# zgchen33/MCGaze

Measured on AMD Instinct MI355X. Metric: clips/sec (7x3x224x224), higher is better.
Workload: dtype f16x3; 1 GPU; full multiclue_gaze_r50 forward (R-50 + FPN + 4 decoder stages + gaze head), 64 clips/GPU x 7 frames x 3x224x224, 64 clips/step; clips_per_gpu=64, clip_length=7, global_clips=64, chunk_frames=0, parallelism=single GPU, trunk_streams=2

## Files before the change

### include/mcgaze_hip.h

```cpp
#ifndef MCGAZE_HIP_H
#define MCGAZE_HIP_H

#include <stddef.h>
#include <stdint.h>

#ifdef __cplusplus
extern "C" {
#endif

#define MCG_ABI_VERSION 20

enum { MCG_OK = 0, MCG_ERR_ARG = 1, MCG_ERR_HIP = 2, MCG_ERR_UNSUPPORTED = 3, MCG_ERR_WORKSPACE = 4 };
typedef enum { MCG_F32 = 0, MCG_BF16 = 1, MCG_F16X3 = 2, MCG_F16 = 3 } mcg_dtype;
#define MCG_ELEM_BYTES(dt) (((dt) == MCG_BF16 || (dt) == MCG_F16) ? 2 : 4)
typedef void* mcg_stream;

int mcg_abi_version(void);
const char* mcg_build_id(void);
const char* mcg_last_error(void);
int mcg_device_info(int* cu_count, size_t* hbm_bytes, char* arch, int arch_len);

int mcg_nchw_to_nhwc(mcg_stream s, mcg_dtype dt, const float* src, void* dst, int N, int C, int H, int W);
int mcg_nhwc_to_nchw(mcg_stream s, mcg_dtype dt, const void* src, float* dst, int N, int C, int H, int W);

enum { MCG_RES_NONE = 0, MCG_RES_ADD = 1, MCG_RES_UPSAMPLE_ADD = 2 };
enum {
  MCG_FLAG_STAGED_GEMM = 1,
  MCG_FLAG_NO_SPECIALISED = 2,
  MCG_FLAG_NO_ATTN_BLOCK = 4
};
typedef struct {
  const void* x;
  const void* w;
  const float* bias;
  const void* residual;
  void* y;
  int N, H, W, Cin, Cout, KH, KW, stride, pad;
  int relu;
  int residual_mode;
  int Hr, Wr;
  const void* x2;
  int Cin2, stride2, H2, W2;
  int tile;
  int flags;
  float wscale;
} mcg_conv_desc;
int mcg_conv2d(mcg_stream s, mcg_dtype dt, const mcg_conv_desc* d);

int mcg_bottleneck_x3(mcg_stream s, const float* x, const float* src2, const void* wstream, const float* bias, float* y, float* z,
                      int frames, int H, int W, int cm, int nsrc, int cn, void* trace);

size_t mcg_conv3x3_wino_x3_weight_bytes(int Cin, int Cout, int g);
int mcg_conv3x3_wino_x3(mcg_stream s, const float* x, const void* u, const float* bias, float* y, int frames, int H, int W,
                        int Cin, int Cout, int relu, int tile, float wscale, int g);
int mcg_conv3x3_wino_x3_blocks(mcg_stream s, const float* x, const void* u, const float* bias, float* y, int frames, int H, int W,
                               int Cin, int Cout, int relu, float wscale, const int* block_list, const int* block_count, int max_blocks,
                               int grid_cap);

int mcg_pointwise_stream(mcg_stream s, mcg_dtype dt, const void* a, const void* wf, const float* bias, const void* res, void* y,
                         int M, int K, int N, int relu, int res_mode, int Ho, int Wo, int Hr, int Wr, float wscale,
                         const int* block_list, const int* block_count, int grid_cap);
int mcg_pointwise_dyn(mcg_stream s, mcg_dtype dt, const void* a, const void* wf, const float* bias, void* y, int M, float wscale, int grid_cap);
int mcg_pointwise_pair(mcg_stream s, mcg_dtype dt, const void* a1, const void* a2, const void* res, const void* w3f, const float* b3,
                       void* y, const void* w1f, const float* b1, void* z, int M, int K2, int C2, int grid_cap);

size_t mcg_stem_workspace_bytes(mcg_dtype dt, int N, int H, int W);
int mcg_stem_forward(mcg_stream s, mcg_dtype dt, const float* img, const void* w_stem, const float* bias,
                     void* y, int N, int H, int W, void* ws, size_t ws_bytes, int flags);

int mcg_roi_align(mcg_stream s, mcg_dtype dt, const void* const feats[4], const int feat_h[4], const int feat_w[4],
                  const int strides[4], int C, const float* boxes, int num_boxes, int boxes_per_frame,
                  void* out, int32_t* levels_out);
int mcg_roi_align_indexed(mcg_stream s, mcg_dtype dt, const void* const feats[4], const int feat_h[4], const int feat_w[4],
                          const int strides[4], int C, const float* boxes, int num_boxes, int boxes_per_frame,
                          const int32_t* frame_of, int pyramid_frames, void* out, int32_t* levels_out);
int mcg_roi_mark_blocks(mcg_stream s, const float* boxes, int num_boxes, int boxes_per_frame, int level, int H, int W, int stride,
                        int* state, int* list, int* count);

enum {
  MCG_SW_IN_PROJ_W = 0, MCG_SW_IN_PROJ_B, MCG_SW_OUT_PROJ_W, MCG_SW_OUT_PROJ_B, MCG_SW_ATTN_LN_G, MCG_SW_ATTN_LN_B,
  MCG_SW_DYN_W,
  MCG_SW_DYN_B,
  MCG_SW_NORM_IN_G, MCG_SW_NORM_IN_B, MCG_SW_NORM_OUT_G, MCG_SW_NORM_OUT_B,
  MCG_SW_FC_W, MCG_SW_FC_B, MCG_SW_FC_LN_G, MCG_SW_FC_LN_B, MCG_SW_IIC_LN_G, MCG_SW_IIC_LN_B,
  MCG_SW_FFN1_W, MCG_SW_FFN1_B, MCG_SW_FFN2_W, MCG_SW_FFN2_B, MCG_SW_FFN_LN_G, MCG_SW_FFN_LN_B,
  MCG_SW_CLS_FC_W, MCG_SW_CLS_LN_G, MCG_SW_CLS_LN_B,
  MCG_SW_REG_FC_W,
  MCG_SW_REG_LN_G,
  MCG_SW_REG_LN_B,
  MCG_SW_HEAD_CLS_W,
  MCG_SW_HEAD_CLS_B,
  MCG_SW_HEAD_REG_W,
  MCG_SW_HEAD_REG_B,
  MCG_SW_OUT_PROJ_WF, MCG_SW_CLS_FC_WF,
  MCG_SW_REG_FC_WF,
  MCG_SW_IN_PROJ_WF,
  MCG_SW_DYN_WF,
  MCG_SW_COUNT
};
enum {
  MCG_GW_FC_W = 0,
  MCG_GW_LN_G,
  MCG_GW_LN_B,
  MCG_GW_OUT_W,
  MCG_GW_OUT_B,
  MCG_GW_FUSE_W,
  MCG_GW_FUSE_B,
  MCG_GW_COUNT
};

size_t mcg_stage_workspace_bytes(mcg_dtype dt, int num_frames);
int mcg_stage_forward(mcg_stream s, mcg_dtype dt, const void* const weights[MCG_SW_COUNT], const void* roi_feat,
                      const void* obj_in, const float* boxes_in, int num_frames, int clip_length,
                      void* obj_out, float* boxes_out, float* cls_out, const float bbox_stds[4],
                      void* ws, size_t ws_bytes, int flags);
int mcg_stage_forward_ragged(mcg_stream s, mcg_dtype dt, const void* const weights[MCG_SW_COUNT], const void* roi_feat,
                             const void* obj_in, const float* boxes_in, int num_frames, const int* clip_start, int num_clips,
                             int max_clip_length, void* obj_out, float* boxes_out, float* cls_out, const float bbox_stds[4],
                             void* ws, size_t ws_bytes, int flags);

size_t mcg_gaze_head_workspace_bytes(mcg_dtype dt, int num_frames);
int mcg_gaze_head(mcg_stream s, mcg_dtype dt, const void* const weights[MCG_GW_COUNT], const void* obj,
                  int num_frames, float* gaze_out, void* ws, size_t ws_bytes);

typedef struct {
  const void* w;
  const float* bias;
  int cin, cout, k, stride, pad;
  const void* wf;
  float wscale;
  const void* wf4;
} mcg_conv_weights;

typedef struct {
  const void* wstream;
  const float* bias;
  int conv2_index;
  int cm, c, cn;
  int nsrc;
} mcg_fused_block;

typedef struct {
  int blocks[4];
  mcg_conv_weights stem;
  const mcg_conv_weights* convs;
  int num_convs;
  mcg_conv_weights lateral[4];
  mcg_conv_weights fpn_out[4];
  mcg_conv_weights c3_ds[4];
  const float* init_boxes;
  const void* init_feats;
  int num_stages;
  const void* const* stage_weights;
  const void* const* gaze_weights;
  float bbox_stds[4];
  const mcg_fused_block* fused;
  int num_fused;
} mcg_model_weights;

typedef struct mcg_engine mcg_engine;
int mcg_engine_create(mcg_engine** out, const mcg_model_weights* w, mcg_dtype dt);
void mcg_engine_destroy(mcg_engine* e);
int mcg_engine_set_option(mcg_engine* e, const char* name, int value);
int mcg_engine_range_audit(mcg_engine* e, unsigned long long* counts, const char** names, int capacity, int* n_out);
size_t mcg_engine_workspace_bytes(const mcg_engine* e, int num_frames, int H, int W, int chunk_frames);
int mcg_backbone_fpn_forward(mcg_engine* e, mcg_stream s, const float* img, int num_frames, int H, int W,
                             int chunk_frames, void* const pyramid[4], void* ws, size_t ws_bytes);
size_t mcg_trunk_workspace_bytes(const mcg_engine* e, int num_frames, int H, int W, int chunk_frames);
size_t mcg_decoder_workspace_bytes(const mcg_engine* e, int num_frames);
int mcg_decoder_forward(mcg_engine* e, mcg_stream s, const void* const pyramid[4], int num_frames, int clip_length, int H, int W,
                        const int* img_hw, float* gaze_out, float* boxes_out, float* scores_out, void* ws, size_t ws_bytes);
int mcg_decoder_forward_indexed(mcg_engine* e, mcg_stream s, const void* const pyramid[4], int pyramid_frames, const int32_t* frame_of,
                                int num_frames, int clip_length, int H, int W, const int* img_hw, float* gaze_out, float* boxes_out,
                                float* scores_out, void* ws, size_t ws_bytes);
int mcg_decoder_forward_ragged(mcg_engine* e, mcg_stream s, const void* const pyramid[4], int pyramid_frames, const int32_t* frame_of,
                               int num_frames, const int* clip_start, int num_clips, int max_clip_length, int H, int W, const int* img_hw,
                               float* gaze_out, float* boxes_out, float* scores_out, void* ws, size_t ws_bytes);
size_t mcg_deferred_pyramid_bytes(const mcg_engine* e, int num_frames, int H, int W);
int mcg_deferred_pyramid_levels(const mcg_engine* e, void* slot, int num_frames, int H, int W, void* levels[4], int* deferred);
int mcg_deferred_pyramid_state(const mcg_engine* e, void* slot, int num_frames, int H, int W, void** inner, int** flags, int** counts,
                               int** lists, int* blocks, int* lateral_deferred);
int mcg_inner_block_neighbours(int id, int H, int W, int out[9]);
int mcg_inner_mark_blocks(mcg_stream s, const int* out_list, const int* out_count, int H, int W, int nblk, int* state, int* list, int* count);
int mcg_backbone_fpn_forward_deferred(mcg_engine* e, mcg_stream s, const float* img, int num_frames, int H, int W, int chunk_frames,
                                      void* slot, size_t slot_bytes, void* ws, size_t ws_bytes);
int mcg_decoder_forward_deferred(mcg_engine* e, mcg_stream s, void* slot, size_t slot_bytes, int num_frames, int clip_length, int H, int W,
                                 const int* img_hw, float* gaze_out, float* boxes_out, float* scores_out, void* ws, size_t ws_bytes);
int mcg_decoder_forward_deferred_ragged(mcg_engine* e, mcg_stream s, void* slot, size_t slot_bytes, int num_frames, const int* clip_start,
                                        int num_clips, int max_clip_length, int H, int W, const int* img_hw, float* gaze_out,
                                        float* boxes_out, float* scores_out, void* ws, size_t ws_bytes);
int mcg_clip_forward(mcg_engine* e, mcg_stream s, const float* img, int num_frames, int clip_length, int H, int W,
                     const int* img_hw, int chunk_frames, float* gaze_out, float* boxes_out, float* scores_out,
                     void* ws, size_t ws_bytes);
int mcg_clip_forward_ragged(mcg_engine* e, mcg_stream s, const float* img, int num_frames, const int* clip_start, int num_clips,
                            int max_clip_length, int H, int W, const int* img_hw, int chunk_frames, float* gaze_out, float* boxes_out,
                            float* scores_out, void* ws, size_t ws_bytes);
int mcg_pyramid_scatter_rows(mcg_stream s, mcg_dtype dt, const void* const src[4], void* const dst[4],
                             int num_frames, int store_rows, int H, int W, const int32_t* row_of);
int mcg_merge_windows(mcg_stream s, const float* gaze, const float* boxes, const float* scores, int num_frames, const float* scale,
                      int scale_per_frame, const int32_t* plan, int num_dst, int max_src, float* store, int store_rows,
                      float person_threshold);
int mcg_smooth_gaze(mcg_stream s, const float* store, int store_rows, const int32_t* plan, int num_out, double alpha, float* out);

typedef struct mcg_frame_desc {
  const void* src;
  int src_h, src_w, src_pitch;
  int crop_y, crop_x, crop_h, crop_w;
  int out_h, out_w;
} mcg_frame_desc;
int mcg_preprocess_frames(mcg_stream stream, const mcg_frame_desc* frames_dev, int num_frames, float* dst, int pad_h, int pad_w,
                          const float mean[3], const float stdinv[3], int to_rgb);
typedef struct mcg_image_desc {
  const void* src;
  int h, w, pitch;
} mcg_image_desc;
int mcg_preprocess_head_crops(mcg_stream s, const mcg_image_desc* images_dev, int num_images, const float* boxes_dev,
                              const int32_t* image_of_dev, int n, double expand, int scale_w, int scale_h, mcg_frame_desc* desc_out_dev,
                              int32_t* img_hw_dev, float* scale_factor_dev, int32_t* flags_dev, float* dst, int pad_h, int pad_w,
                              const float mean[3], const float stdinv[3], int to_rgb);
typedef struct mcg_yuv_coef {
  int y_off, cy, cub, cug, cvg, cvr;
} mcg_yuv_coef;
typedef struct mcg_nv12_image_desc {
  const void* y;
  const void* uv;
  int h, w, pitch_y, pitch_uv;
} mcg_nv12_image_desc;
typedef struct mcg_nv12_frame_desc {
  const void* src;
  int src_h, src_w, src_pitch;
  int crop_y, crop_x, crop_h, crop_w;
  int out_h, out_w;
  const void* uv;
  int uv_pitch;
} mcg_nv12_frame_desc;
int mcg_preprocess_frames_nv12(mcg_stream stream, const mcg_nv12_frame_desc* frames_dev, int num_frames, float* dst, int pad_h, int pad_w,
                               const float mean[3], const float stdinv[3], int to_rgb, const mcg_yuv_coef* coef);
int mcg_preprocess_head_crops_nv12(mcg_stream s, const mcg_nv12_image_desc* images_dev, int num_images, const float* boxes_dev,
                                   const int32_t* image_of_dev, int n, double expand, int scale_w, int scale_h,
                                   mcg_nv12_frame_desc* desc_out_dev, int32_t* img_hw_dev, float* scale_factor_dev, int32_t* flags_dev,
                                   float* dst, int pad_h, int pad_w, const float mean[3], const float stdinv[3], int to_rgb,
                                   const mcg_yuv_coef* coef);

typedef struct mcg_arrow_desc {
  int seg[3][2][2];
  int thickness;
  int x0, y0, x1, y1;
  int image, flag;
  int reserved;
} mcg_arrow_desc;
int mcg_draw_gaze_arrows(mcg_stream s, const mcg_image_desc* images_dev, int num_images, int max_h, int max_w, const float* boxes_dev,
                         const float* gaze_dev, int gaze_stride, const int32_t* image_of_dev, int n, double length, int min_thickness,
                         double thickness_ratio, double tip_length, const unsigned char* color, const unsigned char* colors_dev,
                         mcg_arrow_desc* plan_out_dev, int32_t* flags_dev);
int mcg_draw_gaze_arrows_nv12(mcg_stream s, const mcg_nv12_image_desc* images_dev, int num_images, int max_h, int max_w, const float* boxes_dev,
                              const float* gaze_dev, int gaze_stride, const int32_t* image_of_dev, int n, double length, int min_thickness,
                              double thickness_ratio, double tip_length, const unsigned char* yuv, const unsigned char* yuvs_dev,
                              mcg_arrow_desc* plan_out_dev, int32_t* flags_dev);

size_t mcg_detect_heads_workspace_bytes(int num_images, int num_anchors);
int mcg_detect_heads(mcg_stream s, const float* pred_dev, int num_images, int num_anchors, int num_classes, long long image_stride, int row_stride,
                     int in_h, int in_w, const int32_t* frame_hw_dev , double conf_thres, double iou_thres,
                     int only_class , int agnostic, int max_nms, int max_det,
                     float* boxes_dev , float* scores_dev , int32_t* classes_dev ,
                     int32_t* image_of_dev , int32_t* counts_dev , int32_t* flags_dev ,
                     void* ws_dev, size_t ws_bytes);

enum { MCG_LETTERBOX_U8 = 0, MCG_LETTERBOX_F16 = 1, MCG_LETTERBOX_F32 = 2 };
typedef struct mcg_letterbox_desc {
  mcg_frame_desc frame;
  int top, left;
} mcg_letterbox_desc;
typedef struct mcg_nv12_letterbox_desc {
  mcg_nv12_frame_desc frame;
  int top, left;
} mcg_nv12_letterbox_desc;
int mcg_letterbox_frames(mcg_stream stream, const mcg_letterbox_desc* frames_dev, int num_frames, void* dst, int out_h, int out_w, int out_type,
                         int swap_rb);
int mcg_letterbox_frames_nv12(mcg_stream stream, const mcg_nv12_letterbox_desc* frames_dev, int num_frames, void* dst, int out_h, int out_w,
                              int out_type, int swap_rb, const mcg_yuv_coef* coef);

typedef struct mcg_track_header {
  int32_t next_id;
  int32_t frames_seen;
  int32_t reserved[2];
} mcg_track_header;
typedef struct mcg_track_slot {
  float box[4];
  int32_t id;
  int32_t age;
  int32_t reserved[2];
} mcg_track_slot;
size_t mcg_track_state_bytes(int num_sequences, int slots);
int mcg_track_heads(mcg_stream s, const float* boxes_dev, long long frame_stride, const int32_t* counts_dev, int num_sequences, int num_frames,
                    int max_det, int slots, double match_iou, int max_age, void* state_dev,
                    float* slot_boxes_dev , int32_t* image_of_dev , int32_t* track_id_dev ,
                    int32_t* age_dev , int32_t* det_of_dev , int32_t* flags_dev );

int mcg_track_heads_motion(mcg_stream s, const float* boxes_dev, long long frame_stride, const int32_t* counts_dev, int num_sequences,
                           int num_frames, int max_det, int slots, double match_iou, int max_age, double velocity_gain, double coast_decay,
                           void* state_dev, float* slot_boxes_dev , int32_t* image_of_dev ,
                           int32_t* track_id_dev , int32_t* age_dev , int32_t* det_of_dev ,
                           int32_t* flags_dev , float* state_boxes_dev );

int mcg_live_slots(mcg_stream s, const void* state_dev, int num_cameras, int slots, int tick, int ring_depth, float* crop_boxes_dev,
                   int32_t* image_of_dev, int32_t* ring_id_dev, float* ring_box_dev, int32_t* matched_dev);
int mcg_live_gate(mcg_stream s, const int32_t* ring_id_dev, const float* ring_box_dev, int ring_depth, int num_cameras, int slots, int tick,
                  const int32_t* table_dev, int num_entries, int first_out, int num_out, const float* fused_dev, const float* others_dev,
                  float* fused_smooth_dev, float* others_smooth_dev, int32_t* track_id_dev, int32_t* valid_dev, float* head_box_dev,
                  int32_t* image_of_dev, int32_t* smooth_valid_dev);

int mcg_live_lanes(mcg_stream s, const void* state_dev, int num_cameras, int slots, int lanes, int tick, int ring_depth,
                   int32_t* lane_state_dev, float* crop_boxes_dev, int32_t* image_of_dev, int32_t* ring_id_dev, float* ring_box_dev,
                   int32_t* ring_col_dev, int32_t* lane_of_dev, int32_t* matched_dev, int32_t* overflow_dev);
int mcg_live_gate_lanes(mcg_stream s, const int32_t* ring_id_dev, const float* ring_box_dev, const int32_t* ring_col_dev, int ring_depth,
                        int num_cameras, int slots, int lanes, int tick, const int32_t* table_dev, int num_entries, int first_out, int num_out,
                        const float* fused_dev, const float* others_dev, float* fused_smooth_dev, float* others_smooth_dev,
                        int32_t* track_id_dev, int32_t* valid_dev, int32_t* camera_dev, int32_t* slot_dev, float* head_box_dev,
                        int32_t* image_of_dev, int32_t* smooth_valid_dev);

int mcg_gaze_targets(mcg_stream s, const float* boxes_dev, const float* gaze_dev, int gaze_stride, const int32_t* image_of_dev, int n,
                     const float* regions_dev, const int32_t* region_image_dev, int m, int region_period, double expand, double camera_cos2,
                     int32_t* kind_dev, int32_t* target_dev, float* t_dev, float* hit_dev, int32_t* mutual_dev, int32_t* flags_dev);

int mcg_gaze_dwell(mcg_stream s, const int32_t* person_dev, const int32_t* tag_dev, const int32_t* kind_dev, const int32_t* ident_dev,
                   const int32_t* mutual_dev, int num_frames, int columns, int frame0, int enter, int exit_frames, int32_t* state_dev,
                   int32_t* region_frames_dev, int num_regions, int32_t* dwell_dev, int32_t* ended_dev, int32_t* events_dev, int max_events,
                   int32_t* num_events_dev);

#define MCG_ATTEND_POLY_VERTS 32
int mcg_gaze_targets_poly(mcg_stream s, const float* boxes_dev, const float* gaze_dev, int gaze_stride, const int32_t* image_of_dev, int n,
                          const float* region_xy_dev, int num_vertices, const int32_t* region_start_dev, const int32_t* region_image_dev, int m,
                          int region_period, double expand, double camera_cos2, int32_t* kind_dev, int32_t* target_dev, float* t_dev,
                          float* hit_dev, int32_t* mutual_dev, int32_t* flags_dev);

typedef struct mcg_stroke_desc {
  int seg[3][2][2];
  int thickness;
  int x0, y0, x1, y1;
  int image, flag;
  int layer, count;
  unsigned color, color_active;
  int reserved;
} mcg_stroke_desc;
int mcg_draw_attention(mcg_stream s, const mcg_image_desc* images_dev, int num_images, int max_h, int max_w, const float* boxes_dev,
                       const float* gaze_dev, int gaze_stride, const int32_t* image_of_dev, int n, const int32_t* kind_dev, const int32_t* target_dev,
                       const float* hit_dev, const int32_t* mutual_dev, const float* region_xy_dev, int num_vertices,
                       const int32_t* region_start_dev, const int32_t* region_image_dev, int m, int region_period, const unsigned char* palette,
                       double length, int min_thickness, double thickness_ratio, double tip_length, int line_thickness, int region_thickness,
                       void* workspace_dev, size_t workspace_bytes, int32_t* flags_dev, int32_t* region_flags_dev, int32_t* region_active_dev);
int mcg_draw_attention_nv12(mcg_stream s, const mcg_nv12_image_desc* images_dev, int num_images, int max_h, int max_w, const float* boxes_dev,
                            const float* gaze_dev, int gaze_stride, const int32_t* image_of_dev, int n, const int32_t* kind_dev,
                            const int32_t* target_dev, const float* hit_dev, const int32_t* mutual_dev, const float* region_xy_dev, int num_vertices,
                            const int32_t* region_start_dev, const int32_t* region_image_dev, int m, int region_period, const unsigned char* palette,
                            double length, int min_thickness, double thickness_ratio, double tip_length, int line_thickness, int region_thickness,
                            void* workspace_dev, size_t workspace_bytes, int32_t* flags_dev, int32_t* region_flags_dev, int32_t* region_active_dev);

#define MCG_LABEL_CHARS 24
typedef struct mcg_label_desc {
  int x, y;
  int x0, y0, x1, y1;
  int image, flag;
  int len;
  unsigned color;
  unsigned char text[MCG_LABEL_CHARS];
} mcg_label_desc;
int mcg_format_labels(mcg_stream s, const int32_t* id_dev, const int32_t* value_dev, int n, int num, int den, unsigned char* text_out_dev);
int mcg_draw_labels(mcg_stream s, const mcg_image_desc* images_dev, int num_images, int max_h, int max_w, const float* boxes_dev,
                    const int32_t* image_of_dev, const unsigned char* text_dev, const int32_t* place_dev, int n, const unsigned char* font_dev,
                    int scale, int advance, int pad, const unsigned char* color, const unsigned char* colors_dev, const unsigned char* background,
                    mcg_label_desc* plan_out_dev, int32_t* flags_dev);
int mcg_draw_labels_nv12(mcg_stream s, const mcg_nv12_image_desc* images_dev, int num_images, int max_h, int max_w, const float* boxes_dev,
                         const int32_t* image_of_dev, const unsigned char* text_dev, const int32_t* place_dev, int n, const unsigned char* font_dev,
                         int scale, int advance, int pad, const unsigned char* yuv, const unsigned char* yuvs_dev, const unsigned char* background,
                         mcg_label_desc* plan_out_dev, int32_t* flags_dev);

int mcg_gaze_heat_add(mcg_stream s, const float* hit_dev, const int32_t* kind_dev, const int32_t* image_of_dev, const int32_t* flags_dev,
                      const int32_t* mask_dev, int n, int32_t* heat_dev, int32_t* peak_dev, int C, int GH, int GW, int cell_shift, int radius,
                      int kinds, int period, int decay_shift, void* workspace_dev, size_t workspace_bytes);
int mcg_draw_heat(mcg_stream s, const mcg_image_desc* images_dev, int num_images, int max_h, int max_w, const int32_t* heat_dev,
                  const int32_t* full_dev, int C, int GH, int GW, int cell_shift, int period, const unsigned char* lut_dev, int min_level);
int mcg_draw_heat_nv12(mcg_stream s, const mcg_nv12_image_desc* images_dev, int num_images, int max_h, int max_w, const int32_t* heat_dev,
                       const int32_t* full_dev, int C, int GH, int GW, int cell_shift, int period, const unsigned char* lut_dev, int min_level);

typedef struct mcg_anon_desc {
  int image, flag;
  int x0, y0, x1, y1;
  int cx2, cy2;
  int W, H;
  int shift, shape;
} mcg_anon_desc;
int mcg_anonymize_heads(mcg_stream s, const mcg_image_desc* images_dev, int num_images, int max_h, int max_w, const float* boxes_dev,
                        const int32_t* image_of_dev, int n, double expand, int shape, int cell_shift, int blocks, int mode,
                        const unsigned char* color, mcg_anon_desc* plan_out_dev, int32_t* flags_dev);
int mcg_anonymize_heads_nv12(mcg_stream s, const mcg_nv12_image_desc* images_dev, int num_images, int max_h, int max_w, const float* boxes_dev,
                             const int32_t* image_of_dev, int n, double expand, int shape, int cell_shift, int blocks, int mode,
                             const unsigned char* yuv, mcg_anon_desc* plan_out_dev, int32_t* flags_dev);

int mcg_engine_profile_start(mcg_engine* e, int capacity);
int mcg_engine_profile_stop(mcg_engine* e, int* count, float* ms, double* flops, double* algo_bytes, int* cfg, int* shape_mnk, int capacity);
int mcg_bench_backbone_forward(mcg_engine* e, mcg_stream s, const float* img, int num_frames, int H, int W, void* ws, size_t ws_bytes);
int mcg_bench_backbone_levels(const mcg_engine* e, void* ws, int num_frames, int H, int W, void* levels[4]);

#ifdef __cplusplus
}
#endif
#endif
```

### mcgaze_amd/csrc/check_resources.py

```python
#!/usr/bin/env python3
import re
import sys

RULES = {
    'wino_x3w_kernel': dict(scratch=0, vgpr_spill=0, unit='engine'),
    'wino_x3w_blocks_kernel': dict(scratch=0, vgpr_spill=0, unit='engine'),
    'gaze_targets_kernel': dict(scratch=0, vgpr_spill=0, unit='attend'),
    'gaze_targets_poly_kernel': dict(scratch=0, vgpr_spill=0, unit='attend'),
    'gaze_mutual_kernel': dict(scratch=0, vgpr_spill=0, unit='attend'),
    'gaze_dwell_kernel': dict(scratch=0, vgpr_spill=0, unit='dwell'),
    'gaze_dwell_events_kernel': dict(scratch=0, vgpr_spill=0, unit='dwell'),
    'label_raster_kernel': dict(scratch=0, vgpr_spill=0, unit='labels'),
    'heat_render_kernel': dict(scratch=0, vgpr_spill=0, unit='heat'),
    'anonymize_render_kernel': dict(scratch=0, vgpr_spill=0, unit='anonymize'),
}


def parse(path):
    kernels, cur = [], None
    for line in open(path, errors='replace'):
        m = re.search(r'remark: (?:\s*)Function Name: (\S+)', line)
        if m:
            cur = dict(name=m.group(1))
            kernels.append(cur)
            continue
        m = re.search(r'remark:\s+([A-Za-z \[\]/]+): (\S+) \[-Rpass-analysis', line)
        if m and cur is not None:
            cur[m.group(1).strip()] = m.group(2)
    return kernels


def main():
    path = sys.argv[1]
    kernels = parse(path)
    other = [l.rstrip() for l in open(path, errors='replace') if 'Rpass-analysis=kernel-resource-usage' not in l and not re.match(r'\s+\d* *\|', l) and l.strip()
             and not l.startswith('In file included from') and not re.match(r'\d+ (warning|remark)s? generated', l.strip())]
    for l in other:
        print(l, file=sys.stderr)
    bad = []
    import os
    unit = os.path.basename(path).split('.')[0]
    for prefix, lim in RULES.items():
        if lim.get('unit') == unit and not any(prefix in k['name'] and 'VGPRs Spill' in k and 'ScratchSize [bytes/lane]' in k for k in kernels):
            bad.append(f'{prefix}: no resource remarks found in {path} (expected -Rpass-analysis=kernel-resource-usage output for it)')
    for k in kernels:
        for prefix, lim in RULES.items():
            if prefix in k['name']:
                scratch = int(k.get('ScratchSize [bytes/lane]', '0'))
                spill = int(k.get('VGPRs Spill', '0'))
                if scratch > lim['scratch'] or spill > lim['vgpr_spill']:
                    bad.append(f"{k['name']}: scratch {scratch} B/lane, {spill} spilled VGPRs (limits {lim['scratch']}, {lim['vgpr_spill']})")
    if '--table' in sys.argv:
        print('| kernel | VGPRs | AGPRs | SGPRs | scratch B/lane | VGPR spill | waves/SIMD |\n|---|---|---|---|---|---|---|')
        for k in kernels:
            print(f"| `{k['name']}` | {k.get('VGPRs')} | {k.get('AGPRs')} | {k.get('TotalSGPRs')} | {k.get('ScratchSize [bytes/lane]')} | {k.get('VGPRs Spill')} | {k.get('Occupancy [waves/SIMD]')} |")
    if bad:
        print('check_resources: kernels that must not spill (RULES):\n  ' + '\n  '.join(bad), file=sys.stderr)
        return 1
    return 0


if __name__ == '__main__':
    sys.exit(main())
```

### mcgaze_amd/csrc/engine.hip

```cpp
#include "igemm.hpp"
#include "pw_pair.hpp"
#include "pw_single.hpp"
#include "bneck_x3.hpp"
#include "pw_single_x3.hpp"
#include "wino_x3.hpp"

#include <stdarg.h>
#include <stdlib.h>
#include <string.h>

#include <map>
#include <mutex>
#include <string>
#include <vector>

int launch_roi_align(hipStream_t s, mcg_dtype dt, const void* const feats[4], const int feat_h[4], const int feat_w[4],
                     const int strides[4], int C, const float* boxes, int num_boxes, int boxes_per_frame, const int32_t* frame_of,
                     int pyramid_frames, void* out, int32_t* levels_out);
int launch_init_queries(hipStream_t s, mcg_dtype dt, const float* init_boxes, const void* init_feats, const int* img_hw,
                        const int32_t* frame_of, int pyramid_frames, int H, int W, float* boxes, void* obj, int N);
bool roi_mark_supported(int H, int W);
int launch_defer_clear(hipStream_t s, int* p, int n);
int launch_roi_mark(hipStream_t s, const float* boxes, int num_boxes, int boxes_per_frame, int level, int H, int W, int stride, int* state,
                    int* list, int* count);
int launch_inner_mark(hipStream_t s, const int* out_list, const int* out_count, int H, int W, int nblk, int* state, int* list, int* count);

struct mcg_engine {
  mcg_dtype dt;
  int blocks[4];
  mcg_conv_weights stem;
  std::vector<mcg_conv_weights> convs;
  mcg_conv_weights lateral[4], fpn_out[4], c3_ds[4];
  std::vector<mcg_fused_block> fused;
  bool bneck_fused = true;
  bool bneck_blocked = true;
  int winograd = 1;
  int wino_tile = -1;
  int fpn_deferred = 1;
  int fpn_lateral_deferred = 1;
  static constexpr int kAuditCap = 256;
  unsigned long long* audit_dev = nullptr;
  std::vector<std::string> audit_names;
  const float* init_boxes;
  const void* init_feats;
  int num_stages;
  std::vector<const void*> stage_w;
  const void* gaze_w[MCG_GW_COUNT];
  float stds[4];
  static constexpr int kMaxSplit = 4, kCandidates = 8;
  struct StreamPool* pool = nullptr;
  hipStream_t* cand = nullptr;
  hipEvent_t ev_fork = nullptr, ev_join[kMaxSplit - 1] = {};
  McgCtx ctx;
  Prof prof;
  int trunk_streams = 2;
  int max_range_frames = 0;
  bool pw_single = true;
  bool pw_pair = true;
  std::mutex mu;
};
struct StreamPool {
  hipStream_t cand[mcg_engine::kCandidates] = {};
  hipEvent_t ev_probe[3] = {};
  std::map<hipStream_t, std::vector<int>> side_of;
  std::mutex mu;
  bool ok = false;
};
static StreamPool* stream_pool_for_current_device() {
  static std::mutex g_mu;
  static std::map<int, StreamPool*> g_pools;
  int dev = 0;
  if (hipGetDevice(&dev) != hipSuccess) return nullptr;
  std::lock_guard<std::mutex> lock(g_mu);
  auto it = g_pools.find(dev);
  if (it != g_pools.end()) return it->second;
  StreamPool* p = new StreamPool();
  bool ok = true;
  for (int i = 0; i < mcg_engine::kCandidates; ++i) ok = ok && hipStreamCreateWithFlags(&p->cand[i], hipStreamNonBlocking) == hipSuccess;
  for (int i = 0; i < 3; ++i) ok = ok && hipEventCreate(&p->ev_probe[i]) == hipSuccess;
  p->ok = ok;
  g_pools[dev] = p;
  return p;
}
__global__ void probe_spin_kernel(long long ticks) {
  const long long t0 = wall_clock64();
  while (wall_clock64() - t0 < ticks) {}
}
static const std::vector<int>& side_streams_for(mcg_engine* e, hipStream_t s) {
  StreamPool* p = e->pool;
  std::lock_guard<std::mutex> lock(p->mu);
  auto it = p->side_of.find(s);
  if (it != p->side_of.end()) return it->second;
  std::vector<int> good, rest;
  const long long ticks = 15000;
  for (int c = 0; c < mcg_engine::kCandidates; ++c) {
    bool concurrent = false;
    if (hipEventRecord(p->ev_probe[0], s) == hipSuccess) {
      hipLaunchKernelGGL(probe_spin_kernel, dim3(1), dim3(64), 0, s, ticks);
      hipLaunchKernelGGL(probe_spin_kernel, dim3(1), dim3(64), 0, p->cand[c], ticks);
      float ms = 0.f;
      if (hipEventRecord(p->ev_probe[1], s) == hipSuccess && hipEventRecord(p->ev_probe[2], p->cand[c]) == hipSuccess &&
          hipEventSynchronize(p->ev_probe[1]) == hipSuccess && hipEventSynchronize(p->ev_probe[2]) == hipSuccess &&
          hipEventElapsedTime(&ms, p->ev_probe[0], p->ev_probe[2]) == hipSuccess)
        concurrent = ms < 0.15f * 1.6f;
    }
    (concurrent ? good : rest).push_back(c);
  }
  (void)hipGetLastError();
  good.insert(good.end(), rest.begin(), rest.end());
  return p->side_of.emplace(s, good).first->second;
}
static int range_frame_cap(const mcg_engine* e, int H, int W) {
  const long long per_frame = (long long)(H / 4) * (W / 4) * 256 * (mcg_is16(e->dt) ? 2 : 4);
  long long cap = 0x7FFFFF00ll / (per_frame > 0 ? per_frame : 1);
  if (e->max_range_frames > 0 && e->max_range_frames < cap) cap = e->max_range_frames;
  return cap < 1 ? 1 : (cap > 0x7fffffff ? 0x7fffffff : (int)cap);
}
static const int kMinFramesPerRange = 56;
static int trunk_ranges(const mcg_engine* e, int frames) {
  int k = e->trunk_streams;
  if (k > mcg_engine::kMaxSplit) k = mcg_engine::kMaxSplit;
  while (k > 1 && frames / k < kMinFramesPerRange) --k;
  return k < 1 ? 1 : k;
}

static inline size_t al256(size_t b) { return (b + 255) / 256 * 256; }
static inline size_t esize(mcg_dtype dt) { return mcg_is16(dt) ? 2 : 4; }

extern "C" void mcg_engine_destroy(mcg_engine* e);
extern "C" int mcg_engine_create(mcg_engine** out, const mcg_model_weights* w, mcg_dtype dt) {
  MCG_CHECK_ARG(out && w, "mcg_engine_create: null pointer");
  MCG_CHECK_ARG(dt == MCG_F32 || dt == MCG_BF16 || dt == MCG_F16X3 || dt == MCG_F16, "mcg_engine_create: unknown dtype %d", (int)dt);
  int expect = 0;
  for (int l = 0; l < 4; ++l) {
    MCG_CHECK_ARG(w->blocks[l] > 0, "mcg_engine_create: blocks[%d]=%d", l, w->blocks[l]);
    expect += 3 * w->blocks[l] + 1;
  }
  MCG_CHECK_ARG(w->num_convs == expect && w->convs, "mcg_engine_create: expected %d bottleneck convs, got %d", expect, w->num_convs);
  MCG_CHECK_ARG(w->num_stages > 0 && w->stage_weights && w->gaze_weights && w->init_boxes && w->init_feats, "mcg_engine_create: decoder tables missing");
  for (int i = 0; i < w->num_convs; ++i)
    MCG_CHECK_ARG(w->convs[i].w && w->convs[i].bias, "mcg_engine_create: conv %d has a null pointer", i);
  mcg_engine* e = new mcg_engine();
  e->dt = dt;
  memcpy(e->blocks, w->blocks, sizeof(e->blocks));
  e->stem = w->stem;
  e->convs.assign(w->convs, w->convs + w->num_convs);
  memcpy(e->lateral, w->lateral, sizeof(e->lateral));
  memcpy(e->fpn_out, w->fpn_out, sizeof(e->fpn_out));
  memcpy(e->c3_ds, w->c3_ds, sizeof(e->c3_ds));
  if (w->fused && w->num_fused > 0 && dt == MCG_F16X3) e->fused.assign(w->fused, w->fused + w->num_fused);
  e->init_boxes = w->init_boxes;
  e->init_feats = w->init_feats;
  e->num_stages = w->num_stages;
  e->stage_w.assign(w->stage_weights, w->stage_weights + (size_t)w->num_stages * MCG_SW_COUNT);
  memcpy(e->gaze_w, w->gaze_weights, sizeof(e->gaze_w));
  memcpy(e->stds, w->bbox_stds, sizeof(e->stds));
  bool ok = hipEventCreateWithFlags(&e->ev_fork, hipEventDisableTiming) == hipSuccess;
  e->pool = stream_pool_for_current_device();
  ok = ok && e->pool && e->pool->ok;
  if (e->pool) e->cand = e->pool->cand;
  for (int i = 0; i < mcg_engine::kMaxSplit - 1; ++i) ok = ok && hipEventCreateWithFlags(&e->ev_join[i], hipEventDisableTiming) == hipSuccess;
  if (!ok) {
    mcg_engine_destroy(e);
    mcg_set_error("mcg_engine_create: could not create the side streams / events");
    return MCG_ERR_HIP;
  }
  *out = e;
  return MCG_OK;
}

extern "C" int mcg_engine_set_option(mcg_engine* e, const char* name, int value) {
  MCG_CHECK_ARG(e && name, "mcg_engine_set_option: null pointer");
  std::lock_guard<std::mutex> lock(e->mu);
  if (!strcmp(name, "trunk_streams")) { MCG_CHECK_ARG(value >= 1 && value <= mcg_engine::kMaxSplit, "trunk_streams must be 1..%d", mcg_engine::kMaxSplit); e->trunk_streams = value; }
  else if (!strcmp(name, "max_range_frames")) { MCG_CHECK_ARG(value >= 0, "max_range_frames must be >= 0"); e->max_range_frames = value; }
  else if (!strcmp(name, "tile")) e->ctx.tile = value > 0 ? value : -1;
  else if (!strcmp(name, "staged_gemm")) e->ctx.staged = value != 0;
  else if (!strcmp(name, "conv3x3_c64")) e->ctx.c64 = value != 0;
  else if (!strcmp(name, "stem_fused")) e->ctx.stem_fused = value != 0;
  else if (!strcmp(name, "decoder_chain")) e->ctx.chain = value != 0;
  else if (!strcmp(name, "decoder_attn_block")) e->ctx.attn_block = value != 0;
  else if (!strcmp(name, "pointwise_pair")) e->pw_pair = value != 0;
  else if (!strcmp(name, "pointwise_stream")) e->pw_single = value != 0;
  else if (!strcmp(name, "bottleneck_fused")) e->bneck_fused = value != 0;
  else if (!strcmp(name, "bottleneck_blocked")) e->bneck_blocked = value != 0;
  else if (!strcmp(name, "winograd")) { MCG_CHECK_ARG(value >= 0 && value <= 2, "winograd must be 0, 1 or 2"); e->winograd = value; }
  else if (!strcmp(name, "fpn_deferred")) e->fpn_deferred = value != 0;
  else if (!strcmp(name, "fpn_lateral_deferred")) e->fpn_lateral_deferred = value != 0;
  else if (!strcmp(name, "wino_tile")) { MCG_CHECK_ARG(value >= -1 && value <= 3, "wino_tile must be -1 (by grid size) .. 3"); e->wino_tile = value; }
  else if (!strcmp(name, "range_audit")) {
    MCG_CHECK_ARG(!mcg_is16(e->dt) || !value, "range_audit: f32-storage engines only (MCG_F32, MCG_F16X3)");
    if (value && !e->audit_dev) {
      if (hipMalloc((void**)&e->audit_dev, sizeof(unsigned long long) * 2 * mcg_engine::kAuditCap) != hipSuccess) { e->audit_dev = nullptr; mcg_set_error("range_audit: hipMalloc failed"); return MCG_ERR_HIP; }
    }
    if (value && hipMemset(e->audit_dev, 0, sizeof(unsigned long long) * 2 * mcg_engine::kAuditCap) != hipSuccess) { mcg_set_error("range_audit: hipMemset failed"); return MCG_ERR_HIP; }
    if (!value && e->audit_dev) { (void)hipFree(e->audit_dev); e->audit_dev = nullptr; }
    e->audit_names.clear();
  }
  else { mcg_set_error("mcg_engine_set_option: unknown option '%s'", name); return MCG_ERR_ARG; }
  return MCG_OK;
}

extern "C" int mcg_engine_profile_start(mcg_engine* e, int capacity) {
  MCG_CHECK_ARG(e, "mcg_engine_profile_start: null engine");
  std::lock_guard<std::mutex> lock(e->mu);
  if (e->prof.recs) { mcg_set_error("mcg_engine_profile_start: already armed"); return MCG_ERR_ARG; }
  MCG_CHECK_ARG(capacity > 0 && capacity <= (1 << 20), "mcg_engine_profile_start: bad capacity %d", capacity);
  e->prof.recs = new ProfRec[capacity];
  for (int i = 0; i < capacity; ++i) { e->prof.recs[i].a = nullptr; e->prof.recs[i].b = nullptr; }
  for (int i = 0; i < capacity; ++i) {
    if (hipEventCreate(&e->prof.recs[i].a) != hipSuccess || hipEventCreate(&e->prof.recs[i].b) != hipSuccess) {
      for (int j = 0; j <= i; ++j) {
        if (e->prof.recs[j].a) (void)hipEventDestroy(e->prof.recs[j].a);
        if (e->prof.recs[j].b) (void)hipEventDestroy(e->prof.recs[j].b);
      }
      delete[] e->prof.recs;
      e->prof = Prof();
      mcg_set_error("mcg_engine_profile_start: hipEventCreate failed");
      return MCG_ERR_HIP;
    }
  }
  e->prof.cap = capacity; e->prof.n = 0;
  e->ctx.prof = &e->prof;
  return MCG_OK;
}
extern "C" int mcg_engine_profile_stop(mcg_engine* e, int* count, float* ms, double* flops, double* bytes, int* cfg, int* shape, int capacity) {
  MCG_CHECK_ARG(e, "mcg_engine_profile_stop: null engine");
  std::lock_guard<std::mutex> lock(e->mu);
  if (!e->prof.recs) { mcg_set_error("mcg_engine_profile_stop: not armed"); return MCG_ERR_ARG; }
  const int n = e->prof.n;
  int rc = MCG_OK;
  for (int i = 0; i < n; ++i) {
    const ProfRec& r = e->prof.recs[i];
    float t = 0.f;
    if (hipEventSynchronize(r.b) != hipSuccess || hipEventElapsedTime(&t, r.a, r.b) != hipSuccess) rc = MCG_ERR_HIP;
    if (i < capacity) {
      if (ms) ms[i] = t;
      if (flops) flops[i] = r.flops;
      if (bytes) bytes[i] = r.bytes;
      if (cfg) cfg[i] = r.cfg;
      if (shape) { shape[3 * i] = r.shape[0]; shape[3 * i + 1] = r.shape[1]; shape[3 * i + 2] = r.shape[2]; }
    }
  }
  for (int i = 0; i < e->prof.cap; ++i) { (void)hipEventDestroy(e->prof.recs[i].a); (void)hipEventDestroy(e->prof.recs[i].b); }
  delete[] e->prof.recs;
  e->prof = Prof();
  e->ctx.prof = nullptr;
  if (count) *count = n < capacity ? n : capacity;
  if (rc != MCG_OK) mcg_set_error("mcg_engine_profile_stop: event query failed");
  return rc;
}
extern "C" void mcg_engine_destroy(mcg_engine* e) {
  if (!e) return;
  if (e->ev_fork) (void)hipEventDestroy(e->ev_fork);
  for (int i = 0; i < mcg_engine::kMaxSplit - 1; ++i)
    if (e->ev_join[i]) (void)hipEventDestroy(e->ev_join[i]);
  if (e->prof.recs) {
    for (int i = 0; i < e->prof.cap; ++i) { (void)hipEventDestroy(e->prof.recs[i].a); (void)hipEventDestroy(e->prof.recs[i].b); }
    delete[] e->prof.recs;
  }
  if (e->audit_dev) (void)hipFree(e->audit_dev);
  delete e;
}

__global__ void range_audit_kernel(const float* __restrict__ x, long long n, unsigned long long* __restrict__ cnt) {
  unsigned long long big = 0, bad = 0;
  for (long long i = (long long)blockIdx.x * blockDim.x + threadIdx.x; i < n; i += (long long)gridDim.x * blockDim.x) {
    const float v = x[i];
    if (!(fabsf(v) <= 3.4028235e38f)) ++bad;
    else if (fabsf(v) > 65504.f) ++big;
  }
  big = (unsigned long long)wave_sum((float)big) ;
  bad = (unsigned long long)wave_sum((float)bad);
  if ((threadIdx.x & 63) == 0) {
    if (big) atomicAdd(cnt, big);
    if (bad) atomicAdd(cnt + 1, bad);
  }
}
struct AuditCursor { mcg_engine* e; hipStream_t s; int idx; bool naming; };
__attribute__((format(printf, 4, 5))) static void audit_tensor(AuditCursor& a, const void* p, long long elements, const char* fmt, ...) {
  if (!a.e->audit_dev || a.idx >= mcg_engine::kAuditCap) return;
  if (a.naming) {
    char name[64];
    va_list ap;
    va_start(ap, fmt);
    vsnprintf(name, sizeof(name), fmt, ap);
    va_end(ap);
    a.e->audit_names.push_back(name);
  }
  const long long per_thread = 16;
  long long blocks = (elements + 256 * per_thread - 1) / (256 * per_thread);
  if (blocks > 4096) blocks = 4096;
  if (blocks < 1) blocks = 1;
  hipLaunchKernelGGL(range_audit_kernel, dim3((int)blocks), dim3(256), 0, a.s, (const float*)p, elements, a.e->audit_dev + 2 * a.idx);
  ++a.idx;
}

struct TrunkWs {
  char *stem_ws, *x0, *xa, *xb, *o1, *o2, *ds, *c[4], *l[4];
  size_t stem_bytes, big, total;
};
static TrunkWs trunk_layout(mcg_dtype dt, int n, int H, int W, char* base) {
  const size_t es = esize(dt);
  const size_t h2 = H / 4, w2 = W / 4;
  TrunkWs t;
  size_t off = 0;
  auto take = [&](size_t bytes) { char* p = base ? base + off : nullptr; off += al256(bytes); return p; };
  t.stem_bytes = mcg_stem_workspace_bytes(dt, n, H, W);
  t.stem_ws = take(t.stem_bytes);
  t.big = (size_t)n * h2 * w2 * 256 * es;
  t.x0 = take((size_t)n * h2 * w2 * 64 * es);
  t.xa = take(t.big); t.xb = take(t.big);
  t.o1 = take(t.big / 2); t.o2 = take(t.big / 2);
  t.ds = take(t.big);
  for (int i = 0; i < 4; ++i) {
    const size_t hi = (H / 4) >> i, wi = (W / 4) >> i;
    t.c[i] = take((size_t)n * hi * wi * (256u << i) * es);
    t.l[i] = take((size_t)n * hi * wi * 256 * es);
  }
  t.total = off;
  return t;
}

static int wino_kind(const mcg_engine* e, mcg_dtype dt, const mcg_conv_weights& cw, int n, int h, int w, int rm) {
  return (dt == MCG_F16X3 && e->winograd && e->ctx.tile < 0 && cw.k == 3 && cw.stride == 1 && cw.pad == 1 && rm == MCG_RES_NONE)
             ? ((cw.wf4 && e->winograd >= 2 && wino_x3_applicable(n, h, w, cw.cin, cw.cout, 4)) ? 4 : ((cw.wf && wino_x3_applicable(n, h, w, cw.cin, cw.cout, 2)) ? 2 : 0))
             : 0;
}
static WinoParams wino_params(const mcg_conv_weights& cw, int g, const void* x, int n, int h, int w, void* y, int relu) {
  WinoParams wp;
  memset(&wp, 0, sizeof(wp));
  wp.x = (const float*)x; wp.u = g == 4 ? cw.wf4 : cw.wf; wp.bias = cw.bias; wp.y = (float*)y;
  wp.H = h; wp.W = w; wp.frames = n; wp.Cin = cw.cin; wp.Cout = cw.cout; wp.relu = relu; wp.wscale = cw.wscale;
  return wp;
}
static ProfRec* prof_begin_wino(const McgCtx& ctx, hipStream_t s, const mcg_conv_weights& cw, long long M, bool book = true) {
  return prof_begin(ctx, s, 73, (int)M, cw.cout, 9 * cw.cin, book ? 2.0 * M * 9.0 * cw.cin * cw.cout : 0.0,
                    book ? 4.0 * ((double)M * (cw.cin + cw.cout) + 9.0 * cw.cin * cw.cout) : 0.0);
}
static int launch_done(ProfRec* rec, hipStream_t s, int rc, const char* what) {
  prof_end(rec, s);
  if (rc) { mcg_set_error("%s launch failed", what); return MCG_ERR_HIP; }
  return MCG_OK;
}
static mcg_conv_desc conv_desc(mcg_dtype dt, const mcg_conv_weights& cw, const void* x, int n, int h, int w, void* y, int relu,
                               const void* res, int res_mode, int hr, int wr) {
  mcg_conv_desc d;
  memset(&d, 0, sizeof(d));
  d.x = x; d.w = cw.w; d.bias = cw.bias; d.residual = res; d.y = y;
  d.N = n; d.H = h; d.W = w; d.Cin = cw.cin; d.Cout = cw.cout; d.KH = cw.k; d.KW = cw.k; d.stride = cw.stride; d.pad = cw.pad;
  d.relu = relu; d.residual_mode = res_mode; d.Hr = hr; d.Wr = wr;
  d.wscale = dt == MCG_F16X3 ? cw.wscale : 0.f;
  return d;
}
static int conv_call(const mcg_engine* e, hipStream_t s, mcg_dtype dt, const mcg_conv_weights& cw, const void* x, int n, int h, int w, void* y,
                     int relu, const void* res, int res_mode, int hr, int wr) {
  const long long M = (long long)n * h * w;
  const int rm = res ? res_mode : MCG_RES_NONE;
  const long long res_m = rm == MCG_RES_UPSAMPLE_ADD ? (long long)n * hr * wr : M;
  const bool x3 = dt == MCG_F16X3;
  if ((x3 || mcg_is16(dt)) && e->pw_single && e->ctx.tile < 0 && cw.wf && cw.bias && cw.k == 1 && cw.stride == 1 && cw.pad == 0 && M < 0x7fffffffll &&
      (x3 ? pw_single_x3_applicable(cw.cin, cw.cout, rm, M, res_m) : !e->ctx.staged && pw_single_applicable(cw.cin, cw.cout, rm, M, res_m))) {
    PwSingleParams pp;
    memset(&pp, 0, sizeof(pp));
    pp.a = x; pp.res = res; pp.wf = cw.wf; pp.bias = cw.bias; pp.y = y;
    pp.M = (int)M; pp.relu = relu; pp.Ho = h; pp.Wo = w; pp.wscale = x3 ? cw.wscale : 0.f;
    if (rm == MCG_RES_UPSAMPLE_ADD) { pp.Hr = hr; pp.Wr = wr; pp.rscale_h = (float)hr / (float)h; pp.rscale_w = (float)wr / (float)w; }
    ProfRec* rec = prof_begin(e->ctx, s, x3 ? 71 : 61, pp.M, cw.cout, cw.cin, 2.0 * M * cw.cin * cw.cout,
                              (double)esize(dt) * ((double)M * (cw.cin + cw.cout) + (rm == MCG_RES_NONE ? 0.0 : (double)res_m) * cw.cout + (double)cw.cin * cw.cout));
    const int rmode = rm == MCG_RES_NONE ? 0 : (rm == MCG_RES_ADD ? 1 : 2);
    return launch_done(rec, s, x3 ? launch_pw_single_x3(s, pp, cw.cout, rmode) : launch_pw_single(s, pp, cw.cin, cw.cout, rmode, dt),
                       x3 ? "pw_single_x3" : "pw_single");
  }
  const int wg = wino_kind(e, dt, cw, n, h, w, rm);
  if (wg) {
    ProfRec* rec = prof_begin_wino(e->ctx, s, cw, M);
    return launch_done(rec, s, launch_wino_x3(s, wino_params(cw, wg, x, n, h, w, y, relu), e->wino_tile, wg), "wino_x3");
  }
  const mcg_conv_desc d = conv_desc(dt, cw, x, n, h, w, y, relu, res, res_mode, hr, wr);
  return conv2d_ctx(s, dt, &d, e->ctx);
}

struct TrunkCursor {
  const void* x;
  int h, w, ci;
  char *o1, *o2;
  bool o1_ready;
  bool x_blocked;
};
static const mcg_fused_block* fused_tail_at(const mcg_engine* e, int ci, int b) {
  if (!(e->dt == MCG_F16X3 && e->bneck_fused && e->ctx.tile < 0) || ci + 2 >= (int)e->convs.size()) return nullptr;
  const mcg_fused_block* f = nullptr;
  for (const mcg_fused_block& q : e->fused)
    if (q.conv2_index == ci + 1) f = &q;
  if (!f) return nullptr;
  const bool ds = b == 0;
  const mcg_conv_weights &d2 = e->convs[ci + 1], &d3 = e->convs[ci + 2];
  const int kk = ds ? e->convs[ci + 3].cin : 0, ss = ds ? e->convs[ci + 3].stride : 1;
  const int cn_i = ci + (ds ? 4 : 3);
  const bool nx = f->cn == 0 || (cn_i < (int)e->convs.size() && e->convs[cn_i].k == 1 && e->convs[cn_i].stride == 1 && e->convs[cn_i].cout == f->cn && e->convs[cn_i].cin == f->c);
  return (d2.k == 3 && d2.stride == 1 && d2.pad == 1 && d2.cin == f->cm && d2.cout == f->cm && d3.cout == f->c && f->nsrc == (ds ? 2 : 1) && nx &&
          bneck_x3_applicable(f->cm, f->c, f->cn, f->nsrc, kk, ss)) ? f : nullptr;
}
static int fused_tail_step(const mcg_engine* e, hipStream_t s, const TrunkWs& t, AuditCursor& au, TrunkCursor& c, const mcg_fused_block* fb,
                           int n, int l, int b, void* y) {
  const bool has_ds = b == 0;
  const int k2 = has_ds ? e->convs[c.ci + 3].cin : 0;
  BneckParams bp;
  memset(&bp, 0, sizeof(bp));
  bp.x = (const float*)c.o1; bp.res = (const float*)c.x; bp.wstream = (const char*)fb->wstream; bp.bias = fb->bias;
  bp.y = (float*)y; bp.z = (float*)c.o2; bp.H = c.h; bp.W = c.w;
  const long long blk_bytes = (long long)n * ((c.h + bnx::TH - 1) / bnx::TH) * ((c.w + bnx::TW - 1) / bnx::TW) * bnx::NPIX * fb->c * (long long)esize(e->dt);
  const mcg_fused_block* fnext = (b + 1 < e->blocks[l]) ? fused_tail_at(e, c.ci + (has_ds ? 4 : 3), b + 1) : nullptr;
  bp.res_blocked = c.x_blocked ? 1 : 0;
  bp.y_blocked = (e->bneck_blocked && !e->audit_dev && y != (void*)t.c[l] && fb->cn > 0 && fnext && fnext->nsrc == 1 && fnext->c == fb->c &&
                  blk_bytes <= (long long)t.big) ? 1 : 0;
  const double M = (double)n * c.h * c.w;
  ProfRec* rec = prof_begin(e->ctx, s, 70, n * c.h * c.w, fb->c + fb->cn, 9 * fb->cm + fb->cm + k2 + fb->c,
                            2.0 * M * (9.0 * fb->cm * fb->cm + (double)(fb->cm + k2) * fb->c + (double)fb->c * fb->cn),
                            4.0 * (M * (fb->cm + (has_ds ? k2 : fb->c) + fb->c + fb->cn) + 9.0 * fb->cm * fb->cm + (double)(fb->cm + k2) * fb->c + (double)fb->c * fb->cn));
  MCG_TRY(launch_done(rec, s, launch_bneck_x3(s, bp, n, fb->cm, fb->nsrc, fb->cn), "bneck_x3"));
  audit_tensor(au, y, (long long)n * c.h * c.w * fb->c, "layer%d.%d.out (fused tail)", l + 1, b);
  if (fb->cn > 0) {
    audit_tensor(au, c.o2, (long long)n * c.h * c.w * fb->cn, "layer%d.%d.next_conv1 (fused tail)", l + 1, b);
    std::swap(c.o1, c.o2);
    c.o1_ready = true;
  }
  c.x_blocked = bp.y_blocked != 0;
  return MCG_OK;
}
static const mcg_conv_weights* pw_pair_next(const mcg_engine* e, int ci, int l, int b, long long M) {
  const bool has_ds = b == 0;
  const mcg_conv_weights& c3 = e->convs[ci + 2];
  const mcg_conv_weights* c3w = has_ds ? (e->c3_ds[l].w ? &e->c3_ds[l] : nullptr) : &c3;
  const int ci_next = ci + (has_ds ? 4 : 3);
  const mcg_conv_weights* c1n = ci_next < (int)e->convs.size() ? &e->convs[ci_next] : nullptr;
  const int k2 = has_ds ? e->convs[ci + 3].cin : 0;
  return (mcg_is16(e->dt) && e->pw_pair && l == 0 && c3w && c1n && c3w->wf && c1n->wf && c3w->bias && c1n->bias && c1n->k == 1 && c1n->stride == 1 &&
          c1n->cin == c3.cout && pw_pair_applicable(c3.cin, k2, has_ds ? e->convs[ci + 3].stride : 1, c3.cout, c1n->cout, M) && M < 0x7fffffffll)
             ? c1n : nullptr;
}
static int pw_pair_step(const mcg_engine* e, hipStream_t s, TrunkCursor& c, const mcg_conv_weights& c1n, int n, int l, int b, void* y, int ho, int wo) {
  const bool has_ds = b == 0;
  const mcg_conv_weights& c3 = e->convs[c.ci + 2];
  const mcg_conv_weights& c3w = has_ds ? e->c3_ds[l] : c3;
  PwPairParams pp;
  memset(&pp, 0, sizeof(pp));
  pp.a1 = c.o2; pp.K1 = c3.cin;
  if (has_ds) { pp.a2 = c.x; pp.K2 = e->convs[c.ci + 3].cin; pp.stride2 = e->convs[c.ci + 3].stride; pp.H2 = c.h; pp.W2 = c.w; }
  else pp.res = c.x;
  pp.w3f = c3w.wf; pp.b3 = c3w.bias; pp.y = y;
  pp.w1f = c1n.wf; pp.b1 = c1n.bias; pp.z = c.o1;
  pp.M = n * ho * wo; pp.C = c3.cout; pp.C2 = c1n.cout; pp.Ho = ho; pp.Wo = wo;
  ProfRec* rec = prof_begin(e->ctx, s, 60, pp.M, pp.C + pp.C2, pp.K1 + pp.K2, 2.0 * pp.M * ((double)(pp.K1 + pp.K2) * pp.C + (double)pp.C * pp.C2),
                            2.0 * ((double)pp.M * (pp.K1 + pp.K2 + (has_ds ? 0 : pp.C) + pp.C + pp.C2) + (double)(pp.K1 + pp.K2) * pp.C + (double)pp.C * pp.C2));
  MCG_TRY(launch_done(rec, s, launch_pw_pair(s, pp, e->dt), "pw_pair"));
  c.o1_ready = true;
  return MCG_OK;
}
static int conv3_step(const mcg_engine* e, hipStream_t s, const TrunkWs& t, AuditCursor& au, const TrunkCursor& c, int n, int l, int b, void* y,
                      int ho, int wo) {
  const mcg_conv_weights& c3 = e->convs[c.ci + 2];
  if (b == 0 && e->c3_ds[l].w) {
    const mcg_conv_weights& ds = e->convs[c.ci + 3];
    mcg_conv_desc d = conv_desc(e->dt, e->c3_ds[l], c.o2, n, ho, wo, y, 1, nullptr, MCG_RES_NONE, 0, 0);
    d.Cin = c3.cin;
    d.x2 = c.x; d.Cin2 = ds.cin; d.stride2 = ds.stride; d.H2 = c.h; d.W2 = c.w;
    MCG_TRY(conv2d_ctx(s, e->dt, &d, e->ctx));
  } else {
    const void* identity = c.x;
    if (b == 0) {
      MCG_TRY(conv_call(e, s, e->dt, e->convs[c.ci + 3], c.x, n, c.h, c.w, t.ds, 0, nullptr, MCG_RES_NONE, 0, 0));
      identity = t.ds;
    }
    MCG_TRY(conv_call(e, s, e->dt, c3, c.o2, n, ho, wo, y, 1, identity, MCG_RES_ADD, 0, 0));
  }
  audit_tensor(au, y, (long long)n * ho * wo * c3.cout, "layer%d.%d.out", l + 1, b);
  return MCG_OK;
}

struct TrunkKeep { char *inner, *c2, *l1; };
static int trunk_chunk(mcg_engine* e, hipStream_t s, const float* img, int f0, int n, int H, int W, void* const pyr[4], char* wsbase,
                       bool backbone_only = false, const TrunkKeep tk = TrunkKeep{nullptr, nullptr, nullptr}) {
  const mcg_dtype dt = e->dt;
  const size_t es = esize(dt);
  TrunkWs t = trunk_layout(dt, n, H, W, wsbase);
  char* const inner0 = tk.inner;
  if (inner0) t.l[0] = inner0 + (size_t)f0 * (H / 4) * (W / 4) * 256 * es;
  const bool lateral_deferred = inner0 && tk.c2 && tk.l1;
  if (lateral_deferred) {
    t.c[0] = tk.c2 + (size_t)f0 * (H / 4) * (W / 4) * 256 * es;
    t.l[1] = tk.l1 + (size_t)f0 * (H / 8) * (W / 8) * 256 * es;
  }
  MCG_TRY(stem_forward_ctx(s, dt, img + (size_t)f0 * 3 * H * W, e->stem.w, e->stem.bias, t.x0, n, H, W, t.stem_ws, t.stem_bytes, e->ctx));
  AuditCursor au{e, s, 0, e->audit_dev != nullptr && e->audit_names.empty()};
  audit_tensor(au, t.x0, (long long)n * (H / 4) * (W / 4) * 64, "stem");
  TrunkCursor c{t.x0, H / 4, W / 4, 0, t.o1, t.o2, false, false};
  for (int l = 0; l < 4; ++l) {
    for (int b = 0; b < e->blocks[l]; ++b) {
      const mcg_conv_weights &c1 = e->convs[c.ci], &c2 = e->convs[c.ci + 1];
      const int ho = (c.h + 2 * c2.pad - c2.k) / c2.stride + 1, wo = (c.w + 2 * c2.pad - c2.k) / c2.stride + 1;
      void* y = (b == e->blocks[l] - 1) ? (void*)t.c[l] : (c.x == t.xa ? (void*)t.xb : (void*)t.xa);
      if (!c.o1_ready) {
        MCG_TRY(conv_call(e, s, dt, c1, c.x, n, c.h, c.w, c.o1, 1, nullptr, MCG_RES_NONE, 0, 0));
        audit_tensor(au, c.o1, (long long)n * c.h * c.w * c1.cout, "layer%d.%d.conv1", l + 1, b);
      }
      c.o1_ready = false;
      const mcg_fused_block* fb = fused_tail_at(e, c.ci, b);
      if (c.x_blocked && !(fb && fb->nsrc == 1)) { mcg_set_error("trunk: a blocked tensor reached a kernel that does not read that layout"); return MCG_ERR_UNSUPPORTED; }
      if (fb) {
        MCG_TRY(fused_tail_step(e, s, t, au, c, fb, n, l, b, y));
      } else {
        MCG_TRY(conv_call(e, s, dt, c2, c.o1, n, c.h, c.w, c.o2, 1, nullptr, MCG_RES_NONE, 0, 0));
        audit_tensor(au, c.o2, (long long)n * ho * wo * c2.cout, "layer%d.%d.conv2", l + 1, b);
        const mcg_conv_weights* c1n = pw_pair_next(e, c.ci, l, b, (long long)n * ho * wo);
        MCG_TRY(c1n ? pw_pair_step(e, s, c, *c1n, n, l, b, y, ho, wo) : conv3_step(e, s, t, au, c, n, l, b, y, ho, wo));
      }
      c.x = y; c.h = ho; c.w = wo;
      c.ci += b == 0 ? 4 : 3;
    }
  }
  if (backbone_only) return MCG_OK;
  int hs[4], wsz[4];
  for (int i = 0; i < 4; ++i) { hs[i] = (H / 4) >> i; wsz[i] = (W / 4) >> i; }
  for (int i = 3; i >= (lateral_deferred ? 1 : 0); --i) {
    const void* res = i == 3 ? nullptr : t.l[i + 1];
    MCG_TRY(conv_call(e, s, dt, e->lateral[i], t.c[i], n, hs[i], wsz[i], t.l[i], 0, res, res ? MCG_RES_UPSAMPLE_ADD : MCG_RES_NONE,
                      i == 3 ? 0 : hs[i + 1], i == 3 ? 0 : wsz[i + 1]));
    audit_tensor(au, t.l[i], (long long)n * hs[i] * wsz[i] * 256, "fpn.lateral%d (+ top-down)", i);
  }
  for (int i = inner0 ? 1 : 0; i < 4; ++i) {
    char* dst = (char*)pyr[i] + (size_t)f0 * hs[i] * wsz[i] * 256 * es;
    MCG_TRY(conv_call(e, s, dt, e->fpn_out[i], t.l[i], n, hs[i], wsz[i], dst, 0, nullptr, MCG_RES_NONE, 0, 0));
    audit_tensor(au, dst, (long long)n * hs[i] * wsz[i] * 256, "fpn.P%d", i + 2);
  }
  return MCG_OK;
}

extern "C" int mcg_engine_range_audit(mcg_engine* e, unsigned long long* counts, const char** names, int capacity, int* n_out) {
  MCG_CHECK_ARG(e && counts && n_out && capacity > 0, "mcg_engine_range_audit: bad argument");
  std::lock_guard<std::mutex> lock(e->mu);
  if (!e->audit_dev) { mcg_set_error("mcg_engine_range_audit: the range_audit option is off"); return MCG_ERR_ARG; }
  const int n = (int)e->audit_names.size() < capacity ? (int)e->audit_names.size() : capacity;
  if (hipDeviceSynchronize() != hipSuccess ||
      hipMemcpy(counts, e->audit_dev, sizeof(unsigned long long) * 2 * n, hipMemcpyDeviceToHost) != hipSuccess ||
      hipMemset(e->audit_dev, 0, sizeof(unsigned long long) * 2 * mcg_engine::kAuditCap) != hipSuccess) {
    mcg_set_error("mcg_engine_range_audit: device read failed");
    return MCG_ERR_HIP;
  }
  if (names) for (int i = 0; i < n; ++i) names[i] = e->audit_names[i].c_str();
  *n_out = n;
  return MCG_OK;
}

struct DecWs {
  char *roi, *obj_a, *obj_b, *stage_ws, *gaze_ws;
  float *boxes_a, *boxes_b, *cls;
  size_t stage_bytes, gaze_bytes, total;
};
static DecWs dec_layout(mcg_dtype dt, int N, char* base) {
  const size_t es = esize(dt), R = (size_t)N * 3;
  DecWs c;
  memset(&c, 0, sizeof(c));
  size_t off = 0;
  auto take = [&](size_t bytes) { char* p = base ? base + off : nullptr; off += al256(bytes); return p; };
  c.roi = take(R * 49 * 256 * es);
  c.obj_a = take(R * 256 * es); c.obj_b = take(R * 256 * es);
  c.boxes_a = (float*)take(R * 4 * 4); c.boxes_b = (float*)take(R * 4 * 4); c.cls = (float*)take(R * 4);
  c.stage_bytes = mcg_stage_workspace_bytes(dt, N); c.stage_ws = take(c.stage_bytes);
  c.gaze_bytes = mcg_gaze_head_workspace_bytes(dt, N); c.gaze_ws = take(c.gaze_bytes);
  c.total = off;
  return c;
}
static bool check_shape_ok(int N, int H, int W) { return N > 0 && H >= 32 && W >= 32 && H % 32 == 0 && W % 32 == 0; }
static size_t pyramid_bytes(mcg_dtype dt, int N, int H, int W, int level) {
  return al256((size_t)N * ((H / 4) >> level) * ((W / 4) >> level) * 256 * esize(dt));
}

struct DeferSlot {
  void* p[4];
  char* inner;
  int *state, *count, *list;
  int nblk;
  bool deferred;
  bool lateral;
  char *c2, *l1;
  int *istate, *icount, *ilist;
  size_t total;
};
static bool fpn_deferred_on(const mcg_engine* e, int N, int H, int W) {
  const mcg_conv_weights& cw = e->fpn_out[0];
  const int h = H / 4, w = W / 4;
  return e->fpn_deferred && e->dt == MCG_F16X3 && !e->audit_dev && e->num_stages > 0 && wino_kind(e, e->dt, cw, N, h, w, MCG_RES_NONE) == 2 &&
         wino_x3_blocks_applicable(N, h, w, cw.cin, cw.cout) && roi_mark_supported(h, w);
}
static bool fpn_lateral_deferred_on(const mcg_engine* e, int N, int H, int W) {
  const mcg_conv_weights& cw = e->lateral[0];
  const int h = H / 4, w = W / 4;
  return e->fpn_lateral_deferred && fpn_deferred_on(e, N, H, W) && e->pw_single && e->ctx.tile < 0 && cw.wf && cw.bias && cw.k == 1 && cw.stride == 1 &&
         cw.pad == 0 && h % 2 == 0 && w % 2 == 0 &&
         pw_single_x3_blocks_applicable(cw.cin, cw.cout, h, w, (long long)N * h * w, (long long)N * (h / 2) * (w / 2));
}
static DeferSlot defer_layout(const mcg_engine* e, int N, int H, int W, char* base) {
  DeferSlot d;
  memset(&d, 0, sizeof(d));
  size_t off = 0;
  auto take = [&](size_t bytes) { char* p = base ? base + off : nullptr; off += al256(bytes); return p; };
  for (int i = 0; i < 4; ++i) d.p[i] = take(pyramid_bytes(e->dt, N, H, W, i));
  d.deferred = fpn_deferred_on(e, N, H, W);
  if (d.deferred) {
    d.inner = take((size_t)N * (H / 4) * (W / 4) * 256 * esize(e->dt));
    d.nblk = N * wino_x3_blocks_per_frame(H / 4, W / 4);
    d.lateral = fpn_lateral_deferred_on(e, N, H, W);
    const size_t per = (size_t)d.nblk + e->num_stages;
    d.state = (int*)take(sizeof(int) * per * (d.lateral ? 2 : 1));
    d.count = d.state ? d.state + d.nblk : nullptr;
    d.list = (int*)take(sizeof(int) * (size_t)d.nblk * e->num_stages);
    if (d.lateral) {
      d.istate = d.state ? d.state + per : nullptr;
      d.icount = d.istate ? d.istate + d.nblk : nullptr;
      d.ilist = (int*)take(sizeof(int) * (size_t)d.nblk * e->num_stages);
      d.c2 = take((size_t)N * (H / 4) * (W / 4) * 256 * esize(e->dt));
      d.l1 = take((size_t)N * (H / 8) * (W / 8) * 256 * esize(e->dt));
    }
  }
  d.total = off;
  return d;
}

extern "C" size_t mcg_trunk_workspace_bytes(const mcg_engine* e, int N, int H, int W, int chunk) {
  if (!e || N <= 0) return 0;
  if (chunk <= 0 || chunk > N) chunk = N;
  if (chunk < N) return trunk_layout(e->dt, chunk, H, W, nullptr).total;
  size_t total = 0;
  const int cap = range_frame_cap(e, H, W);
  for (int k = 1; k <= mcg_engine::kMaxSplit; ++k) {
    const int per = (N + k - 1) / k < cap ? (N + k - 1) / k : cap;
    const size_t t = (size_t)k * al256(trunk_layout(e->dt, per, H, W, nullptr).total);
    if (t > total) total = t;
  }
  return total;
}
extern "C" size_t mcg_decoder_workspace_bytes(const mcg_engine* e, int N) {
  if (!e || N <= 0) return 0;
  return dec_layout(e->dt, N, nullptr).total;
}
extern "C" size_t mcg_engine_workspace_bytes(const mcg_engine* e, int N, int H, int W, int chunk) {
  if (!e || N <= 0) return 0;
  return mcg_trunk_workspace_bytes(e, N, H, W, chunk) + mcg_decoder_workspace_bytes(e, N) + defer_layout(e, N, H, W, nullptr).total;
}
extern "C" size_t mcg_deferred_pyramid_bytes(const mcg_engine* e, int N, int H, int W) {
  if (!e || N <= 0 || check_shape_ok(N, H, W) == false) return 0;
  return defer_layout(e, N, H, W, nullptr).total;
}

static int check_shape(int N, int H, int W) {
  MCG_CHECK_ARG(N > 0, "num_frames must be positive (got %d)", N);
  MCG_CHECK_ARG(H >= 32 && W >= 32 && H % 32 == 0 && W % 32 == 0, "frame size %dx%d must be a multiple of 32 (Pad(size_divisor=32))", H, W);
  return MCG_OK;
}

static int trunk_forward(mcg_engine* e, mcg_stream s_, const float* img, int N, int H, int W, int chunk,
                         void* const pyramid[4], void* ws, size_t ws_bytes, bool backbone_only, const TrunkKeep tk = TrunkKeep{nullptr, nullptr, nullptr}) {
  MCG_CHECK_ARG(e && img && (pyramid || backbone_only) && ws, "mcg_backbone_fpn_forward: null pointer");
  MCG_TRY(check_shape(N, H, W));
  std::lock_guard<std::mutex> lock(e->mu);
  if (chunk <= 0 || chunk > N) chunk = N;
  const size_t need = mcg_trunk_workspace_bytes(e, N, H, W, chunk);
  if (ws_bytes < need) { mcg_set_error("mcg_backbone_fpn_forward: workspace too small (%zu < %zu)", ws_bytes, need); return MCG_ERR_WORKSPACE; }
  const int k = chunk < N ? 1 : trunk_ranges(e, N), cap = range_frame_cap(e, H, W);
  const int per = chunk < N ? chunk : ((N + k - 1) / k < cap ? (N + k - 1) / k : cap);
  const hipStream_t s = (hipStream_t)s_;
  hipStream_t si[mcg_engine::kMaxSplit] = {s};
  if (k > 1) {
    const std::vector<int>& sides = side_streams_for(e, s);
    for (int i = 1; i < k; ++i) si[i] = e->cand[sides[i - 1]];
    if (hipEventRecord(e->ev_fork, s) != hipSuccess) { mcg_set_error("mcg_backbone_fpn_forward: hipEventRecord failed"); return MCG_ERR_HIP; }
    for (int i = 1; i < k; ++i)
      if (hipStreamWaitEvent(si[i], e->ev_fork, 0) != hipSuccess) { mcg_set_error("mcg_backbone_fpn_forward: hipStreamWaitEvent failed"); return MCG_ERR_HIP; }
  }
  const size_t part_ws = k > 1 ? al256(trunk_layout(e->dt, per, H, W, nullptr).total) : 0;
  int rc = MCG_OK;
  for (int f0 = 0, i = 0; f0 < N && rc == MCG_OK; f0 += per, i = (i + 1) % k)
    rc = trunk_chunk(e, si[i], img, f0, (N - f0) < per ? (N - f0) : per, H, W, pyramid, (char*)ws + (size_t)i * part_ws, backbone_only, tk);
  for (int i = 1; i < k; ++i) {
    if (hipEventRecord(e->ev_join[i - 1], si[i]) != hipSuccess || hipStreamWaitEvent(s, e->ev_join[i - 1], 0) != hipSuccess) {
      mcg_set_error("mcg_backbone_fpn_forward: join failed");
      rc = rc == MCG_OK ? MCG_ERR_HIP : rc;
    }
  }
  return rc;
}

extern "C" int mcg_bottleneck_x3(mcg_stream s, const float* x, const float* src2, const void* wstream, const float* bias, float* y, float* z,
                                 int frames, int H, int W, int cm, int nsrc, int cn, void* trace) {
  MCG_CHECK_ARG(x && src2 && wstream && bias && y && (z || cn == 0), "mcg_bottleneck_x3: null pointer");
  MCG_CHECK_ARG(frames > 0 && H > 0 && W > 0, "mcg_bottleneck_x3: empty problem");
  MCG_CHECK_ARG(bneck_x3_applicable(cm, 4 * cm, cn, nsrc, 64, 1), "mcg_bottleneck_x3: unsupported shape (cm=%d nsrc=%d cn=%d)", cm, nsrc, cn);
  BneckParams bp;
  memset(&bp, 0, sizeof(bp));
  bp.x = x; bp.res = src2; bp.wstream = (const char*)wstream; bp.bias = bias; bp.y = y; bp.z = z; bp.H = H; bp.W = W; bp.trace = (unsigned long long*)trace;
  if (launch_bneck_x3((hipStream_t)s, bp, frames, cm, nsrc, cn)) { mcg_set_error("mcg_bottleneck_x3: launch failed"); return MCG_ERR_HIP; }
  return MCG_OK;
}

extern "C" size_t mcg_conv3x3_wino_x3_weight_bytes(int Cin, int Cout, int g) {
  return (Cin > 0 && Cout > 0 && Cin % 32 == 0 && Cout % wnx::UNT == 0 && (g == 2 || g == 4)) ? wino_x3_weight_bytes(Cin, Cout, g) : 0;
}
extern "C" int mcg_conv3x3_wino_x3(mcg_stream s, const float* x, const void* u, const float* bias, float* y, int frames, int H, int W,
                                   int Cin, int Cout, int relu, int tile, float wscale, int g) {
  MCG_CHECK_ARG(x && u && y, "mcg_conv3x3_wino_x3: null pointer");
  MCG_CHECK_ARG(tile >= 0 && tile <= 4, "mcg_conv3x3_wino_x3: tile must be 0 (by grid size) .. 4");
  if (!wino_x3_applicable(frames, H, W, Cin, Cout, g)) {
    mcg_set_error("mcg_conv3x3_wino_x3: unsupported shape (frames=%d %dx%d, %d -> %d channels, F(%d,3)): Cin %% 32, Cout %% 128, W <= 62 (F(4,3): W %% 4 == 0, W >= 16), a tile's window within its buffer", frames, H, W, Cin, Cout, g);
    return MCG_ERR_UNSUPPORTED;
  }
  WinoParams wp;
  memset(&wp, 0, sizeof(wp));
  wp.x = x; wp.u = u; wp.bias = bias; wp.y = y; wp.H = H; wp.W = W; wp.frames = frames; wp.Cin = Cin; wp.Cout = Cout; wp.relu = relu;
  wp.wscale = wscale;
  if (launch_wino_x3((hipStream_t)s, wp, tile - 1, g)) { mcg_set_error("mcg_conv3x3_wino_x3: launch failed"); return MCG_ERR_HIP; }
  return MCG_OK;
}
extern "C" int mcg_conv3x3_wino_x3_blocks(mcg_stream s, const float* x, const void* u, const float* bias, float* y, int frames, int H, int W,
                                          int Cin, int Cout, int relu, float wscale, const int* block_list, const int* block_count,
                                          int max_blocks, int grid_cap) {
  MCG_CHECK_ARG(x && u && y && block_list && block_count, "mcg_conv3x3_wino_x3_blocks: null pointer");
  MCG_CHECK_ARG(max_blocks > 0 && grid_cap >= 0, "mcg_conv3x3_wino_x3_blocks: max_blocks must be positive and grid_cap >= 0 (max_blocks=%d grid_cap=%d)",
                max_blocks, grid_cap);
  if (H <= 0 || W <= 0 || H % 8 != 0 || W % 8 != 0 || !wino_x3_blocks_applicable(frames, H, W, Cin, Cout)) {
    mcg_set_error("mcg_conv3x3_wino_x3_blocks: unsupported shape (frames=%d %dx%d, %d -> %d channels): H %% 8, W %% 8, Cin %% 32, Cout %% 128, operands within 2 GiB",
                  frames, H, W, Cin, Cout);
    return MCG_ERR_UNSUPPORTED;
  }
  WinoParams wp;
  memset(&wp, 0, sizeof(wp));
  wp.x = x; wp.u = u; wp.bias = bias; wp.y = y; wp.H = H; wp.W = W; wp.frames = frames; wp.Cin = Cin; wp.Cout = Cout; wp.relu = relu;
  wp.wscale = wscale;
  if (launch_wino_x3_blocks((hipStream_t)s, wp, block_list, block_count, max_blocks, grid_cap)) {
    mcg_set_error("mcg_conv3x3_wino_x3_blocks: launch failed");
    return MCG_ERR_HIP;
  }
  return MCG_OK;
}

extern "C" int mcg_pointwise_stream(mcg_stream s, mcg_dtype dt, const void* a, const void* wf, const float* bias, const void* res, void* y,
                                    int M, int K, int N, int relu, int res_mode, int Ho, int Wo, int Hr, int Wr, float wscale,
                                    const int* block_list, const int* block_count, int grid_cap) {
  MCG_CHECK_ARG(a && wf && bias && y, "mcg_pointwise_stream: null pointer");
  MCG_CHECK_ARG(M > 0 && grid_cap >= 0, "mcg_pointwise_stream: M must be positive and grid_cap >= 0 (M=%d grid_cap=%d)", M, grid_cap);
  MCG_CHECK_ARG(res_mode >= MCG_RES_NONE && res_mode <= MCG_RES_UPSAMPLE_ADD && (res != nullptr) == (res_mode != MCG_RES_NONE),
                "mcg_pointwise_stream: res_mode %d needs %s residual", res_mode, res_mode == MCG_RES_NONE ? "no" : "a");
  MCG_CHECK_ARG((block_list != nullptr) == (block_count != nullptr), "mcg_pointwise_stream: block_list and block_count come together");
  const bool x3 = dt == MCG_F16X3, up = res_mode == MCG_RES_UPSAMPLE_ADD;
  if (up) MCG_CHECK_ARG(Ho > 0 && Wo > 0 && Hr > 0 && Wr > 0 && M % ((long long)Ho * Wo) == 0,
                        "mcg_pointwise_stream: upsample residual: M = frames * Ho * Wo (M=%d, %dx%d from %dx%d)", M, Ho, Wo, Hr, Wr);
  const long long res_rows = up ? M / ((long long)Ho * Wo) * Hr * Wr : M;
  bool ok = x3 ? pw_single_x3_dispatched(K, N, M, res_rows) : mcg_is16(dt) && pw_single_dispatched(K, N, res_mode, M, res_rows);
  if (block_list) ok = x3 && up && pw_single_x3_blocks_applicable(K, N, Ho, Wo, M, res_rows);
  if (!ok) {
    mcg_set_error("mcg_pointwise_stream: unsupported (dtype %d, %d -> %d channels, res_mode %d, M=%d%s): see include/mcgaze_hip.h for the table", (int)dt, K, N,
                  res_mode, M, block_list ? ", block list" : "");
    return MCG_ERR_UNSUPPORTED;
  }
  PwSingleParams pp;
  memset(&pp, 0, sizeof(pp));
  pp.a = a; pp.res = res; pp.wf = wf; pp.bias = bias; pp.y = y;
  pp.M = M; pp.relu = relu; pp.Ho = up ? Ho : 1; pp.Wo = up ? Wo : 1; pp.wscale = x3 ? wscale : 0.f;
  if (up) { pp.Hr = Hr; pp.Wr = Wr; pp.rscale_h = (float)Hr / (float)Ho; pp.rscale_w = (float)Wr / (float)Wo; }
  const int rc = block_list ? launch_pw_single_x3_blocks((hipStream_t)s, pp, block_list, block_count, M / 64, grid_cap)
                 : x3       ? launch_pw_single_x3((hipStream_t)s, pp, N, res_mode, grid_cap)
                            : launch_pw_single((hipStream_t)s, pp, K, N, res_mode, dt, grid_cap);
  if (rc) { mcg_set_error("mcg_pointwise_stream: launch failed"); return MCG_ERR_HIP; }
  return MCG_OK;
}

extern "C" int mcg_pointwise_pair(mcg_stream s, mcg_dtype dt, const void* a1, const void* a2, const void* res, const void* w3f, const float* b3,
                                  void* y, const void* w1f, const float* b1, void* z, int M, int K2, int C2, int grid_cap) {
  MCG_CHECK_ARG(a1 && w3f && b3 && y && w1f && b1 && z, "mcg_pointwise_pair: null pointer");
  MCG_CHECK_ARG(M > 0 && grid_cap >= 0, "mcg_pointwise_pair: M must be positive and grid_cap >= 0 (M=%d grid_cap=%d)", M, grid_cap);
  MCG_CHECK_ARG((a2 != nullptr) == (K2 != 0), "mcg_pointwise_pair: a second source comes with K2 = 64, none with K2 = 0");
  if (!mcg_is16(dt) || !pw_pair_applicable(64, K2, 1, 256, C2, M) || (K2 != 0 && res)) {
    mcg_set_error("mcg_pointwise_pair: unsupported (dtype %d, K2=%d, C2=%d, M=%d%s): bf16 / fp16, K2 0 or 64, C2 64 or 128, a residual only without a second source",
                  (int)dt, K2, C2, M, res ? ", residual" : "");
    return MCG_ERR_UNSUPPORTED;
  }
  PwPairParams pp;
  memset(&pp, 0, sizeof(pp));
  pp.a1 = a1; pp.K1 = 64; pp.a2 = a2; pp.K2 = K2; pp.stride2 = 1; pp.res = res;
  pp.w3f = w3f; pp.b3 = b3; pp.y = y; pp.w1f = w1f; pp.b1 = b1; pp.z = z;
  pp.M = M; pp.C = 256; pp.C2 = C2; pp.Ho = 1; pp.Wo = M; pp.H2 = 1; pp.W2 = M;
  if (launch_pw_pair((hipStream_t)s, pp, dt, grid_cap)) { mcg_set_error("mcg_pointwise_pair: launch failed"); return MCG_ERR_HIP; }
  return MCG_OK;
}

extern "C" int mcg_backbone_fpn_forward(mcg_engine* e, mcg_stream s, const float* img, int N, int H, int W, int chunk,
                                        void* const pyramid[4], void* ws, size_t ws_bytes) {
  return trunk_forward(e, s, img, N, H, W, chunk, pyramid, ws, ws_bytes, false);
}
extern "C" int mcg_bench_backbone_forward(mcg_engine* e, mcg_stream s, const float* img, int N, int H, int W, void* ws, size_t ws_bytes) {
  return trunk_forward(e, s, img, N, H, W, 0, nullptr, ws, ws_bytes, true);
}

extern "C" int mcg_bench_backbone_levels(const mcg_engine* e, void* ws, int N, int H, int W, void* levels[4]) {
  MCG_CHECK_ARG(e && ws && levels, "mcg_bench_backbone_levels: null pointer");
  MCG_TRY(check_shape(N, H, W));
  MCG_CHECK_ARG(trunk_ranges(e, N) == 1 && N <= range_frame_cap(e, H, W), "mcg_bench_backbone_levels: the batch runs as several frame ranges (set trunk_streams = 1)");
  const TrunkWs t = trunk_layout(e->dt, N, H, W, (char*)ws);
  for (int i = 0; i < 4; ++i) levels[i] = t.c[i];
  return MCG_OK;
}

static int defer_stage_forward(const mcg_engine* e, hipStream_t s, const DeferSlot& d, int st, const float* boxes, int N, int h, int w) {
  const mcg_conv_weights& cw = e->fpn_out[0];
  int* list = d.list + (size_t)st * d.nblk;
  MCG_TRY(launch_roi_mark(s, boxes, N * 3, 3, 0, h, w, 4, d.state, list, d.count + st));
  if (d.lateral) {
    const mcg_conv_weights& lw = e->lateral[0];
    int* ilist = d.ilist + (size_t)st * d.nblk;
    MCG_TRY(launch_inner_mark(s, list, d.count + st, h, w, d.nblk, d.istate, ilist, d.icount + st));
    const long long M = (long long)N * h * w, res_m = (long long)N * (h / 2) * (w / 2);
    PwSingleParams pp;
    memset(&pp, 0, sizeof(pp));
    pp.a = d.c2; pp.res = d.l1; pp.wf = lw.wf; pp.bias = lw.bias; pp.y = d.inner;
    pp.M = (int)M; pp.relu = 0; pp.Ho = h; pp.Wo = w; pp.wscale = lw.wscale;
    pp.Hr = h / 2; pp.Wr = w / 2; pp.rscale_h = (float)pp.Hr / (float)h; pp.rscale_w = (float)pp.Wr / (float)w;
    const bool book = st == 0;
    ProfRec* lrec = prof_begin(e->ctx, s, 71, pp.M, lw.cout, lw.cin, book ? 2.0 * M * lw.cin * lw.cout : 0.0,
                               book ? 4.0 * ((double)M * (lw.cin + lw.cout) + (double)res_m * lw.cout + (double)lw.cin * lw.cout) : 0.0);
    MCG_TRY(launch_done(lrec, s, launch_pw_single_x3_blocks(s, pp, ilist, d.icount + st, d.nblk), "pw_single_x3 block"));
  }
  ProfRec* rec = prof_begin_wino(e->ctx, s, cw, (long long)N * h * w, st == 0);
  return launch_done(rec, s, launch_wino_x3_blocks(s, wino_params(cw, 2, d.inner, N, h, w, d.p[0], 0), list, d.count + st, d.nblk), "wino_x3 block");
}

static int decoder_forward(mcg_engine* e, hipStream_t s, const void* const pyramid[4], int pyramid_frames, const int32_t* frame_of, int N,
                           const ClipTable& ct, int H, int W, const int* img_hw, float* gaze_out, float* boxes_out, float* scores_out, void* ws,
                           size_t ws_bytes, const DeferSlot* d = nullptr) {
  MCG_CHECK_ARG(e && pyramid && gaze_out && boxes_out && scores_out && ws, "mcg_decoder_forward: null pointer");
  MCG_TRY(check_shape(N, H, W));
  MCG_TRY(check_clips("mcg_decoder_forward", N, ct));
  DecWs c = dec_layout(e->dt, N, (char*)ws);
  if (ws_bytes < c.total) { mcg_set_error("mcg_decoder_forward: workspace too small (%zu < %zu)", ws_bytes, c.total); return MCG_ERR_WORKSPACE; }
  MCG_TRY(launch_init_queries(s, e->dt, e->init_boxes, e->init_feats, img_hw, frame_of, pyramid_frames, H, W, c.boxes_a, c.obj_a, N));
  int fh[4], fw[4];
  const int strides[4] = {4, 8, 16, 32};
  for (int i = 0; i < 4; ++i) { fh[i] = (H / 4) >> i; fw[i] = (W / 4) >> i; }
  char* obj_in = c.obj_a; char* obj_out = c.obj_b;
  float* b_in = c.boxes_a; float* b_out = c.boxes_b;
  const bool defer = d && d->deferred;
  if (defer) MCG_TRY(launch_defer_clear(s, d->state, (d->nblk + e->num_stages) * (d->lateral ? 2 : 1)));
  for (int st = 0; st < e->num_stages; ++st) {
    if (defer) MCG_TRY(defer_stage_forward(e, s, *d, st, b_in, N, fh[0], fw[0]));
    MCG_TRY(launch_roi_align(s, e->dt, pyramid, fh, fw, strides, 256, b_in, N * 3, 3, frame_of, pyramid_frames, c.roi, nullptr));
    float* bdst = (st == e->num_stages - 1) ? boxes_out : b_out;
    MCG_TRY(stage_forward_ctx(s, e->dt, &e->stage_w[(size_t)st * MCG_SW_COUNT], c.roi, obj_in, b_in, N, ct, obj_out, bdst,
                              c.cls, e->stds, c.stage_ws, c.stage_bytes, e->ctx));
    char* t = obj_in; obj_in = obj_out; obj_out = t;
    if (st != e->num_stages - 1) { float* tb = b_in; b_in = b_out; b_out = tb; }
  }
  MCG_TRY(gaze_head_ctx(s, e->dt, e->gaze_w, obj_in, N, gaze_out, c.gaze_ws, c.gaze_bytes, e->ctx, c.cls, scores_out));
  return MCG_OK;
}

extern "C" int mcg_decoder_forward(mcg_engine* e, mcg_stream s_, const void* const pyramid[4], int N, int clip_length, int H, int W,
                                   const int* img_hw, float* gaze_out, float* boxes_out, float* scores_out, void* ws, size_t ws_bytes) {
  return decoder_forward(e, (hipStream_t)s_, pyramid, N, nullptr, N, ClipTable::uniform(N, clip_length), H, W, img_hw, gaze_out, boxes_out, scores_out, ws,
                         ws_bytes);
}

extern "C" int mcg_decoder_forward_indexed(mcg_engine* e, mcg_stream s_, const void* const pyramid[4], int pyramid_frames, const int32_t* frame_of,
                                           int N, int clip_length, int H, int W, const int* img_hw, float* gaze_out, float* boxes_out,
                                           float* scores_out, void* ws, size_t ws_bytes) {
  MCG_CHECK_ARG(frame_of, "mcg_decoder_forward_indexed: null frame_of (mcg_decoder_forward is the plain path)");
  MCG_CHECK_ARG(pyramid_frames > 0, "mcg_decoder_forward_indexed: empty pyramid store (pyramid_frames=%d)", pyramid_frames);
  return decoder_forward(e, (hipStream_t)s_, pyramid, pyramid_frames, frame_of, N, ClipTable::uniform(N, clip_length), H, W, img_hw, gaze_out, boxes_out,
                         scores_out, ws, ws_bytes);
}

extern "C" int mcg_decoder_forward_ragged(mcg_engine* e, mcg_stream s_, const void* const pyramid[4], int pyramid_frames, const int32_t* frame_of,
                                          int N, const int* clip_start, int num_clips, int max_clip_length, int H, int W, const int* img_hw,
                                          float* gaze_out, float* boxes_out, float* scores_out, void* ws, size_t ws_bytes) {
  MCG_CHECK_ARG(clip_start, "mcg_decoder_forward_ragged: null clip_start (mcg_decoder_forward is the equal-length path)");
  MCG_CHECK_ARG(pyramid_frames > 0, "mcg_decoder_forward_ragged: empty pyramid store (pyramid_frames=%d)", pyramid_frames);
  MCG_CHECK_ARG(frame_of || pyramid_frames == N, "mcg_decoder_forward_ragged: without frame_of the pyramid holds one row per frame (%d rows, %d frames)",
                pyramid_frames, N);
  return decoder_forward(e, (hipStream_t)s_, pyramid, pyramid_frames, frame_of, N, ClipTable{clip_start, num_clips, max_clip_length}, H, W, img_hw,
                         gaze_out, boxes_out, scores_out, ws, ws_bytes);
}

extern "C" int mcg_deferred_pyramid_levels(const mcg_engine* e, void* slot, int N, int H, int W, void* levels[4], int* deferred) {
  MCG_CHECK_ARG(e && slot && levels, "mcg_deferred_pyramid_levels: null pointer");
  MCG_TRY(check_shape(N, H, W));
  const DeferSlot d = defer_layout(e, N, H, W, (char*)slot);
  for (int i = 0; i < 4; ++i) levels[i] = d.p[i];
  if (deferred) *deferred = d.deferred ? 1 : 0;
  return MCG_OK;
}

extern "C" int mcg_backbone_fpn_forward_deferred(mcg_engine* e, mcg_stream s, const float* img, int N, int H, int W, int chunk, void* slot,
                                                 size_t slot_bytes, void* ws, size_t ws_bytes) {
  MCG_CHECK_ARG(e && slot, "mcg_backbone_fpn_forward_deferred: null pointer");
  MCG_TRY(check_shape(N, H, W));
  const DeferSlot d = defer_layout(e, N, H, W, (char*)slot);
  if (slot_bytes < d.total) { mcg_set_error("mcg_backbone_fpn_forward_deferred: slot too small (%zu < %zu)", slot_bytes, d.total); return MCG_ERR_WORKSPACE; }
  return trunk_forward(e, s, img, N, H, W, chunk, d.p, ws, ws_bytes, false,
                       TrunkKeep{d.deferred ? d.inner : nullptr, d.lateral ? d.c2 : nullptr, d.lateral ? d.l1 : nullptr});
}

extern "C" int mcg_deferred_pyramid_state(const mcg_engine* e, void* slot, int N, int H, int W, void** inner, int** flags, int** counts, int** lists,
                                          int* blocks, int* lateral_deferred) {
  MCG_CHECK_ARG(e && slot, "mcg_deferred_pyramid_state: null pointer");
  MCG_TRY(check_shape(N, H, W));
  const DeferSlot d = defer_layout(e, N, H, W, (char*)slot);
  if (inner) *inner = d.inner;
  if (flags) *flags = d.istate;
  if (counts) *counts = d.icount;
  if (lists) *lists = d.ilist;
  if (blocks) *blocks = d.nblk;
  if (lateral_deferred) *lateral_deferred = d.lateral ? 1 : 0;
  return MCG_OK;
}

static int decoder_forward_deferred(mcg_engine* e, mcg_stream s, void* slot, size_t slot_bytes, int N, const ClipTable& ct, int H, int W,
                                    const int* img_hw, float* gaze_out, float* boxes_out, float* scores_out, void* ws, size_t ws_bytes) {
  MCG_CHECK_ARG(e && slot, "mcg_decoder_forward_deferred: null pointer");
  MCG_TRY(check_shape(N, H, W));
  const DeferSlot d = defer_layout(e, N, H, W, (char*)slot);
  if (slot_bytes < d.total) { mcg_set_error("mcg_decoder_forward_deferred: slot too small (%zu < %zu)", slot_bytes, d.total); return MCG_ERR_WORKSPACE; }
  return decoder_forward(e, (hipStream_t)s, d.p, N, nullptr, N, ct, H, W, img_hw, gaze_out, boxes_out, scores_out, ws, ws_bytes, &d);
}

extern "C" int mcg_decoder_forward_deferred(mcg_engine* e, mcg_stream s, void* slot, size_t slot_bytes, int N, int clip_length, int H, int W,
                                            const int* img_hw, float* gaze_out, float* boxes_out, float* scores_out, void* ws, size_t ws_bytes) {
  return decoder_forward_deferred(e, s, slot, slot_bytes, N, ClipTable::uniform(N, clip_length), H, W, img_hw, gaze_out, boxes_out, scores_out, ws, ws_bytes);
}

extern "C" int mcg_decoder_forward_deferred_ragged(mcg_engine* e, mcg_stream s, void* slot, size_t slot_bytes, int N, const int* clip_start,
                                                   int num_clips, int max_clip_length, int H, int W, const int* img_hw, float* gaze_out,
                                                   float* boxes_out, float* scores_out, void* ws, size_t ws_bytes) {
  MCG_CHECK_ARG(clip_start, "mcg_decoder_forward_deferred_ragged: null clip_start (mcg_decoder_forward_deferred is the equal-length path)");
  return decoder_forward_deferred(e, s, slot, slot_bytes, N, ClipTable{clip_start, num_clips, max_clip_length}, H, W, img_hw, gaze_out, boxes_out,
                                  scores_out, ws, ws_bytes);
}

static int clip_forward(mcg_engine* e, mcg_stream s_, const float* img, int N, const ClipTable& ct, int H, int W, const int* img_hw, int chunk,
                        float* gaze_out, float* boxes_out, float* scores_out, void* ws, size_t ws_bytes) {
  MCG_CHECK_ARG(e && img && gaze_out && boxes_out && scores_out && ws, "mcg_clip_forward: null pointer");
  MCG_TRY(check_shape(N, H, W));
  MCG_TRY(check_clips("mcg_clip_forward", N, ct));
  const size_t need = mcg_engine_workspace_bytes(e, N, H, W, chunk);
  if (ws_bytes < need) { mcg_set_error("mcg_clip_forward: workspace too small (%zu < %zu)", ws_bytes, need); return MCG_ERR_WORKSPACE; }
  char* base = (char*)ws;
  const size_t trunk_bytes = mcg_trunk_workspace_bytes(e, N, H, W, chunk);
  const size_t slot_bytes = defer_layout(e, N, H, W, nullptr).total;
  const size_t off = trunk_bytes + slot_bytes;
  MCG_TRY(mcg_backbone_fpn_forward_deferred(e, s_, img, N, H, W, chunk, base + trunk_bytes, slot_bytes, base, trunk_bytes));
  return decoder_forward_deferred(e, s_, base + trunk_bytes, slot_bytes, N, ct, H, W, img_hw, gaze_out, boxes_out, scores_out, base + off,
                                  ws_bytes - off);
}

extern "C" int mcg_clip_forward(mcg_engine* e, mcg_stream s_, const float* img, int N, int clip_length, int H, int W,
                                const int* img_hw, int chunk, float* gaze_out, float* boxes_out, float* scores_out,
                                void* ws, size_t ws_bytes) {
  return clip_forward(e, s_, img, N, ClipTable::uniform(N, clip_length), H, W, img_hw, chunk, gaze_out, boxes_out, scores_out, ws, ws_bytes);
}

extern "C" int mcg_clip_forward_ragged(mcg_engine* e, mcg_stream s_, const float* img, int N, const int* clip_start, int num_clips,
                                       int max_clip_length, int H, int W, const int* img_hw, int chunk, float* gaze_out, float* boxes_out,
                                       float* scores_out, void* ws, size_t ws_bytes) {
  MCG_CHECK_ARG(clip_start, "mcg_clip_forward_ragged: null clip_start (mcg_clip_forward is the equal-length path)");
  return clip_forward(e, s_, img, N, ClipTable{clip_start, num_clips, max_clip_length}, H, W, img_hw, chunk, gaze_out, boxes_out, scores_out, ws,
                      ws_bytes);
}
```

### mcgaze_amd/csrc/roi_align.hip

```cpp
#include "common.hpp"
#include "roi_sample.hpp"

struct RoiLevels {
  const void* feat[4];
  int h[4], w[4];
  float scale[4];
};

template <typename T>
__global__ __launch_bounds__(256) void roi_align_kernel(RoiLevels lv, int C, const float* __restrict__ boxes, int boxes_per_frame,
                                                        const int32_t* __restrict__ frame_of, int pyramid_frames,
                                                        T* __restrict__ out, int32_t* __restrict__ levels_out, float finest_scale) {
  constexpr int EPC = Elem<T>::kPerChunk;
  constexpr int P = 7, S = 2, NS = P * S;
  __shared__ int s_lo[2][NS], s_hi[2][NS];
  __shared__ float s_l[2][NS], s_h[2][NS];
  __shared__ int s_valid[2][NS];
  const int box = blockIdx.x, tid = threadIdx.x;
  const float x1 = boxes[box * 4 + 0], y1 = boxes[box * 4 + 1], x2 = boxes[box * 4 + 2], y2 = boxes[box * 4 + 3];
  const int level = roi_level(x1, y1, x2, y2, finest_scale);
  const int H = lv.h[level], W = lv.w[level];
  const float ss = lv.scale[level];
  if (tid < 2 * NS) {
    const int axis = tid / NS, i = tid % NS;
    int lo, hi, valid;
    float l;
    roi_axis_sample<P, S>(axis == 0 ? y1 : x1, axis == 0 ? y2 : x2, ss, axis == 0 ? H : W, i, lo, hi, l, valid);
    s_lo[axis][i] = lo; s_hi[axis][i] = hi; s_l[axis][i] = l; s_h[axis][i] = 1.f - l; s_valid[axis][i] = valid;
  }
  if (tid == 0) {
    if (levels_out) levels_out[box] = level;
  }
  __syncthreads();
  int frame = box / boxes_per_frame;
  bool bad_row = false;
  if (frame_of) {
    frame = __builtin_amdgcn_readfirstlane(frame_of[frame]);
    bad_row = frame < 0 || frame >= pyramid_frames;
    if (bad_row) frame = 0;
  }
  const T* __restrict__ F = (const T*)lv.feat[level] + (long long)frame * H * W * C;
  const int groups = C / EPC, bins_per_pass = 256 / groups;
  const int cg = tid % groups, slot = tid / groups;
  if (bad_row) {
    float nan[EPC];
#pragma unroll
    for (int e = 0; e < EPC; ++e) nan[e] = __builtin_nanf("");
    for (int bin = slot; bin < P * P; bin += bins_per_pass)
      *(uint4*)(out + ((long long)box * (P * P) + bin) * C + cg * EPC) = f32_to_chunk(nan, (T*)nullptr);
    return;
  }
  for (int bin = slot; bin < P * P; bin += bins_per_pass) {
    const int ph = bin / P, pw = bin % P;
    float acc[EPC];
#pragma unroll
    for (int e = 0; e < EPC; ++e) acc[e] = 0.f;
#pragma unroll
    for (int iy = 0; iy < S; ++iy) {
      const int yi = ph * S + iy;
#pragma unroll
      for (int ix = 0; ix < S; ++ix) {
        const int xi = pw * S + ix;
        if (!(s_valid[0][yi] && s_valid[1][xi])) continue;
        const int yl = s_lo[0][yi], yh = s_hi[0][yi], xl = s_lo[1][xi], xh = s_hi[1][xi];
        const float ly = s_l[0][yi], hy = s_h[0][yi], lx = s_l[1][xi], hx = s_h[1][xi];
        const float w1 = hy * hx, w2 = hy * lx, w3 = ly * hx, w4 = ly * lx;
        float v1[EPC], v2[EPC], v3[EPC], v4[EPC];
        chunk_to_f32(*(const uint4*)(F + ((long long)yl * W + xl) * C + cg * EPC), v1, (T*)nullptr);
        chunk_to_f32(*(const uint4*)(F + ((long long)yl * W + xh) * C + cg * EPC), v2, (T*)nullptr);
        chunk_to_f32(*(const uint4*)(F + ((long long)yh * W + xl) * C + cg * EPC), v3, (T*)nullptr);
        chunk_to_f32(*(const uint4*)(F + ((long long)yh * W + xh) * C + cg * EPC), v4, (T*)nullptr);
#pragma unroll
        for (int e = 0; e < EPC; ++e) acc[e] += w1 * v1[e] + w2 * v2[e] + w3 * v3[e] + w4 * v4[e];
      }
    }
#pragma unroll
    for (int e = 0; e < EPC; ++e) acc[e] *= (1.0f / (float)(S * S));
    *(uint4*)(out + ((long long)box * (P * P) + bin) * C + cg * EPC) = f32_to_chunk(acc, (T*)nullptr);
  }
}

constexpr int kMarkMaxBlocks = 64;
__global__ __launch_bounds__(256) void roi_mark_kernel(const float* __restrict__ boxes, int boxes_per_frame, int level_deferred, int H, int W,
                                                       float ss, int* __restrict__ state, int* __restrict__ list, int* __restrict__ count,
                                                       float finest_scale) {
  constexpr int P = 7, S = 2, NS = P * S;
  __shared__ int s_hit[2][kMarkMaxBlocks];
  const int box = blockIdx.x, tid = threadIdx.x;
  const float x1 = boxes[box * 4 + 0], y1 = boxes[box * 4 + 1], x2 = boxes[box * 4 + 2], y2 = boxes[box * 4 + 3];
  if (roi_level(x1, y1, x2, y2, finest_scale) != level_deferred) return;
  const int by_n = (H + 7) / 8, bx_n = (W + 7) / 8;
  if (tid < 2 * kMarkMaxBlocks) s_hit[tid / kMarkMaxBlocks][tid % kMarkMaxBlocks] = 0;
  __syncthreads();
  if (tid < 2 * NS) {
    const int axis = tid / NS, i = tid % NS;
    int lo, hi, valid;
    float l;
    roi_axis_sample<P, S>(axis == 0 ? y1 : x1, axis == 0 ? y2 : x2, ss, axis == 0 ? H : W, i, lo, hi, l, valid);
    if (valid) { s_hit[axis][lo >> 3] = 1; s_hit[axis][hi >> 3] = 1; }
  }
  __syncthreads();
  const int frame = box / boxes_per_frame;
  for (int t = tid; t < by_n * bx_n; t += 256) {
    const int by = t / bx_n, bx = t - by * bx_n;
    if (s_hit[0][by] && s_hit[1][bx]) {
      const int id = frame * (by_n * bx_n) + t;
      if (atomicCAS(&state[id], 0, 1) == 0) list[atomicAdd(count, 1)] = id;
    }
  }
}
__host__ __device__ inline int inner_neighbour(int id, int k, int by_n, int bx_n) {
  const int bpf = by_n * bx_n, f = id / bpf, rem = id - f * bpf, by = rem / bx_n + k / 3 - 1, bx = rem % bx_n + k % 3 - 1;
  return (by < 0 || by >= by_n || bx < 0 || bx >= bx_n) ? -1 : f * bpf + by * bx_n + bx;
}
__global__ __launch_bounds__(256) void inner_mark_kernel(const int* __restrict__ out_list, const int* __restrict__ out_count, int by_n, int bx_n,
                                                         int nblk, int* __restrict__ state, int* __restrict__ list, int* __restrict__ count) {
  const int n = min(*out_count, nblk) * 9;
  for (int t = blockIdx.x * blockDim.x + threadIdx.x; t < n; t += gridDim.x * blockDim.x) {
    const int src = out_list[t / 9];
    if (src < 0 || src >= nblk) continue;
    const int id = inner_neighbour(src, t % 9, by_n, bx_n);
    if (id >= 0 && atomicCAS(&state[id], 0, 1) == 0) list[atomicAdd(count, 1)] = id;
  }
}
int launch_inner_mark(hipStream_t s, const int* out_list, const int* out_count, int H, int W, int nblk, int* state, int* list, int* count) {
  const long long threads = (long long)nblk * 9;
  const int blocks = (int)((threads + 255) / 256 < 1024 ? (threads + 255) / 256 : 1024);
  hipLaunchKernelGGL(inner_mark_kernel, dim3(blocks > 0 ? blocks : 1), dim3(256), 0, s, out_list, out_count, (H + 7) / 8, (W + 7) / 8, nblk, state,
                     list, count);
  MCG_CHECK_LAUNCH("inner_mark");
  return MCG_OK;
}
extern "C" int mcg_inner_block_neighbours(int id, int H, int W, int out[9]) {
  int n = 0;
  for (int k = 0; k < 9; ++k) {
    const int v = inner_neighbour(id, k, (H + 7) / 8, (W + 7) / 8);
    if (v >= 0) out[n++] = v;
  }
  return n;
}
__global__ void defer_clear_kernel(int* __restrict__ p, int n) {
  for (int i = blockIdx.x * blockDim.x + threadIdx.x; i < n; i += gridDim.x * blockDim.x) p[i] = 0;
}
bool roi_mark_supported(int H, int W) { return (H + 7) / 8 <= kMarkMaxBlocks && (W + 7) / 8 <= kMarkMaxBlocks; }
int launch_defer_clear(hipStream_t s, int* p, int n) {
  const int blocks = (n + 255) / 256 < 1024 ? (n + 255) / 256 : 1024;
  hipLaunchKernelGGL(defer_clear_kernel, dim3(blocks > 0 ? blocks : 1), dim3(256), 0, s, p, n);
  MCG_CHECK_LAUNCH("defer_clear");
  return MCG_OK;
}
int launch_roi_mark(hipStream_t s, const float* boxes, int num_boxes, int boxes_per_frame, int level, int H, int W, int stride, int* state,
                    int* list, int* count) {
  MCG_CHECK_ARG(roi_mark_supported(H, W), "roi_mark: deferred level of %dx%d pixels exceeds %d blocks per axis", H, W, kMarkMaxBlocks);
  hipLaunchKernelGGL(roi_mark_kernel, dim3(num_boxes), dim3(256), 0, s, boxes, boxes_per_frame, level, H, W, 1.0f / (float)stride, state, list,
                     count, 56.f);
  MCG_CHECK_LAUNCH("roi_mark");
  return MCG_OK;
}
extern "C" int mcg_roi_mark_blocks(mcg_stream s, const float* boxes, int num_boxes, int boxes_per_frame, int level, int H, int W, int stride,
                                   int* state, int* list, int* count) {
  MCG_CHECK_ARG(boxes && state && list && count, "mcg_roi_mark_blocks: null pointer");
  MCG_CHECK_ARG(num_boxes > 0 && boxes_per_frame > 0, "mcg_roi_mark_blocks: empty box set");
  MCG_CHECK_ARG(level >= 0 && level <= 3 && H > 0 && W > 0 && stride > 0, "mcg_roi_mark_blocks: bad level (level=%d %dx%d stride=%d)", level, H, W, stride);
  return launch_roi_mark((hipStream_t)s, boxes, num_boxes, boxes_per_frame, level, H, W, stride, state, list, count);
}
extern "C" int mcg_inner_mark_blocks(mcg_stream s, const int* out_list, const int* out_count, int H, int W, int nblk, int* state, int* list,
                                     int* count) {
  MCG_CHECK_ARG(out_list && out_count && state && list && count, "mcg_inner_mark_blocks: null pointer");
  MCG_CHECK_ARG(H > 0 && W > 0 && nblk > 0 && nblk % (((H + 7) / 8) * ((W + 7) / 8)) == 0,
                "mcg_inner_mark_blocks: nblk = frames * blocks per frame (nblk=%d, %dx%d pixels)", nblk, H, W);
  return launch_inner_mark((hipStream_t)s, out_list, out_count, H, W, nblk, state, list, count);
}

int launch_roi_align(hipStream_t s, mcg_dtype dt, const void* const feats[4], const int feat_h[4], const int feat_w[4],
                     const int strides[4], int C, const float* boxes, int num_boxes, int boxes_per_frame, const int32_t* frame_of,
                     int pyramid_frames, void* out, int32_t* levels_out) {
  RoiLevels lv;
  for (int i = 0; i < 4; ++i) {
    lv.feat[i] = feats[i]; lv.h[i] = feat_h[i]; lv.w[i] = feat_w[i];
    lv.scale[i] = 1.0f / (float)strides[i];
  }
  const int epc = mcg_is16(dt) ? 8 : 4;
  MCG_CHECK_ARG(C % epc == 0 && C / epc <= 256 && 256 % (C / epc) == 0, "roi_align: unsupported channel count %d", C);
  dispatch_elem(dt, [&](auto e) {
    hipLaunchKernelGGL(roi_align_kernel<decltype(e)>, dim3(num_boxes), dim3(256), 0, s, lv, C, boxes, boxes_per_frame, frame_of, pyramid_frames, (decltype(e)*)out, levels_out, 56.f);
  });
  MCG_CHECK_LAUNCH("roi_align");
  return MCG_OK;
}

extern "C" int mcg_roi_align(mcg_stream s, mcg_dtype dt, const void* const feats[4], const int feat_h[4], const int feat_w[4],
                             const int strides[4], int C, const float* boxes, int num_boxes, int boxes_per_frame,
                             void* out, int32_t* levels_out) {
  MCG_CHECK_ARG(feats && feat_h && feat_w && strides && boxes && out, "mcg_roi_align: null pointer");
  MCG_CHECK_ARG(num_boxes > 0 && boxes_per_frame > 0, "mcg_roi_align: empty box set");
  for (int i = 0; i < 4; ++i) MCG_CHECK_ARG(feats[i] && feat_h[i] > 0 && feat_w[i] > 0 && strides[i] > 0, "mcg_roi_align: bad level %d", i);
  return launch_roi_align((hipStream_t)s, dt, feats, feat_h, feat_w, strides, C, boxes, num_boxes, boxes_per_frame, nullptr, 0, out, levels_out);
}

extern "C" int mcg_roi_align_indexed(mcg_stream s, mcg_dtype dt, const void* const feats[4], const int feat_h[4], const int feat_w[4],
                                     const int strides[4], int C, const float* boxes, int num_boxes, int boxes_per_frame,
                                     const int32_t* frame_of, int pyramid_frames, void* out, int32_t* levels_out) {
  MCG_CHECK_ARG(feats && feat_h && feat_w && strides && boxes && out && frame_of, "mcg_roi_align_indexed: null pointer");
  MCG_CHECK_ARG(num_boxes > 0 && boxes_per_frame > 0 && pyramid_frames > 0, "mcg_roi_align_indexed: empty box set or pyramid");
  for (int i = 0; i < 4; ++i) MCG_CHECK_ARG(feats[i] && feat_h[i] > 0 && feat_w[i] > 0 && strides[i] > 0, "mcg_roi_align_indexed: bad level %d", i);
  return launch_roi_align((hipStream_t)s, dt, feats, feat_h, feat_w, strides, C, boxes, num_boxes, boxes_per_frame, frame_of, pyramid_frames,
                          out, levels_out);
}
```

### mcgaze_amd/csrc/wino_x3.hpp

```cpp
#pragma once
#include "igemm_dma.hpp"

namespace wnx {
constexpr int KS = 16;
constexpr int UNT = 128;
constexpr int ustage(int g) { return (g + 2) * 4 * 2 * 1024; }
constexpr int wcap(int g, int ct) { return (g == 4 && ct == 4) ? 32 * 1024 : 48 * 1024; }
constexpr int W_LDS = 4 * 64 * 128 * 4;
}

struct WinoParams {
  const float* x;
  const void* u;
  const float* bias;
  float* y;
  int H, W, PW, frames, Cin, Cout, relu;
  int total_pairs, n_tiles;
  int tpf, gpf;
  float wscale;
  const int* blk_list;
  const int* blk_count;
  int bxn, bpf;
};

// ... 281 lines not shown
#pragma unroll
        for (int j2 = 0; j2 < CT; ++j2) acc[i2][j2] = x3_mfma(fh[SL][i2], bl[j2], acc[i2][j2]);
#pragma unroll
      for (int i2 = 0; i2 < RT; ++i2)
#pragma unroll
        for (int j2 = 0; j2 < CT; ++j2) acc[i2][j2] = x3_mfma(fh[SL][i2], bh[j2], acc[i2][j2]);
      static_for<2 * NM1 - 1>([&](auto) {
        __builtin_amdgcn_sched_group_barrier(0x008, 1, 0);
        __builtin_amdgcn_sched_group_barrier(0x002, VPM, 0);
      });
      __builtin_amdgcn_sched_group_barrier(0x008, 1, 0);
      __builtin_amdgcn_sched_group_barrier(0x002, 8, 0);
    });
  }
  asm volatile("s_waitcnt vmcnt(0) lgkmcnt(0)" ::: "memory");
  __syncthreads();

  constexpr int PP = 32 * RT, CPR = NT / 4;
  static_assert(NV * PP * NT * 4 <= 2 * WIN_CAP + 2 * BSTAGE, "epilogue staging");
  float* const C = (float*)smem;
  const float wsc = p.wscale > 0.f ? p.wscale : 1.f;
#pragma unroll 1
  for (int pass = 0; pass < RH; ++pass) {
    if (rh == pass) {
#pragma unroll
      for (int rt = 0; rt < RT; ++rt)
#pragma unroll
        for (int ct = 0; ct < CT; ++ct) stage_acc<PP, NT>(C, nu, rt, ct, lane, acc[rt][ct]);
    }
    __syncthreads();
    for (int item = tid; item < PP * CPR; item += NTHREADS) {
      const int prl = item / CPR, ch4 = (item - prl * CPR) * 4;
      const int q = q0 + pass * PP + prl, R = q / p.PW;
      epilogue_item<G, PP, NT>(p, C, prl, ch4, n0, wsc, R, G * (q - R * p.PW), q < q_end);
    }
    __syncthreads();
  }
}

typedef uint32_t u32x4v __attribute__((ext_vector_type(4)));
template <int IMM>
__device__ __forceinline__ void buf_load16(u32x4v& dst, uint32_t voffset, const u32x4& srd, uint32_t soffset_uniform) {
  asm volatile("buffer_load_dwordx4 %0, %1, %2, %3 offen offset:%4" : "=&v"(dst) : "v"(voffset), "s"(srd), "s"(soffset_uniform), "n"(IMM) : "memory");
}
template <int NB, bool BLK>
__device__ __forceinline__ void wino_x3w_tile(const WinoParams& p, const int logical) {
  using namespace wnx;
  constexpr int G = 2, NW = 4, RT = 4, CT = 4, MT = 128, NT = 128;
  constexpr int ROWB = NB * 1024, WIN_CAP = 48 * 1024, USTAGE = ustage(2);
  constexpr int MAXP = WIN_CAP / 1024 / NW;
  constexpr int HB = MAXP / 2;
  constexpr int BWR = 10;
  static_assert(!BLK || (NB == 1 && RT * BWR <= NW * MAXP), "block tile: one piece per window row, every block's rows in the window");
  extern __shared__ __attribute__((aligned(16))) char smem[];
  char* const s_win = smem;
  const int tid = threadIdx.x, lane = tid & 63;
  const int wave = __builtin_amdgcn_readfirstlane(tid >> 6);
  const int nu = wave;
  const int mt = logical / p.n_tiles, ntile = logical - mt * p.n_tiles;
  int q0 = 0, q_end = 0;
  int bf[RT], by0[RT], bxg[RT];
  uint32_t bokm = 0;
  if constexpr (BLK) {
    const int cnt = __builtin_amdgcn_readfirstlane(*p.blk_count);
#pragma unroll
    for (int rt = 0; rt < RT; ++rt) {
      const int e = RT * mt + rt;
      if (e < cnt) bokm |= 1u << rt;
      const int id = __builtin_amdgcn_readfirstlane(p.blk_list[e < cnt ? e : RT * mt]);
      const int f = id / p.bpf, r = id - f * p.bpf, by = r / p.bxn;
      bf[rt] = f; by0[rt] = 8 * by; bxg[rt] = 4 * (r - by * p.bxn);
    }
  } else {
    tile_range(p, mt, MT, q0, q_end);
  }
  auto pick = [&](const int (&a)[RT], int i) { return i == 0 ? a[0] : (i == 1 ? a[1] : (i == 2 ? a[2] : a[3])); };
  const int q_last = q_end - 1;
  const int sig_b = BLK ? 0 : __builtin_amdgcn_readfirstlane(slot_of(p, q0) - 1);
  const int NP = BLK ? RT * BWR : __builtin_amdgcn_readfirstlane((slot_of(p, q_last) - sig_b + 2) * NB);
  const int NSL = p.Cin / KS, KT = 3 * NSL;
  const int n0 = ntile * NT;
  const u32x4 srd_x = make_srd(p.x);
  const u32x4 srd_u = make_srd((const char*)p.u + (size_t)(n0 / UNT) * KT * USTAGE);
  const uint32_t lds_win = (uint32_t)(uintptr_t)(__attribute__((address_space(3))) char*)s_win;

  uint32_t prow[MAXP];
  int pxo[MAXP];
  uint32_t pokm = 0, prowokm = 0;
  static_for<MAXP>([&](auto nc) {
    constexpr int n = decltype(nc)::value;
    const int pi = wave + NW * n;
    if constexpr (BLK) {
      const int rb = min(pi / BWR, RT - 1), y = pick(by0, rb) + pi - BWR * rb - 1, f = pick(bf, rb);
      const bool rowok = y >= 0 && y < p.H;
      if (pi < NP && ((bokm >> rb) & 1)) pokm |= 1u << n;
      if (rowok) prowokm |= 1u << n;
      prow[n] = __builtin_amdgcn_readfirstlane(row_base(p, f, rowok ? y : 0));
      pxo[n] = __builtin_amdgcn_readfirstlane(2 * pick(bxg, rb));
    } else {
      const WinRow row = win_row(p, sig_b + pi / NB);
      if (pi < NP) pokm |= 1u << n;
      if (row.ok) prowokm |= 1u << n;
      prow[n] = __builtin_amdgcn_readfirstlane(row.base);
      pxo[n] = 0;
    }
  });
  pokm = __builtin_amdgcn_readfirstlane(pokm);
  prowokm = __builtin_amdgcn_readfirstlane(prowokm);
  int l_x, l_c;
  win_lane<G>(lane, wave & (NB - 1), l_x, l_c);
  const uint32_t w_voff = BLK ? (uint32_t)(4 * l_c * 4) : win_voff(p, l_x, l_c);
  auto piece_voff = [&](auto nc) -> uint32_t {
    constexpr int n = decltype(nc)::value;
    if (!(prowokm & (1u << n))) return MCG_OOB_OFFSET;
    if constexpr (BLK) {
      const int x = pxo[n] + l_x;
      return (unsigned)x < (unsigned)p.W ? (uint32_t)(x * p.Cin * 4) + w_voff : MCG_OOB_OFFSET;
    } else {
      return w_voff;
    }
  };
  auto issue_window = [&](auto hc, int cs, uint32_t dst) {
    constexpr int h0 = decltype(hc)::value * HB;
    static_for<HB>([&](auto nc) {
      constexpr int n = h0 + decltype(nc)::value;
      if (pokm & (1u << n)) {
        const uint32_t v = piece_voff(std::integral_constant<int, n>{});
        lds_dma16<0>(v, srd_x, prow[n] + (uint32_t)cs * (KS * 4), dst + (uint32_t)(wave + NW * n) * 1024u);
      }
    });
  };
  const uint32_t b_voff = (uint32_t)lane * 16u + (uint32_t)nu * 8192u;
  u32x4v bh[2][CT], bl[2][CT];
  auto issue_b1 = [&](auto slc, auto jc, uint32_t koff) {
    constexpr int SLX = decltype(slc)::value, J = decltype(jc)::value;
    if constexpr (J & 1) buf_load16<(J & 3) * 1024>(bl[SLX][J >> 1], b_voff, srd_u, koff + (J >> 2) * 4096u);
    else buf_load16<(J & 3) * 1024>(bh[SLX][J >> 1], b_voff, srd_u, koff + (J >> 2) * 4096u);
  };

  int toff[2];
  float tsg;
  f23_position(nu, toff, tsg);
  const int pl = lane & 31, h = lane >> 5;
  const char* ap[RT][2][2];
#pragma unroll
  for (int rt = 0; rt < RT; ++rt) {
    int jrow, xg;
    if constexpr (BLK) {
      jrow = BWR * rt + (pl >> 2);
      xg = pl & 3;
    } else {
      const int q = min(q0 + rt * 32 + pl, q_last);
      xg = q - q / p.PW * p.PW;
      jrow = slot_of(p, q) - sig_b - 1;
    }
#pragma unroll
    for (int t = 0; t < 2; ++t)
#pragma unroll
      for (int ch = 0; ch < 2; ++ch) ap[rt][t][ch] = a_addr<G>(s_win, jrow, ROWB, xg, toff[t], 2 * h + ch);
  }

  f32x16 acc[RT][CT];
#pragma unroll
  for (int i = 0; i < RT; ++i)
#pragma unroll
    for (int j = 0; j < CT; ++j)
#pragma unroll
      for (int r = 0; r < 16; ++r) acc[i][j][r] = 0.f;

  struct Raw { uint4 d[RT][2][2]; };
  auto load_raw = [&](auto wbc, auto kyc, Raw& r) {
    constexpr int AOFF = decltype(wbc)::value * WIN_CAP + decltype(kyc)::value * ROWB;
#pragma unroll
    for (int rt = 0; rt < RT; ++rt)
#pragma unroll
      for (int t = 0; t < 2; ++t) { r.d[rt][t][0] = *(const uint4*)(ap[rt][t][0] + AOFF); r.d[rt][t][1] = *(const uint4*)(ap[rt][t][1] + AOFF); }
  };

  issue_window(std::integral_constant<int, 0>{}, 0, lds_win);
  issue_window(std::integral_constant<int, 1>{}, 0, lds_win);
  static_for<8>([&](auto jc) { issue_b1(std::integral_constant<int, 0>{}, jc, 0u); });
  if (NSL > 1) issue_window(std::integral_constant<int, 0>{}, 1, lds_win + WIN_CAP);
  bf16x8 fh[2][RT], fl[2][RT];
  asm volatile("s_waitcnt vmcnt(0)" ::: "memory");
  __builtin_amdgcn_s_barrier();
  {
    Raw r0;
    load_raw(std::integral_constant<int, 0>{}, std::integral_constant<int, 0>{}, r0);
#pragma unroll
    for (int rt = 0; rt < RT; ++rt) f23_fragment(r0.d[rt], tsg, fh[0][rt], fl[0][rt]);
  }
  constexpr int NM1 = RT * CT;
  uint32_t nh[RT][4], nl[RT][4];
#pragma nounroll
  for (int s2 = 0; s2 < NSL / 2; ++s2) {
    static_for<6>([&](auto uc) {
      constexpr int U = decltype(uc)::value, KY = U % 3, SL = U & 1, WB = U / 3;
      constexpr int U1 = (U + 1) % 6, KY1 = U1 % 3, WB1 = U1 / 3;
      const int k = 6 * s2 + U, cs = 2 * s2 + WB;
      asm volatile("s_waitcnt vmcnt(0)"
                   : "+v"(bh[SL][0]), "+v"(bh[SL][1]), "+v"(bh[SL][2]), "+v"(bh[SL][3]), "+v"(bl[SL][0]), "+v"(bl[SL][1]), "+v"(bl[SL][2]), "+v"(bl[SL][3])
                   :
                   : "memory");
      if constexpr (KY == 2) __builtin_amdgcn_s_barrier();
      Raw raw;
      load_raw(std::integral_constant<int, WB1>{}, std::integral_constant<int, KY1>{}, raw);
      __builtin_amdgcn_sched_barrier(0);
      const uint32_t kn = (uint32_t)min(k + 1, KT - 1) * USTAGE;
      auto vmem_slot = [&](auto vc) {
        constexpr int V = decltype(vc)::value;
        if constexpr (V < 8) {
          issue_b1(std::integral_constant<int, SL ^ 1>{}, std::integral_constant<int, V>{}, kn);
        } else if constexpr (KY != 1 && V < 8 + HB) {
          constexpr int n = (KY == 0 ? HB : 0) + (V - 8);
          const int csn = KY == 0 ? cs + 1 : cs + 2;
          if (csn < NSL && (pokm & (1u << n))) {
            const uint32_t v = piece_voff(std::integral_constant<int, n>{});
            lds_dma16<0>(v, srd_x, prow[n] + (uint32_t)csn * (KS * 4), lds_win + (KY == 0 ? (WB ^ 1) : WB) * WIN_CAP + (uint32_t)(wave + NW * n) * 1024u);
          }
        }
      };
      static_for<NM1>([&](auto mc) {
        constexpr int M = decltype(mc)::value, I = M / CT, J = M % CT;
        acc[I][J] = x3_mfma(fl[SL][I], __builtin_bit_cast(bf16x8, bh[SL][J]), acc[I][J]);
        if constexpr (M % 3 == 0) {
          __builtin_amdgcn_sched_barrier(0);
          vmem_slot(std::integral_constant<int, M / 3>{});
          __builtin_amdgcn_sched_barrier(0);
        }
      });
      __builtin_amdgcn_sched_barrier(0);
      static_for<8>([&](auto qc) {
        constexpr int Q = decltype(qc)::value, I = Q & 3, TERM3 = Q >> 2;
        constexpr int XR = Q >> 1, XC = Q & 1;
        {
          float v[4];
          f23_chunk(raw.d[XR][0][XC], raw.d[XR][1][XC], tsg, v);
          split_pair(v[0], v[1], nh[XR][2 * XC], nl[XR][2 * XC]);
          split_pair(v[2], v[3], nh[XR][2 * XC + 1], nl[XR][2 * XC + 1]);
        }
#pragma unroll
        for (int j2 = 0; j2 < CT; ++j2)
          acc[I][j2] = x3_mfma(fh[SL][I], __builtin_bit_cast(bf16x8, TERM3 ? bh[SL][j2] : bl[SL][j2]), acc[I][j2]);
        asm volatile("" : "+v"(nh[XR][2 * XC]), "+v"(nh[XR][2 * XC + 1]), "+v"(nl[XR][2 * XC]), "+v"(nl[XR][2 * XC + 1]));
        static_for<4>([&](auto) {
          __builtin_amdgcn_sched_group_barrier(0x008, 1, 0);
          __builtin_amdgcn_sched_group_barrier(0x002, 4, 0);
        });
        __builtin_amdgcn_sched_barrier(0);
        vmem_slot(std::integral_constant<int, 6 + Q>{});
        __builtin_amdgcn_sched_barrier(0);
      });
#pragma unroll
      for (int rt = 0; rt < RT; ++rt) {
        fh[SL ^ 1][rt] = __builtin_bit_cast(bf16x8, make_uint4(nh[rt][0], nh[rt][1], nh[rt][2], nh[rt][3]));
        fl[SL ^ 1][rt] = __builtin_bit_cast(bf16x8, make_uint4(nl[rt][0], nl[rt][1], nl[rt][2], nl[rt][3]));
      }
    });
  }
  asm volatile("s_waitcnt vmcnt(0) lgkmcnt(0)"
               : "+v"(bh[0][0]), "+v"(bh[0][1]), "+v"(bh[0][2]), "+v"(bh[0][3]), "+v"(bl[0][0]), "+v"(bl[0][1]), "+v"(bl[0][2]), "+v"(bl[0][3]),
                 "+v"(bh[1][0]), "+v"(bh[1][1]), "+v"(bh[1][2]), "+v"(bh[1][3]), "+v"(bl[1][0]), "+v"(bl[1][1]), "+v"(bl[1][2]), "+v"(bl[1][3])
               :
               : "memory");
  __syncthreads();

  constexpr int PP = 64, CPR = NT / 4;
  float* const C = (float*)smem;
  const float wsc = p.wscale > 0.f ? p.wscale : 1.f;
#pragma unroll
  for (int pass = 0; pass < 2; ++pass) {
#pragma unroll
    for (int rt = 0; rt < 2; ++rt)
#pragma unroll
      for (int ct = 0; ct < CT; ++ct) stage_acc<PP, NT>(C, nu, rt, ct, lane, acc[2 * pass + rt][ct]);
    __syncthreads();
    for (int item = tid; item < PP * CPR; item += 256) {
      const int prl = item / CPR, ch4 = (item - prl * CPR) * 4;
      if constexpr (BLK) {
        const int rt = 2 * pass + (prl >> 5), pl = prl & 31;
        const int y = pick(by0, rt) + (pl >> 2), xo = G * (pick(bxg, rt) + (pl & 3));
        epilogue_item<G, PP, NT>(p, C, prl, ch4, n0, wsc, pick(bf, rt) * p.H + y, xo, ((bokm >> rt) & 1) && y < p.H && xo < p.W);
      } else {
        const int q = q0 + pass * PP + prl, R = q / p.PW;
        epilogue_item<G, PP, NT>(p, C, prl, ch4, n0, wsc, R, G * (q - R * p.PW), q < q_end);
      }
    }
    __syncthreads();
  }
}
template <int NB>
__global__ __launch_bounds__(256, 1) void wino_x3w_kernel(const WinoParams p) {
  wino_x3w_tile<NB, false>(p, xcd_remap(blockIdx.x, gridDim.x));
}
__global__ __launch_bounds__(256, 1) void wino_x3w_blocks_kernel(const WinoParams p) {
  const int units = __builtin_amdgcn_readfirstlane(((*p.blk_count + 3) >> 2) * p.n_tiles);
  const int padded = p.n_tiles == 2 ? (units + 15) & ~15 : units;
  for (int u = blockIdx.x; u < padded; u += gridDim.x) {
    int logical = u;
    if (p.n_tiles == 2) { const int x = u & 7, j = u >> 3; logical = (j & 1) + 2 * (x + 8 * (j >> 1)); }
    if (logical < units) wino_x3w_tile<1, true>(p, logical);
  }
}

static inline int wino_x3_tile_groups(int g, int shape) { return g == 2 ? ((shape == 0 || shape == 3) ? 128 : (shape == 1 ? 64 : 32)) : (shape == 0 ? 64 : 32); }
static inline int wino_x3_tile_channels(int shape) { return (shape == 0 || shape == 3) ? 128 : 64; }
static inline int wino_x3_pieces(int W, int g) { return (g * ((W + g - 1) / g) + 2 + 8 * g - 1) / (8 * g) * (g / 2); }
static inline int wino_x3_max_rows(int H, int W, int mt, int g, bool cross) {
  const int PW = (W + g - 1) / g;
  int rows = (PW - 1 + mt - 1) / PW + 1;
  if (!cross && rows > H) rows = H;
  const int nz = cross ? (rows >= 2 ? (rows - 2) / H + 1 : 0) : 0;
  return rows + nz + 2;
}
static inline int wino_x3_nb_template(int pieces) { return pieces <= 1 ? 1 : (pieces <= 2 ? 2 : 4); }
static inline bool wino_x3_operands_ok(int frames, int H, int W, int Cin, int Cout) {
  const long long px = (long long)frames * H * W;
  return Cin % 32 == 0 && Cout % wnx::UNT == 0 && H >= 1 && W >= 2 && frames >= 1 && px * Cin * 4 < MCG_DMA_MAX_BYTES &&
         px * Cout * 4 < MCG_DMA_MAX_BYTES && px < 0x7fffffffLL;
}
static inline int wino_x3_mode(int frames, int H, int W, int Cin, int Cout, int g) {
  if (!wino_x3_operands_ok(frames, H, W, Cin, Cout) || (g != 2 && g != 4)) return 0;
  if (g == 4 && (W % 4 != 0 || W < 16)) return 0;
  const int pcs = wino_x3_pieces(W, g);
  if (pcs > 4) return 0;
  const int nb = wino_x3_nb_template(pcs);
  const int mt = wino_x3_tile_groups(g, 0), cap = wnx::wcap(g, 4);
  if (wino_x3_max_rows(H, W, mt, g, true) * nb * 1024 <= cap) return 1;
  if (wino_x3_max_rows(H, W, mt, g, false) * nb * 1024 <= cap) return 2;
  return 0;
}
static inline bool wino_x3_applicable(int frames, int H, int W, int Cin, int Cout, int g = 2) { return wino_x3_mode(frames, H, W, Cin, Cout, g) != 0; }
static inline size_t wino_x3_weight_bytes(int Cin, int Cout, int g = 2) { return (size_t)(Cout / wnx::UNT) * (3 * Cin / wnx::KS) * wnx::ustage(g); }

template <int NB, int RH, int RT, int CT, int G>
static inline int launch_wino_x3_t(hipStream_t s, const WinoParams& p, int grid) {
  constexpr int kLds = 2 * wnx::wcap(G, CT) + 2 * ((G + 2) * CT * 2 * 1024);
  if (kernel_ready<wino_x3_kernel<NB, RH, RT, CT, G>>(kLds)) return 1;
  hipLaunchKernelGGL((wino_x3_kernel<NB, RH, RT, CT, G>), dim3(grid), dim3(64 * (G + 2) * RH), kLds, s, p);
  return hipGetLastError() == hipSuccess ? 0 : 1;
}
template <int NB>
static inline int launch_wino_x3w(hipStream_t s, const WinoParams& p, int grid) {
  if (kernel_ready<wino_x3w_kernel<NB>>(wnx::W_LDS)) return 1;
  hipLaunchKernelGGL((wino_x3w_kernel<NB>), dim3(grid), dim3(256), wnx::W_LDS, s, p);
  return hipGetLastError() == hipSuccess ? 0 : 1;
}
template <int NB>
static inline int launch_wino_x3_nb(hipStream_t s, const WinoParams& p, int g, int shape, int grid) {
  if (g == 2 && shape == 3) return launch_wino_x3w<NB>(s, p, grid);
  if (g == 4) return shape == 0 ? launch_wino_x3_t<NB, 2, 1, 4, 4>(s, p, grid) : launch_wino_x3_t<NB, 1, 1, 2, 4>(s, p, grid);
  if (shape == 0) return launch_wino_x3_t<NB, 2, 2, 4, 2>(s, p, grid);
  if (shape == 1) return launch_wino_x3_t<NB, 2, 1, 2, 2>(s, p, grid);
  return launch_wino_x3_t<NB, 1, 1, 2, 2>(s, p, grid);
}
static inline bool wino_x3_blocks_applicable(int frames, int H, int W, int Cin, int Cout) { return wino_x3_operands_ok(frames, H, W, Cin, Cout); }
static inline int wino_x3_blocks_per_frame(int H, int W) { return ((H + 7) / 8) * ((W + 7) / 8); }
static inline int launch_wino_x3_blocks(hipStream_t s, WinoParams p, const int* list, const int* count, int max_blocks, int cap = 0) {
  int cus;
  if (kernel_ready<wino_x3w_blocks_kernel>(wnx::W_LDS, &cus)) return 1;
  p.PW = (p.W + 1) / 2;
  p.n_tiles = p.Cout / 128;
  p.bxn = (p.W + 7) / 8;
  p.bpf = wino_x3_blocks_per_frame(p.H, p.W);
  p.blk_list = list; p.blk_count = count;
  const int units = (max_blocks + 3) / 4 * p.n_tiles;
  int grid = units < cus ? units : cus / 16 * 16;
  if (cap > 0 && grid > cap) grid = cap;
  hipLaunchKernelGGL(wino_x3w_blocks_kernel, dim3(grid > 0 ? grid : 1), dim3(256), wnx::W_LDS, s, p);
  return hipGetLastError() == hipSuccess ? 0 : 1;
}
static const int kWinoMinGrid = 130;
static inline int launch_wino_x3(hipStream_t s, WinoParams p, int shape = -1, int g = 2) {
  const int mode = wino_x3_mode(p.frames, p.H, p.W, p.Cin, p.Cout, g);
  if (mode == 0) return 1;
  p.PW = (p.W + g - 1) / g;
  p.gpf = p.H * p.PW;
  p.total_pairs = p.frames * p.gpf;
  auto mtiles = [&](int sh) {
    const int mt = wino_x3_tile_groups(g, sh);
    return mode == 2 ? p.frames * ((p.gpf + mt - 1) / mt) : (p.total_pairs + mt - 1) / mt;
  };
  auto grid_of = [&](int sh) { return mtiles(sh) * (p.Cout / wino_x3_tile_channels(sh)); };
  if (shape < 0) shape = grid_of(0) >= kWinoMinGrid ? (g == 2 ? 3 : 0) : ((g == 2 && grid_of(1) >= kWinoMinGrid) ? 1 : 2);
  if (g == 4 && (shape == 1 || shape == 3)) shape = 2;
  p.n_tiles = p.Cout / wino_x3_tile_channels(shape);
  p.tpf = mode == 2 ? (p.gpf + wino_x3_tile_groups(g, shape) - 1) / wino_x3_tile_groups(g, shape) : 0;
  const int grid = grid_of(shape);
  const int nb = wino_x3_nb_template(wino_x3_pieces(p.W, g));
  if (nb == 1) return launch_wino_x3_nb<1>(s, p, g, shape, grid);
  if (nb == 2) return launch_wino_x3_nb<2>(s, p, g, shape, grid);
  return launch_wino_x3_nb<4>(s, p, g, shape, grid);
}
```

### mcgaze_amd/engine.py

```python
import ctypes as C
import os

import numpy as np
import torch

from . import lib as L
from .packing import PackedWeights

_TORCH_DT = {'bf16': torch.bfloat16, 'f16': torch.float16, 'fp16': torch.float16, 'fp32': torch.float32, 'f32': torch.float32, 'f16x3': torch.float32, 'bf16x3': torch.float32}
_CODE = {'bf16': L.MCG_BF16, 'f16': L.MCG_F16, 'fp16': L.MCG_F16, 'fp32': L.MCG_F32, 'f32': L.MCG_F32, 'f16x3': L.MCG_F16X3,
         'bf16x3': L.MCG_F16X3}


def _code(dtype):
    return L.MCG_BF16 if dtype == torch.bfloat16 else (L.MCG_F16 if dtype == torch.float16 else L.MCG_F32)


def _ptr(t):
    return C.c_void_p(t.data_ptr()) if t is not None else C.c_void_p(0)


def _stream(device=None):
    return C.c_void_p(torch.cuda.current_stream(device).cuda_stream)


def _require_gpu():
    if not torch.cuda.is_available():
        raise L.McgError('mcgaze_amd needs a HIP device (MI355X / gfx950); there is no CPU fallback path')


def _ws(nbytes, device):
    return torch.empty(max(int(nbytes), 256), dtype=torch.uint8, device=device)


def to_nhwc(x_nchw, dtype):
    _require_gpu()
    lib = L.load()
    N, Cc, H, W = x_nchw.shape
    x = x_nchw.contiguous().float()
    out = torch.empty(N, H, W, Cc, dtype=dtype, device=x.device)
    L.check(lib.mcg_nchw_to_nhwc(_stream(), _code(dtype), _ptr(x), _ptr(out), N, Cc, H, W), 'mcg_nchw_to_nhwc')
    return out


def to_nchw(x_nhwc):
    _require_gpu()
    lib = L.load()
    N, H, W, Cc = x_nhwc.shape
    out = torch.empty(N, Cc, H, W, dtype=torch.float32, device=x_nhwc.device)
    L.check(lib.mcg_nhwc_to_nchw(_stream(), _code(x_nhwc.dtype), _ptr(x_nhwc.contiguous()), _ptr(out), N, Cc, H, W), 'mcg_nhwc_to_nchw')
    return out


def conv2d(x, w, bias=None, stride=1, pad=0, relu=False, residual=None, residual_mode=L.RES_NONE, x2=None, stride2=1, split=False,
           tile=0, flags=0, prescale=True):
    _require_gpu()
    lib = L.load()
    N, H, W, Cin = x.shape
    Cout, KH, KW, _ = w.shape
    wscale = 0.0
    if split:
        from .packing import pow2_prescale, split_pack
        assert x.dtype == torch.float32 and w.dtype == torch.float32
        ws, wscale = pow2_prescale(w.reshape(Cout, -1).cpu()) if prescale else (w.reshape(Cout, -1).cpu(), 0.0)
        w = split_pack(ws).to(x.device)
    Cin2 = x2.shape[3] if x2 is not None else 0
    Ho, Wo = (H + 2 * pad - KH) // stride + 1, (W + 2 * pad - KW) // stride + 1
    y = torch.empty(N, Ho, Wo, Cout, dtype=x.dtype, device=x.device)
    d = L.ConvDesc(x.data_ptr(), w.data_ptr(), bias.data_ptr() if bias is not None else None,
                   residual.data_ptr() if residual is not None else None, y.data_ptr(),
                   N, H, W, Cin, Cout, KH, KW, stride, pad, int(relu), residual_mode if residual is not None else L.RES_NONE,
                   residual.shape[1] if residual is not None else 0, residual.shape[2] if residual is not None else 0,
                   x2.data_ptr() if x2 is not None else None, Cin2, stride2, x2.shape[1] if x2 is not None else 0,
                   x2.shape[2] if x2 is not None else 0, tile, flags, wscale)
    L.check(lib.mcg_conv2d(_stream(), L.MCG_F16X3 if split else _code(x.dtype), C.byref(d)), 'mcg_conv2d')
    return y


def pointwise_weights(w, dtype, split=False, device='cuda'):
    from .packing import frag_major, frag_major_split, pow2_prescale
    if split:
        ws, wscale = pow2_prescale(w.cpu())
        return frag_major_split(ws).to(device), wscale
    return frag_major(w.cpu().to(dtype)).contiguous().to(device), 0.0


def _rows_out(out, M, N, dtype, device):
    if out is None:
        return torch.empty(M, N, dtype=dtype, device=device)
    assert out.is_contiguous() and out.dtype == dtype and out.shape[0] >= M and tuple(out.shape[1:]) == (N,), (tuple(out.shape), M, N)
    return out


def pointwise_stream(a, wf, bias, N, relu=False, residual=None, residual_mode=L.RES_NONE, out_hw=None, split=False, wscale=0.0,
                     many_slices=False, blocks=None, grid_cap=0, out=None):
    _require_gpu()
    lib = L.load()
    M, K = a.shape
    code = L.MCG_F16X3 if split else _code(a.dtype)
    y = _rows_out(out, M, N, a.dtype, a.device)
    a = a.contiguous()
    if many_slices:
        assert residual is None and blocks is None and N == 32768 and K == 256
        L.check(lib.mcg_pointwise_dyn(_stream(), code, _ptr(a), _ptr(wf), _ptr(bias), _ptr(y), M, wscale, grid_cap), 'mcg_pointwise_dyn')
        return y
    mode = residual_mode if residual is not None else L.RES_NONE
    Ho, Wo = out_hw if out_hw is not None else (1, M)
    Hr, Wr = (residual.shape[1], residual.shape[2]) if mode == L.RES_UPSAMPLE_ADD else (Ho, Wo)
    blist = bcount = None
    if blocks is not None:
        blist, bcount = _block_list(blocks, a.device)
    L.check(lib.mcg_pointwise_stream(_stream(), code, _ptr(a), _ptr(wf), _ptr(bias), _ptr(residual.contiguous() if residual is not None else None),
                                     _ptr(y), M, K, N, int(relu), mode, Ho, Wo, Hr, Wr, wscale, _ptr(blist), _ptr(bcount), grid_cap),
            'mcg_pointwise_stream')
    return y


def pointwise_pair(a1, w3f, b3, w1f, b1, C2, a2=None, residual=None, grid_cap=0, out=None):
    _require_gpu()
    lib = L.load()
    M = a1.shape[0]
    y = _rows_out(out[0] if out else None, M, 256, a1.dtype, a1.device)
    z = _rows_out(out[1] if out else None, M, C2, a1.dtype, a1.device)
    cont = lambda t: t.contiguous() if t is not None else None
    L.check(lib.mcg_pointwise_pair(_stream(), _code(a1.dtype), _ptr(a1.contiguous()), _ptr(cont(a2)), _ptr(cont(residual)), _ptr(w3f), _ptr(b3),
                                   _ptr(y), _ptr(w1f), _ptr(b1), _ptr(z), M, a2.shape[1] if a2 is not None else 0, C2, grid_cap), 'mcg_pointwise_pair')
    return y, z


def conv3x3_wino(x, w, bias=None, relu=False, tile=0, g=2):
    _require_gpu()
    lib = L.load()
    N, H, W, Cin = x.shape
    Cout = w.shape[0]
    u, wscale = wino_weights(w, g, x.device)
    assert u.numel() * 2 == lib.mcg_conv3x3_wino_x3_weight_bytes(Cin, Cout, g), (u.numel(), Cin, Cout)
    y = torch.empty(N, H, W, Cout, dtype=torch.float32, device=x.device)
    L.check(lib.mcg_conv3x3_wino_x3(_stream(), _ptr(x.contiguous()), _ptr(u), _ptr(bias), _ptr(y), N, H, W, Cin, Cout, int(relu), tile, wscale, g), 'mcg_conv3x3_wino_x3')
    return y


def _block_list(blocks, device):
    if isinstance(blocks, tuple) and len(blocks) == 2 and all(isinstance(t, torch.Tensor) for t in blocks):
        blist, bcount = blocks
        for t in (blist, bcount):
            assert t.dtype == torch.int32 and t.is_contiguous() and t.device == torch.device(device), (t.dtype, t.device)
        assert blist.dim() == 1 and blist.numel() >= 1 and bcount.numel() == 1
        return blist, bcount
    ids = _flat_ints(blocks, 'blocks must be a flat sequence', 'blocks must be integers', False)
    blist = torch.zeros(max(len(ids), 1), dtype=torch.int32, device=device)
    blist[:len(ids)] = torch.from_numpy(ids.astype(np.int32)).to(device)
    return blist, torch.tensor([len(ids)], dtype=torch.int32, device=device)


def wino_weights(w, g=2, device='cuda'):
    from .packing import pow2_prescale, wino_pack
    ws, wscale = pow2_prescale(w.cpu())
    return wino_pack(ws, g=g).to(device), wscale


def conv3x3_wino_blocks(x, packed, blocks, out, bias=None, relu=False, grid_cap=0):
    _require_gpu()
    lib = L.load()
    N, H, W, Cin = x.shape
    u, wscale = packed
    Cout = out.shape[-1]
    assert x.dtype == torch.float32 and x.is_contiguous() and out.dtype == torch.float32 and out.is_contiguous() and tuple(out.shape) == (N, H, W, Cout)
    assert u.numel() * 2 == lib.mcg_conv3x3_wino_x3_weight_bytes(Cin, Cout, 2), (u.numel(), Cin, Cout)
    blist, bcount = _block_list(blocks, x.device)
    L.check(lib.mcg_conv3x3_wino_x3_blocks(_stream(), _ptr(x), _ptr(u), _ptr(bias), _ptr(out), N, H, W, Cin, Cout, int(relu), wscale,
                                           _ptr(blist), _ptr(bcount), blist.numel(), grid_cap), 'mcg_conv3x3_wino_x3_blocks')
    return out


def bottleneck_x3(x, src2, wstream, bias, cn, nsrc, trace=None):
    _require_gpu()
    lib = L.load()
    N, H, W, cm = x.shape
    y = torch.empty(N, H, W, 4 * cm, dtype=torch.float32, device=x.device)
    z = torch.empty(N, H, W, cn, dtype=torch.float32, device=x.device) if cn else None
    L.check(lib.mcg_bottleneck_x3(_stream(), _ptr(x.contiguous()), _ptr(src2.contiguous()), _ptr(wstream), _ptr(bias), _ptr(y), _ptr(z),
                                  N, H, W, cm, nsrc, cn, _ptr(trace)), 'mcg_bottleneck_x3')
    return y, z


def stem(img, w_stem, bias, dtype, flags=0, split=False):
    _require_gpu()
    lib = L.load()
    N, _, H, W = img.shape
    code = L.MCG_F16X3 if split else _code(dtype)
    ws = _ws(lib.mcg_stem_workspace_bytes(code, N, H, W), img.device)
    y = torch.empty(N, H // 4, W // 4, 64, dtype=dtype, device=img.device)
    L.check(lib.mcg_stem_forward(_stream(), code, _ptr(img.contiguous()), _ptr(w_stem), _ptr(bias), _ptr(y), N, H, W,
                                 _ptr(ws), ws.numel(), flags), 'mcg_stem_forward')
    return y


def roi_align(feats, boxes, strides=(4, 8, 16, 32)):
    return roi_align_indexed(feats, boxes, None, strides)


def _mark_buffers(nblk, state, blist, count, device):
    z = lambda n: torch.zeros(n, dtype=torch.int32, device=device)
    state, blist, count = (z(nblk) if state is None else state), (z(nblk) if blist is None else blist), (z(1) if count is None else count)
    for t in (state, blist, count):
        assert t.dtype == torch.int32 and t.is_contiguous() and t.device == torch.device(device), (t.dtype, t.device)
    assert state.numel() == nblk and blist.numel() >= nblk and count.numel() == 1, (state.numel(), blist.numel(), nblk)
    return state, blist, count


def roi_mark_blocks(boxes, hw, level=0, stride=4, state=None, blist=None, count=None):
    _require_gpu()
    lib = L.load()
    N, P = boxes.shape[:2]
    H, W = hw
    b = boxes.contiguous().float()
    state, blist, count = _mark_buffers(N * ((H + 7) // 8) * ((W + 7) // 8), state, blist, count, b.device)
    L.check(lib.mcg_roi_mark_blocks(_stream(), _ptr(b), N * P, P, level, H, W, stride, _ptr(state), _ptr(blist), _ptr(count)), 'mcg_roi_mark_blocks')
    return state, blist, count


def inner_mark_blocks(out_list, out_count, hw, frames, state=None, blist=None, count=None):
    _require_gpu()
    lib = L.load()
    H, W = hw
    nblk = frames * ((H + 7) // 8) * ((W + 7) // 8)
    state, blist, count = _mark_buffers(nblk, state, blist, count, out_list.device)
    _mark_buffers(nblk, state, out_list, out_count, out_list.device)
    L.check(lib.mcg_inner_mark_blocks(_stream(), _ptr(out_list), _ptr(out_count), H, W, nblk, _ptr(state), _ptr(blist), _ptr(count)), 'mcg_inner_mark_blocks')
    return state, blist, count


def roi_align_indexed(feats, boxes, frame_of, strides=(4, 8, 16, 32)):
    _require_gpu()
    lib = L.load()
    N, P = boxes.shape[:2]
    K, Cc = feats[0].shape[0], feats[0].shape[-1]
    name, gather = 'mcg_roi_align', ()
    if frame_of is not None:
        table = torch.from_numpy(check_frame_table(frame_of, K, 1)).to(boxes.device)
        if table.numel() != N:
            raise L.McgError(f'frame_of holds {table.numel()} entries for {N} frames of boxes')
        name, gather = 'mcg_roi_align_indexed', (_ptr(table), K)
    out = torch.empty(N * P, 49, Cc, dtype=feats[0].dtype, device=boxes.device)
    lv = torch.empty(N * P, dtype=torch.int32, device=boxes.device)
    fp = (C.c_void_p * 4)(*[f.data_ptr() for f in feats])
    fh = (C.c_int * 4)(*[f.shape[1] for f in feats])
    fw = (C.c_int * 4)(*[f.shape[2] for f in feats])
    st = (C.c_int * 4)(*strides)
    b = boxes.contiguous().float()
    L.check(getattr(lib, name)(_stream(), _code(feats[0].dtype), fp, fh, fw, st, Cc, _ptr(b), N * P, P, *gather, _ptr(out), _ptr(lv)), name)
    return out, lv


def _flat_ints(seq, must, must_int, nonempty):
    t = seq.numpy() if isinstance(seq, torch.Tensor) else seq
    try:
        a = np.asarray(t)
    except Exception as ex:
        raise L.McgError(f'{must} ({ex})')
    if a.ndim != 1 or (nonempty and a.size == 0) or (a.size and not np.issubdtype(a.dtype, np.integer)):
        raise L.McgError(f'{must_int} (got {a.dtype} of shape {a.shape})')
    return a


def check_frame_table(frame_of, pyramid_frames, clip_length):
    a = _flat_ints(frame_of, 'frame_of must be a flat sequence of row indices', 'frame_of must be a flat sequence of integer row indices', False)
    if clip_length < 1 or a.size == 0 or a.size % clip_length:
        raise L.McgError(f'frame_of holds {a.size} entries, not a positive multiple of clip_length={clip_length}')
    if pyramid_frames < 1 or int(a.min()) < 0 or int(a.max()) >= pyramid_frames:
        raise L.McgError(f'frame_of entries must lie in [0, {pyramid_frames}) (got {int(a.min())} .. {int(a.max())})')
    return a.astype(np.int32)


def check_row_table(rows, store_rows, num_frames):
    a = _flat_ints(rows, 'rows must be a flat sequence of row indices', 'rows must be a flat sequence of integer row indices', False)
    if a.size != int(num_frames):
        raise L.McgError(f'rows holds {a.size} entries for {int(num_frames)} frames')
    if a.size and (store_rows < 1 or int(a.min()) < 0 or int(a.max()) >= store_rows):
        raise L.McgError(f'rows entries must lie in [0, {store_rows}) (got {int(a.min())} .. {int(a.max())})')
    if a.size > 1 and len(set(a.tolist())) != a.size:
        u, n = np.unique(a, return_counts=True)
        raise L.McgError(f'rows names row {int(u[n.argmax()])} for {int(n.max())} frames: every frame needs a row of its own')
    return a.astype(np.int32)


def check_clip_lengths(lengths, num_frames):
    a = _flat_ints(lengths, 'clip lengths must be a flat sequence of integers', 'clip lengths must be a non-empty flat sequence of integers', True)
    if int(a.min()) < 1:
        raise L.McgError(f'every clip must hold at least one frame (got a length of {int(a.min())})')
    total = int(a.astype(np.int64).sum())
    if num_frames is not None and total != int(num_frames):
        raise L.McgError(f'clip lengths sum to {total} frames, the batch holds {int(num_frames)}')
    start = np.zeros(a.size + 1, dtype=np.int32)
    np.cumsum(a, out=start[1:])
    return start


class ClipTable:

    def __init__(self, lengths, device='cuda:0'):
        self.start = check_clip_lengths(lengths, None)
        self.num_frames, self.num_clips, self.max_len = int(self.start[-1]), self.start.size - 1, int(np.diff(self.start).max())
        self.device = torch.device(device)
        self.table = torch.from_numpy(self.start).to(self.device)


def _upload_table(table, device):
    t = torch.as_tensor(table)
    return t.pin_memory().to(device, non_blocking=True) if torch.device(device).type == 'cuda' else t.to(device)


def _outputs(N, device, alloc=torch.empty):
    return dict(gaze=alloc(4, N, 3, dtype=torch.float32, device=device), boxes=alloc(N, 3, 4, dtype=torch.float32, device=device),
                scores=alloc(N, 3, dtype=torch.float32, device=device))


class _Clips:

    def __init__(self, clip_length, num_frames, device):
        self.ragged = not isinstance(clip_length, (int, np.integer))
        if not self.ragged:
            self.args = (clip_length,)
        elif isinstance(clip_length, ClipTable):
            ct = clip_length
            if ct.num_frames != num_frames or ct.device != torch.device(device):
                raise L.McgError(f'the ClipTable holds {ct.num_frames} frames on {ct.device}, the batch {num_frames} on {device}')
            self.table, self.args = ct.table, (_ptr(ct.table), ct.num_clips, ct.max_len)
        else:
            start = check_clip_lengths(clip_length, num_frames)
            self.table = _upload_table(start, device)
            self.args = (_ptr(self.table), start.size - 1, int(np.diff(start).max()))

    def pick(self, fixed, ragged):
        return ragged if self.ragged else fixed


def _table(d, keys):
    return (C.c_void_p * len(keys))(*[d[k].data_ptr() for k in keys])


def stage_forward(stage_w, roi_feat, obj, boxes, clip_length, stds=(0.5, 0.5, 1.0, 1.0), split=False, flags=0):
    _require_gpu()
    lib = L.load()
    N = obj.shape[0]
    dt = L.MCG_F16X3 if split else _code(obj.dtype)
    ws = _ws(lib.mcg_stage_workspace_bytes(dt, N), obj.device)
    obj_out = torch.empty_like(obj)
    boxes_out = torch.empty(N, 3, 4, dtype=torch.float32, device=obj.device)
    cls = torch.empty(N, 3, dtype=torch.float32, device=obj.device)
    sd = (C.c_float * 4)(*stds)
    clips = _Clips(clip_length, N, obj.device)
    name = clips.pick('mcg_stage_forward', 'mcg_stage_forward_ragged')
    L.check(getattr(lib, name)(_stream(), dt, _table(stage_w, L.STAGE_KEYS), _ptr(roi_feat.contiguous()), _ptr(obj.contiguous()),
                               _ptr(boxes.contiguous().float()), N, *clips.args, _ptr(obj_out), _ptr(boxes_out), _ptr(cls), sd, _ptr(ws), ws.numel(),
                               flags), name)
    return obj_out, boxes_out, cls


def gaze_head(gaze_w, obj, split=False):
    _require_gpu()
    lib = L.load()
    N = obj.shape[0]
    dt = L.MCG_F16X3 if split else _code(obj.dtype)
    ws = _ws(lib.mcg_gaze_head_workspace_bytes(dt, N), obj.device)
    out = torch.empty(4, N, 3, dtype=torch.float32, device=obj.device)
    L.check(lib.mcg_gaze_head(_stream(), dt, _table(gaze_w, L.GAZE_KEYS), _ptr(obj.contiguous()), N, _ptr(out), _ptr(ws), ws.numel()), 'mcg_gaze_head')
    return out


class HipEngine:

    def __init__(self, state_dict, depth=50, num_stages=4, precision='f16x3', device='cuda:0', bbox_stds=(0.5, 0.5, 1.0, 1.0), fuse_downsample=True):
        _require_gpu()
        self.lib = L.load()
        self.device = torch.device(device)
        self.dtype = _TORCH_DT[precision]
        self.code = _CODE[precision]
        self.precision = precision
        self.weights = PackedWeights(state_dict, depth=depth, num_stages=num_stages, dtype=self.dtype, device=self.device,
                                     fuse_downsample=fuse_downsample, split=self.code == L.MCG_F16X3)
        w = self.weights
        mk = lambda c: L.ConvWeights(c['w'].data_ptr(), c['bias'].data_ptr(), c['cin'], c['cout'], c['k'], c['stride'], c['pad'],
                                     c['wf'].data_ptr() if c.get('wf') is not None else None, float(c.get('wscale', 0.0)),
                                     c['wf4'].data_ptr() if c.get('wf4') is not None else None)
        self._convs = (L.ConvWeights * len(w.convs))(*[mk(c) for c in w.convs])
        self._stage_tab = (C.c_void_p * (num_stages * L.SW_COUNT))(*[st[k].data_ptr() for st in w.stages for k in L.STAGE_KEYS])
        self._gaze_tab = _table(w.gaze, L.GAZE_KEYS)
        mw = L.ModelWeights()
        mw.blocks = (C.c_int * 4)(*w.blocks)
        mw.stem = mk(w.stem)
        mw.convs = C.cast(self._convs, C.POINTER(L.ConvWeights))
        mw.num_convs = len(w.convs)
        mw.lateral = (L.ConvWeights * 4)(*[mk(c) for c in w.lateral])
        mw.fpn_out = (L.ConvWeights * 4)(*[mk(c) for c in w.fpn_out])
        if len(w.c3_ds) == 4:
            mw.c3_ds = (L.ConvWeights * 4)(*[mk(c) for c in w.c3_ds])
        mw.init_boxes = w.init_boxes.data_ptr()
        mw.init_feats = w.init_feats.data_ptr()
        mw.num_stages = num_stages
        mw.stage_weights = C.cast(self._stage_tab, C.POINTER(C.c_void_p))
        mw.gaze_weights = C.cast(self._gaze_tab, C.POINTER(C.c_void_p))
        mw.bbox_stds = (C.c_float * 4)(*bbox_stds)
        if w.fused:
            self._fused = (L.FusedBlock * len(w.fused))(*[L.FusedBlock(f['wstream'].data_ptr(), f['bias'].data_ptr(), f['conv2_index'], f['cm'], f['c'],
                                                                      f['cn'], f['nsrc']) for f in w.fused])
            mw.fused, mw.num_fused = C.cast(self._fused, C.POINTER(L.FusedBlock)), len(w.fused)
        self._handle = C.c_void_p()
        with torch.cuda.device(self.device):
            L.check(self.lib.mcg_engine_create(C.byref(self._handle), C.byref(mw), self.code), 'mcg_engine_create')
        self._ws = None
        self._dec_ws = None
        self._row_ws = None

    def set_option(self, name, value):
        L.check(self.lib.mcg_engine_set_option(self._handle, name.encode(), int(value)), f'mcg_engine_set_option({name})')

    def range_audit(self, capacity=256):
        counts = (C.c_ulonglong * (2 * capacity))()
        names = (C.c_char_p * capacity)()
        n = C.c_int()
        L.check(self.lib.mcg_engine_range_audit(self._handle, counts, names, capacity, C.byref(n)), 'mcg_engine_range_audit')
        return [(names[i].decode(), int(counts[2 * i]), int(counts[2 * i + 1])) for i in range(n.value)]

    def profile_start(self, capacity=4096):
        L.check(self.lib.mcg_engine_profile_start(self._handle, capacity), 'mcg_engine_profile_start')

    def profile_stop(self, capacity=4096):
        cnt = C.c_int()
        ms = (C.c_float * capacity)(); fl = (C.c_double * capacity)(); by = (C.c_double * capacity)()
        cf = (C.c_int * capacity)(); sh = (C.c_int * (3 * capacity))()
        L.check(self.lib.mcg_engine_profile_stop(self._handle, C.byref(cnt), ms, fl, by, cf, sh, capacity), 'mcg_engine_profile_stop')
        return [(ms[i], fl[i], cf[i], (sh[3 * i], sh[3 * i + 1], sh[3 * i + 2]), by[i]) for i in range(cnt.value)]

    def backbone_only(self, img, return_levels=False):
        self._check_img(img)
        N, _, H, W = img.shape
        with torch.cuda.device(self.device):
            ws = self._workspace(N, H, W, 0)
            L.check(self.lib.mcg_bench_backbone_forward(self._handle, _stream(self.device), _ptr(img), N, H, W, _ptr(ws), ws.numel()), 'mcg_bench_backbone_forward')
            if not return_levels:
                return None
            tab = (C.c_void_p * 4)()
            L.check(self.lib.mcg_bench_backbone_levels(self._handle, _ptr(ws), N, H, W, tab), 'mcg_bench_backbone_levels')
            es = ws.element_size() * (2 if self.dtype in (torch.bfloat16, torch.float16) else 4)
            out = []
            for i in range(4):
                shape = (N, (H // 4) >> i, (W // 4) >> i, 256 << i)
                n = shape[0] * shape[1] * shape[2] * shape[3]
                off = tab[i] - ws.data_ptr()
                out.append(ws[off:off + n * es].view(self.dtype).view(shape))
            return out

    def __del__(self):
        h = getattr(self, '_handle', None)
        if h is not None and h.value:
            self.lib.mcg_engine_destroy(h)
            self._handle = None

    def _grown(self, name, need):
        if getattr(self, name) is None or getattr(self, name).numel() < need:
            setattr(self, name, None)
            setattr(self, name, _ws(need, self.device))
        return getattr(self, name)

    def _workspace(self, N, H, W, chunk):
        return self._grown('_ws', self.lib.mcg_engine_workspace_bytes(self._handle, N, H, W, chunk))

    def _check_img(self, img):
        if not (img.is_cuda and img.device == self.device and img.dtype == torch.float32 and img.is_contiguous() and img.dim() == 4):
            raise L.McgError(f'img must be a contiguous float32 [N,3,H,W] tensor on {self.device} (got {img.dtype} {tuple(img.shape)} on {img.device})')

    def backbone_fpn(self, img, chunk_frames=0, out=None, row=0):
        self._check_img(img)
        N, _, H, W = img.shape
# ... 207 lines not shown
```

### mcgaze_amd/lib.py

```python
import ctypes as C
import os

_HERE = os.path.dirname(os.path.abspath(__file__))
LIB_PATH = os.environ.get('MCGAZE_LIB') or os.path.join(_HERE, 'libmcgaze_hip.so')

MCG_OK = 0
MCG_F32, MCG_BF16, MCG_F16X3, MCG_F16 = 0, 1, 2, 3
ABI_VERSION = 20
RES_NONE, RES_ADD, RES_UPSAMPLE_ADD = 0, 1, 2
FLAG_STAGED_GEMM, FLAG_NO_SPECIALISED, FLAG_NO_ATTN_BLOCK = 1, 2, 4

STAGE_KEYS = [
    'IN_PROJ_W', 'IN_PROJ_B', 'OUT_PROJ_W', 'OUT_PROJ_B', 'ATTN_LN_G', 'ATTN_LN_B', 'DYN_W', 'DYN_B',
    'NORM_IN_G', 'NORM_IN_B', 'NORM_OUT_G', 'NORM_OUT_B', 'FC_W', 'FC_B', 'FC_LN_G', 'FC_LN_B', 'IIC_LN_G', 'IIC_LN_B',
    'FFN1_W', 'FFN1_B', 'FFN2_W', 'FFN2_B', 'FFN_LN_G', 'FFN_LN_B', 'CLS_FC_W', 'CLS_LN_G', 'CLS_LN_B',
    'REG_FC_W', 'REG_LN_G', 'REG_LN_B', 'HEAD_CLS_W', 'HEAD_CLS_B', 'HEAD_REG_W', 'HEAD_REG_B', 'OUT_PROJ_WF', 'CLS_FC_WF', 'REG_FC_WF', 'IN_PROJ_WF', 'DYN_WF']
GAZE_KEYS = ['FC_W', 'LN_G', 'LN_B', 'OUT_W', 'OUT_B', 'FUSE_W', 'FUSE_B']
SW_COUNT, GW_COUNT = len(STAGE_KEYS), len(GAZE_KEYS)

EXPORTS = ['mcg_abi_version', 'mcg_build_id', 'mcg_last_error', 'mcg_device_info', 'mcg_nchw_to_nhwc', 'mcg_nhwc_to_nchw', 'mcg_conv2d',
           'mcg_stem_workspace_bytes', 'mcg_stem_forward', 'mcg_roi_align', 'mcg_stage_workspace_bytes', 'mcg_stage_forward',
           'mcg_gaze_head_workspace_bytes', 'mcg_gaze_head', 'mcg_engine_create', 'mcg_engine_destroy',
           'mcg_engine_workspace_bytes', 'mcg_trunk_workspace_bytes', 'mcg_decoder_workspace_bytes', 'mcg_backbone_fpn_forward',
           'mcg_decoder_forward', 'mcg_clip_forward', 'mcg_preprocess_frames', 'mcg_engine_set_option', 'mcg_engine_profile_start',
           'mcg_engine_profile_stop', 'mcg_bench_backbone_forward', 'mcg_bottleneck_x3', 'mcg_bench_backbone_levels', 'mcg_conv3x3_wino_x3',
           'mcg_conv3x3_wino_x3_weight_bytes', 'mcg_engine_range_audit', 'mcg_roi_align_indexed', 'mcg_decoder_forward_indexed',
           'mcg_deferred_pyramid_bytes', 'mcg_deferred_pyramid_levels', 'mcg_backbone_fpn_forward_deferred', 'mcg_decoder_forward_deferred',
           'mcg_stage_forward_ragged', 'mcg_decoder_forward_ragged', 'mcg_decoder_forward_deferred_ragged', 'mcg_clip_forward_ragged',
           'mcg_pyramid_scatter_rows', 'mcg_preprocess_head_crops', 'mcg_merge_windows', 'mcg_smooth_gaze', 'mcg_preprocess_frames_nv12',
           'mcg_preprocess_head_crops_nv12', 'mcg_draw_gaze_arrows', 'mcg_draw_gaze_arrows_nv12',
           'mcg_detect_heads_workspace_bytes', 'mcg_detect_heads', 'mcg_letterbox_frames', 'mcg_letterbox_frames_nv12',
           'mcg_track_state_bytes', 'mcg_track_heads', 'mcg_track_heads_motion', 'mcg_live_slots', 'mcg_live_gate', 'mcg_live_lanes', 'mcg_live_gate_lanes',
           'mcg_deferred_pyramid_state', 'mcg_inner_block_neighbours', 'mcg_gaze_targets', 'mcg_gaze_dwell', 'mcg_gaze_targets_poly',
           'mcg_pointwise_stream', 'mcg_pointwise_dyn', 'mcg_pointwise_pair', 'mcg_draw_attention', 'mcg_draw_attention_nv12',
           'mcg_format_labels', 'mcg_draw_labels', 'mcg_draw_labels_nv12', 'mcg_gaze_heat_add', 'mcg_draw_heat', 'mcg_draw_heat_nv12',
           'mcg_anonymize_heads', 'mcg_anonymize_heads_nv12', 'mcg_roi_mark_blocks', 'mcg_inner_mark_blocks', 'mcg_conv3x3_wino_x3_blocks']
LABEL_CHARS = 24
LETTERBOX_U8, LETTERBOX_F16, LETTERBOX_F32 = 0, 1, 2


class ConvDesc(C.Structure):
    _fields_ = [('x', C.c_void_p), ('w', C.c_void_p), ('bias', C.c_void_p), ('residual', C.c_void_p), ('y', C.c_void_p),
                ('N', C.c_int), ('H', C.c_int), ('W', C.c_int), ('Cin', C.c_int), ('Cout', C.c_int), ('KH', C.c_int),
                ('KW', C.c_int), ('stride', C.c_int), ('pad', C.c_int), ('relu', C.c_int), ('residual_mode', C.c_int),
                ('Hr', C.c_int), ('Wr', C.c_int), ('x2', C.c_void_p), ('Cin2', C.c_int), ('stride2', C.c_int), ('H2', C.c_int),
                ('W2', C.c_int), ('tile', C.c_int), ('flags', C.c_int), ('wscale', C.c_float)]


class ConvWeights(C.Structure):
    _fields_ = [('w', C.c_void_p), ('bias', C.c_void_p), ('cin', C.c_int), ('cout', C.c_int), ('k', C.c_int),
                ('stride', C.c_int), ('pad', C.c_int), ('wf', C.c_void_p), ('wscale', C.c_float), ('wf4', C.c_void_p)]


class FusedBlock(C.Structure):
    _fields_ = [('wstream', C.c_void_p), ('bias', C.c_void_p), ('conv2_index', C.c_int), ('cm', C.c_int), ('c', C.c_int), ('cn', C.c_int),
                ('nsrc', C.c_int)]


class ModelWeights(C.Structure):
    _fields_ = [('blocks', C.c_int * 4), ('stem', ConvWeights), ('convs', C.POINTER(ConvWeights)), ('num_convs', C.c_int),
                ('lateral', ConvWeights * 4), ('fpn_out', ConvWeights * 4), ('c3_ds', ConvWeights * 4), ('init_boxes', C.c_void_p),
                ('init_feats', C.c_void_p), ('num_stages', C.c_int), ('stage_weights', C.POINTER(C.c_void_p)),
                ('gaze_weights', C.POINTER(C.c_void_p)), ('bbox_stds', C.c_float * 4), ('fused', C.POINTER(FusedBlock)), ('num_fused', C.c_int)]


class FrameDesc(C.Structure):
    _fields_ = [('src', C.c_void_p), ('src_h', C.c_int), ('src_w', C.c_int), ('src_pitch', C.c_int), ('crop_y', C.c_int),
                ('crop_x', C.c_int), ('crop_h', C.c_int), ('crop_w', C.c_int), ('out_h', C.c_int), ('out_w', C.c_int)]


class ImageDesc(C.Structure):
    _fields_ = [('src', C.c_void_p), ('h', C.c_int), ('w', C.c_int), ('pitch', C.c_int)]


class YuvCoef(C.Structure):
    _fields_ = [(n, C.c_int) for n in ('y_off', 'cy', 'cub', 'cug', 'cvg', 'cvr')]


class Nv12ImageDesc(C.Structure):
    _fields_ = [('y', C.c_void_p), ('uv', C.c_void_p), ('h', C.c_int), ('w', C.c_int), ('pitch_y', C.c_int), ('pitch_uv', C.c_int)]


class Nv12FrameDesc(C.Structure):
    _fields_ = FrameDesc._fields_ + [('uv', C.c_void_p), ('uv_pitch', C.c_int)]


class LetterboxDesc(C.Structure):
    _fields_ = [('frame', FrameDesc), ('top', C.c_int), ('left', C.c_int)]


class Nv12LetterboxDesc(C.Structure):
    _fields_ = [('frame', Nv12FrameDesc), ('top', C.c_int), ('left', C.c_int)]


class ArrowDesc(C.Structure):
    _fields_ = [('seg', C.c_int * 2 * 2 * 3), ('thickness', C.c_int), ('x0', C.c_int), ('y0', C.c_int), ('x1', C.c_int), ('y1', C.c_int),
                ('image', C.c_int), ('flag', C.c_int), ('reserved', C.c_int)]


class StrokeDesc(C.Structure):
    _fields_ = [('seg', C.c_int * 2 * 2 * 3), ('thickness', C.c_int), ('x0', C.c_int), ('y0', C.c_int), ('x1', C.c_int), ('y1', C.c_int),
                ('image', C.c_int), ('flag', C.c_int), ('layer', C.c_int), ('count', C.c_int), ('color', C.c_uint), ('color_active', C.c_uint),
                ('reserved', C.c_int)]


class LabelDesc(C.Structure):
    _fields_ = [(n, C.c_int) for n in ('x', 'y', 'x0', 'y0', 'x1', 'y1', 'image', 'flag', 'len')] + [('color', C.c_uint), ('text', C.c_ubyte * LABEL_CHARS)]


class AnonDesc(C.Structure):
    _fields_ = [(n, C.c_int) for n in ('image', 'flag', 'x0', 'y0', 'x1', 'y1', 'cx2', 'cy2', 'W', 'H', 'shift', 'shape')]


class McgError(RuntimeError):
    pass


_lib = None


def load():
    global _lib
    if _lib is not None:
        return _lib
    if not os.path.exists(LIB_PATH):
        raise McgError(f'{LIB_PATH} not found: build it with `python -c "import __graft_entry__ as g; g.build()"` '
                       f'(or `make -C mcgaze_amd/csrc`); mcgaze_amd has no CPU fallback')
    lib = C.CDLL(LIB_PATH)
    vp, i, sz = C.c_void_p, C.c_int, C.c_size_t
    lib.mcg_abi_version.restype = i
    lib.mcg_last_error.restype = C.c_char_p
    lib.mcg_build_id.restype = C.c_char_p
    lib.mcg_device_info.argtypes = [C.POINTER(i), C.POINTER(sz), C.c_char_p, i]
    lib.mcg_nchw_to_nhwc.argtypes = [vp, i, vp, vp, i, i, i, i]
    lib.mcg_nhwc_to_nchw.argtypes = [vp, i, vp, vp, i, i, i, i]
    lib.mcg_conv2d.argtypes = [vp, i, C.POINTER(ConvDesc)]
    lib.mcg_stem_workspace_bytes.restype = sz
    lib.mcg_stem_workspace_bytes.argtypes = [i, i, i, i]
    lib.mcg_stem_forward.argtypes = [vp, i, vp, vp, vp, vp, i, i, i, vp, sz, i]
    lib.mcg_roi_align.argtypes = [vp, i, C.POINTER(vp), C.POINTER(i), C.POINTER(i), C.POINTER(i), i, vp, i, i, vp, vp]
    lib.mcg_roi_align_indexed.argtypes = [vp, i, C.POINTER(vp), C.POINTER(i), C.POINTER(i), C.POINTER(i), i, vp, i, i, vp, i, vp, vp]
    lib.mcg_stage_workspace_bytes.restype = sz
    lib.mcg_stage_workspace_bytes.argtypes = [i, i]
    lib.mcg_stage_forward.argtypes = [vp, i, C.POINTER(vp), vp, vp, vp, i, i, vp, vp, vp, C.POINTER(C.c_float), vp, sz, i]
    lib.mcg_gaze_head_workspace_bytes.restype = sz
    lib.mcg_gaze_head_workspace_bytes.argtypes = [i, i]
    lib.mcg_gaze_head.argtypes = [vp, i, C.POINTER(vp), vp, i, vp, vp, sz]
    lib.mcg_engine_create.argtypes = [C.POINTER(vp), C.POINTER(ModelWeights), i]
    lib.mcg_engine_destroy.argtypes = [vp]
    lib.mcg_engine_destroy.restype = None
    lib.mcg_engine_workspace_bytes.restype = sz
    lib.mcg_engine_workspace_bytes.argtypes = [vp, i, i, i, i]
    lib.mcg_trunk_workspace_bytes.restype = sz
    lib.mcg_trunk_workspace_bytes.argtypes = [vp, i, i, i, i]
    lib.mcg_decoder_workspace_bytes.restype = sz
    lib.mcg_decoder_workspace_bytes.argtypes = [vp, i]
    lib.mcg_decoder_forward.argtypes = [vp, vp, C.POINTER(vp), i, i, i, i, vp, vp, vp, vp, vp, sz]
    lib.mcg_decoder_forward_indexed.argtypes = [vp, vp, C.POINTER(vp), i, vp, i, i, i, i, vp, vp, vp, vp, vp, sz]
    lib.mcg_backbone_fpn_forward.argtypes = [vp, vp, vp, i, i, i, i, C.POINTER(vp), vp, sz]
    lib.mcg_deferred_pyramid_bytes.restype = sz
    lib.mcg_deferred_pyramid_bytes.argtypes = [vp, i, i, i]
    lib.mcg_deferred_pyramid_levels.argtypes = [vp, vp, i, i, i, C.POINTER(vp), C.POINTER(i)]
    lib.mcg_deferred_pyramid_state.argtypes = [vp, vp, i, i, i, C.POINTER(vp), C.POINTER(vp), C.POINTER(vp), C.POINTER(vp), C.POINTER(i), C.POINTER(i)]
    lib.mcg_inner_block_neighbours.argtypes = [i, i, i, C.POINTER(i)]
    lib.mcg_backbone_fpn_forward_deferred.argtypes = [vp, vp, vp, i, i, i, i, vp, sz, vp, sz]
    lib.mcg_decoder_forward_deferred.argtypes = [vp, vp, vp, sz, i, i, i, i, vp, vp, vp, vp, vp, sz]
    lib.mcg_clip_forward.argtypes = [vp, vp, vp, i, i, i, i, vp, i, vp, vp, vp, vp, sz]
    lib.mcg_stage_forward_ragged.argtypes = [vp, i, C.POINTER(vp), vp, vp, vp, i, vp, i, i, vp, vp, vp, C.POINTER(C.c_float), vp, sz, i]
    lib.mcg_decoder_forward_ragged.argtypes = [vp, vp, C.POINTER(vp), i, vp, i, vp, i, i, i, i, vp, vp, vp, vp, vp, sz]
    lib.mcg_decoder_forward_deferred_ragged.argtypes = [vp, vp, vp, sz, i, vp, i, i, i, i, vp, vp, vp, vp, vp, sz]
    lib.mcg_clip_forward_ragged.argtypes = [vp, vp, vp, i, vp, i, i, i, i, vp, i, vp, vp, vp, vp, sz]
    lib.mcg_pyramid_scatter_rows.argtypes = [vp, i, C.POINTER(vp), C.POINTER(vp), i, i, i, i, vp]
    lib.mcg_merge_windows.argtypes = [vp, vp, vp, vp, i, vp, i, vp, i, i, vp, i, C.c_float]
    lib.mcg_smooth_gaze.argtypes = [vp, vp, i, vp, i, C.c_double, vp]
    lib.mcg_preprocess_frames.argtypes =[vp, vp, i, vp, i, i, C.POINTER(C.c_float), C.POINTER(C.c_float), i]
    lib.mcg_preprocess_head_crops.argtypes = [vp, vp, i, vp, vp, i, C.c_double, i, i, vp, vp, vp, vp, vp, i, i, C.POINTER(C.c_float), C.POINTER(C.c_float), i]
    lib.mcg_preprocess_frames_nv12.argtypes = lib.mcg_preprocess_frames.argtypes + [C.POINTER(YuvCoef)]
    lib.mcg_preprocess_head_crops_nv12.argtypes = lib.mcg_preprocess_head_crops.argtypes + [C.POINTER(YuvCoef)]
    u8p = C.POINTER(C.c_ubyte)
    lib.mcg_draw_gaze_arrows.argtypes = [vp, vp, i, i, i, vp, vp, i, vp, i, C.c_double, i, C.c_double, C.c_double, u8p, vp, vp, vp]
    lib.mcg_draw_gaze_arrows_nv12.argtypes = lib.mcg_draw_gaze_arrows.argtypes
    lib.mcg_detect_heads_workspace_bytes.restype = sz
    lib.mcg_detect_heads_workspace_bytes.argtypes = [i, i]
    lib.mcg_detect_heads.argtypes = [vp, vp, i, i, i, C.c_longlong, i, i, i, vp, C.c_double, C.c_double, i, i, i, i, vp, vp, vp, vp, vp, vp, vp, sz]
    lib.mcg_letterbox_frames.argtypes = [vp, vp, i, vp, i, i, i, i]
    lib.mcg_letterbox_frames_nv12.argtypes = lib.mcg_letterbox_frames.argtypes + [C.POINTER(YuvCoef)]
    lib.mcg_track_state_bytes.restype = sz
    lib.mcg_track_state_bytes.argtypes = [i, i]
    lib.mcg_track_heads.argtypes = [vp, vp, C.c_longlong, vp, i, i, i, i, C.c_double, i, vp, vp, vp, vp, vp, vp, vp]
    lib.mcg_track_heads_motion.argtypes = [vp, vp, C.c_longlong, vp, i, i, i, i, C.c_double, i, C.c_double, C.c_double, vp, vp, vp, vp, vp, vp, vp, vp]
    lib.mcg_live_slots.argtypes = [vp, vp, i, i, i, i, vp, vp, vp, vp, vp]
    lib.mcg_live_gate.argtypes = [vp, vp, vp, i, i, i, i, vp, i, i, i, vp, vp, vp, vp, vp, vp, vp, vp, vp]
    lib.mcg_live_lanes.argtypes = [vp, vp, i, i, i, i, i, vp, vp, vp, vp, vp, vp, vp, vp, vp]
    lib.mcg_live_gate_lanes.argtypes = [vp, vp, vp, vp, i, i, i, i, i, vp, i, i, i, vp, vp, vp, vp, vp, vp, vp, vp, vp, vp, vp]
    lib.mcg_gaze_targets.argtypes = [vp, vp, vp, i, vp, i, vp, vp, i, i, C.c_double, C.c_double, vp, vp, vp, vp, vp, vp]
    lib.mcg_gaze_targets_poly.argtypes = [vp, vp, vp, i, vp, i, vp, i, vp, vp, i, i, C.c_double, C.c_double, vp, vp, vp, vp, vp, vp]
    lib.mcg_draw_attention.argtypes = [vp, vp, i, i, i, vp, vp, i, vp, i, vp, vp, vp, vp, vp, i, vp, vp, i, i, u8p, C.c_double, i, C.c_double, C.c_double,
                                       i, i, vp, sz, vp, vp, vp]
    lib.mcg_draw_attention_nv12.argtypes = lib.mcg_draw_attention.argtypes
    lib.mcg_format_labels.argtypes = [vp, vp, vp, i, i, i, vp]
    lib.mcg_draw_labels.argtypes = [vp, vp, i, i, i, vp, vp, vp, vp, i, vp, i, i, i, u8p, vp, u8p, vp, vp]
    lib.mcg_draw_labels_nv12.argtypes = lib.mcg_draw_labels.argtypes
    lib.mcg_gaze_heat_add.argtypes = [vp, vp, vp, vp, vp, vp, i, vp, vp, i, i, i, i, i, i, i, i, vp, sz]
    lib.mcg_draw_heat.argtypes = [vp, vp, i, i, i, vp, vp, i, i, i, i, i, vp, i]
    lib.mcg_draw_heat_nv12.argtypes = lib.mcg_draw_heat.argtypes
    lib.mcg_anonymize_heads.argtypes = [vp, vp, i, i, i, vp, vp, i, C.c_double, i, i, i, i, u8p, vp, vp]
    lib.mcg_anonymize_heads_nv12.argtypes = lib.mcg_anonymize_heads.argtypes
    lib.mcg_gaze_dwell.argtypes =[vp, vp, vp, vp, vp, vp, i, i, i, i, i, vp, vp, i, vp, vp, vp, i, vp]
    lib.mcg_engine_set_option.argtypes = [vp, C.c_char_p, i]
    lib.mcg_engine_profile_start.argtypes = [vp, i]
    lib.mcg_engine_profile_stop.argtypes = [vp, C.POINTER(i), C.POINTER(C.c_float), C.POINTER(C.c_double), C.POINTER(C.c_double), C.POINTER(i), C.POINTER(i), i]
    lib.mcg_bench_backbone_forward.argtypes = [vp, vp, vp, i, i, i, vp, sz]
    lib.mcg_bench_backbone_levels.argtypes = [vp, vp, i, i, i, C.POINTER(vp)]
    lib.mcg_bottleneck_x3.argtypes = [vp, vp, vp, vp, vp, vp, vp, i, i, i, i, i, i, vp]
    lib.mcg_conv3x3_wino_x3.argtypes = [vp, vp, vp, vp, vp, i, i, i, i, i, i, i, C.c_float, i]
    lib.mcg_conv3x3_wino_x3_blocks.argtypes = [vp, vp, vp, vp, vp, i, i, i, i, i, i, C.c_float, vp, vp, i, i]
    lib.mcg_roi_mark_blocks.argtypes = [vp, vp, i, i, i, i, i, i, vp, vp, vp]
    lib.mcg_inner_mark_blocks.argtypes = [vp, vp, vp, i, i, i, vp, vp, vp]
    lib.mcg_conv3x3_wino_x3_weight_bytes.restype = sz
    lib.mcg_pointwise_stream.argtypes = [vp, i, vp, vp, vp, vp, vp, i, i, i, i, i, i, i, i, i, C.c_float, vp, vp, i]
    lib.mcg_pointwise_dyn.argtypes = [vp, i, vp, vp, vp, vp, i, C.c_float, i]
    lib.mcg_pointwise_pair.argtypes = [vp, i, vp, vp, vp, vp, vp, vp, vp, vp, vp, i, i, i, i]
    lib.mcg_engine_range_audit.argtypes = [vp, C.POINTER(C.c_ulonglong), C.POINTER(C.c_char_p), i, C.POINTER(i)]
    lib.mcg_conv3x3_wino_x3_weight_bytes.argtypes = [i, i, i]
    for name in EXPORTS:
        fn = getattr(lib, name)
        if fn.restype is C.c_int and name not in ('mcg_abi_version',):
            fn.restype = i
    if lib.mcg_abi_version() != ABI_VERSION:
        raise McgError(f'ABI mismatch: library reports {lib.mcg_abi_version()}, binding expects {ABI_VERSION}')
    _lib = lib
    return lib


def build_id():
    return load().mcg_build_id().decode()


def source_id():
    import hashlib
    src = os.path.join(_HERE, 'csrc')
    names = sorted(n for n in os.listdir(src) if n.endswith('.hip') or n.endswith('.hpp'))
    h = hashlib.sha256()
    for n in names:
        h.update(open(os.path.join(src, n), 'rb').read())
    h.update(open(os.path.join(_HERE, '..', 'include', 'mcgaze_hip.h'), 'rb').read())
    return h.hexdigest()[:16]


def check(rc, what):
    if rc != MCG_OK:
        msg = load().mcg_last_error().decode(errors='replace')
        raise McgError(f'{what} failed (code {rc}): {msg}')
```

Before: 3629 clips/s.

## Defer FPN output convs on coarse levels to frames hit by ROI boxes

Extends deferred FPN computation to levels P3-P5. The trunk keeps their lateral inputs and skips the output convs. Each decoder stage's ROI mark kernel now also records which frames have boxes mapped to each level. A new frame-list Winograd kernel then computes the output conv only for those frames. This avoids computing pyramid outputs that ROI align never reads, at the cost of extra slot memory, atomics in the mark kernel and per-stage kernel launches. By default only P5 (mask 8) is deferred.

```diff
diff --git a/include/mcgaze_hip.h b/include/mcgaze_hip.h
--- a/include/mcgaze_hip.h
+++ b/include/mcgaze_hip.h
@@ -56,6 +56,8 @@
 int mcg_conv3x3_wino_x3_blocks(mcg_stream s, const float* x, const void* u, const float* bias, float* y, int frames, int H, int W,
                                int Cin, int Cout, int relu, float wscale, const int* block_list, const int* block_count, int max_blocks,
                                int grid_cap);
+int mcg_conv3x3_wino_x3_frames(mcg_stream s, const float* x, const void* u, const float* bias, float* y, int frames, int H, int W,
+                               int Cin, int Cout, const int* frame_list, const int* frame_count, int grid_cap);
 
 int mcg_pointwise_stream(mcg_stream s, mcg_dtype dt, const void* a, const void* wf, const float* bias, const void* res, void* y,
                          int M, int K, int N, int relu, int res_mode, int Ho, int Wo, int Hr, int Wr, float wscale,
@@ -76,6 +78,7 @@
                           const int32_t* frame_of, int pyramid_frames, void* out, int32_t* levels_out);
 int mcg_roi_mark_blocks(mcg_stream s, const float* boxes, int num_boxes, int boxes_per_frame, int level, int H, int W, int stride,
                         int* state, int* list, int* count);
+int mcg_roi_mark_frames(mcg_stream s, const float* boxes, int num_boxes, int boxes_per_frame, int level, int* state, int* list, int* count);
 
 enum {
   MCG_SW_IN_PROJ_W = 0, MCG_SW_IN_PROJ_B, MCG_SW_OUT_PROJ_W, MCG_SW_OUT_PROJ_B, MCG_SW_ATTN_LN_G, MCG_SW_ATTN_LN_B,
@@ -180,6 +183,8 @@
 int mcg_deferred_pyramid_levels(const mcg_engine* e, void* slot, int num_frames, int H, int W, void* levels[4], int* deferred);
 int mcg_deferred_pyramid_state(const mcg_engine* e, void* slot, int num_frames, int H, int W, void** inner, int** flags, int** counts,
                                int** lists, int* blocks, int* lateral_deferred);
+int mcg_deferred_pyramid_frame_state(const mcg_engine* e, void* slot, int num_frames, int H, int W, int level, int** flags, int** counts,
+                                     int** lists, int* frame_deferred);
 int mcg_inner_block_neighbours(int id, int H, int W, int out[9]);
 int mcg_inner_mark_blocks(mcg_stream s, const int* out_list, const int* out_count, int H, int W, int nblk, int* state, int* list, int* count);
 int mcg_backbone_fpn_forward_deferred(mcg_engine* e, mcg_stream s, const float* img, int num_frames, int H, int W, int chunk_frames,
diff --git a/mcgaze_amd/csrc/check_resources.py b/mcgaze_amd/csrc/check_resources.py
--- a/mcgaze_amd/csrc/check_resources.py
+++ b/mcgaze_amd/csrc/check_resources.py
@@ -5,6 +5,7 @@
 RULES = {
     'wino_x3w_kernel': dict(scratch=0, vgpr_spill=0, unit='engine'),
     'wino_x3w_blocks_kernel': dict(scratch=0, vgpr_spill=0, unit='engine'),
+    'wino_x3w_frames_kernel': dict(scratch=0, vgpr_spill=0, unit='engine'),
     'gaze_targets_kernel': dict(scratch=0, vgpr_spill=0, unit='attend'),
     'gaze_targets_poly_kernel': dict(scratch=0, vgpr_spill=0, unit='attend'),
     'gaze_mutual_kernel': dict(scratch=0, vgpr_spill=0, unit='attend'),
diff --git a/mcgaze_amd/csrc/engine.hip b/mcgaze_amd/csrc/engine.hip
--- a/mcgaze_amd/csrc/engine.hip
+++ b/mcgaze_amd/csrc/engine.hip
@@ -22,7 +22,7 @@
 bool roi_mark_supported(int H, int W);
 int launch_defer_clear(hipStream_t s, int* p, int n);
 int launch_roi_mark(hipStream_t s, const float* boxes, int num_boxes, int boxes_per_frame, int level, int H, int W, int stride, int* state,
-                    int* list, int* count);
+                    int* list, int* count, int* const* frame_state, int* const* frame_list, int* const* frame_count);
 int launch_inner_mark(hipStream_t s, const int* out_list, const int* out_count, int H, int W, int nblk, int* state, int* list, int* count);
 
 struct mcg_engine {
@@ -38,6 +38,8 @@
   int wino_tile = -1;
   int fpn_deferred = 1;
   int fpn_lateral_deferred = 1;
+  int fpn_levels_deferred = 1;
+  static constexpr int kDeferLevelsDefault = 8;
   static constexpr int kAuditCap = 256;
   unsigned long long* audit_dev = nullptr;
   std::vector<std::string> audit_names;
@@ -187,6 +189,10 @@
   else if (!strcmp(name, "winograd")) { MCG_CHECK_ARG(value >= 0 && value <= 2, "winograd must be 0, 1 or 2"); e->winograd = value; }
   else if (!strcmp(name, "fpn_deferred")) e->fpn_deferred = value != 0;
   else if (!strcmp(name, "fpn_lateral_deferred")) e->fpn_lateral_deferred = value != 0;
+  else if (!strcmp(name, "fpn_levels_deferred")) {
+    MCG_CHECK_ARG(value >= 0 && value <= 15 && !(value & 1 && value > 1), "fpn_levels_deferred: 0, 1 or a mask of 2 (P3) | 4 (P4) | 8 (P5) (got %d)", value);
+    e->fpn_levels_deferred = value;
+  }
   else if (!strcmp(name, "wino_tile")) { MCG_CHECK_ARG(value >= -1 && value <= 3, "wino_tile must be -1 (by grid size) .. 3"); e->wino_tile = value; }
   else if (!strcmp(name, "range_audit")) {
     MCG_CHECK_ARG(!mcg_is16(e->dt) || !value, "range_audit: f32-storage engines only (MCG_F32, MCG_F16X3)");
@@ -479,9 +485,10 @@
   return MCG_OK;
 }
 
-struct TrunkKeep { char *inner, *c2, *l1; };
+struct TrunkKeep { char *inner, *c2, *l1, *lin[4]; };
+static const TrunkKeep kNoKeep = {nullptr, nullptr, nullptr, {nullptr, nullptr, nullptr, nullptr}};
 static int trunk_chunk(mcg_engine* e, hipStream_t s, const float* img, int f0, int n, int H, int W, void* const pyr[4], char* wsbase,
-                       bool backbone_only = false, const TrunkKeep tk = TrunkKeep{nullptr, nullptr, nullptr}) {
+                       bool backbone_only = false, const TrunkKeep tk = kNoKeep) {
   const mcg_dtype dt = e->dt;
   const size_t es = esize(dt);
   TrunkWs t = trunk_layout(dt, n, H, W, wsbase);
@@ -492,6 +499,8 @@
     t.c[0] = tk.c2 + (size_t)f0 * (H / 4) * (W / 4) * 256 * es;
     t.l[1] = tk.l1 + (size_t)f0 * (H / 8) * (W / 8) * 256 * es;
   }
+  for (int i = 1; i < 4; ++i)
+    if (tk.lin[i]) t.l[i] = tk.lin[i] + (size_t)f0 * ((H / 4) >> i) * ((W / 4) >> i) * 256 * es;
   MCG_TRY(stem_forward_ctx(s, dt, img + (size_t)f0 * 3 * H * W, e->stem.w, e->stem.bias, t.x0, n, H, W, t.stem_ws, t.stem_bytes, e->ctx));
   AuditCursor au{e, s, 0, e->audit_dev != nullptr && e->audit_names.empty()};
   audit_tensor(au, t.x0, (long long)n * (H / 4) * (W / 4) * 64, "stem");
@@ -530,6 +539,7 @@
     audit_tensor(au, t.l[i], (long long)n * hs[i] * wsz[i] * 256, "fpn.lateral%d (+ top-down)", i);
   }
   for (int i = inner0 ? 1 : 0; i < 4; ++i) {
+    if (tk.lin[i]) continue;
     char* dst = (char*)pyr[i] + (size_t)f0 * hs[i] * wsz[i] * 256 * es;
     MCG_TRY(conv_call(e, s, dt, e->fpn_out[i], t.l[i], n, hs[i], wsz[i], dst, 0, nullptr, MCG_RES_NONE, 0, 0));
     audit_tensor(au, dst, (long long)n * hs[i] * wsz[i] * 256, "fpn.P%d", i + 2);
@@ -586,6 +596,10 @@
   bool lateral;
   char *c2, *l1;
   int *istate, *icount, *ilist;
+  int level_mask;
+  char* lin[4];
+  int *fstate[4], *fcount[4], *flist[4];
+  int clear_n;
   size_t total;
 };
 static bool fpn_deferred_on(const mcg_engine* e, int N, int H, int W) {
@@ -600,6 +614,17 @@
   return e->fpn_lateral_deferred && fpn_deferred_on(e, N, H, W) && e->pw_single && e->ctx.tile < 0 && cw.wf && cw.bias && cw.k == 1 && cw.stride == 1 &&
          cw.pad == 0 && h % 2 == 0 && w % 2 == 0 &&
          pw_single_x3_blocks_applicable(cw.cin, cw.cout, h, w, (long long)N * h * w, (long long)N * (h / 2) * (w / 2));
+}
+static int fpn_levels_deferred_mask(const mcg_engine* e, int N, int H, int W) {
+  if (!e->fpn_levels_deferred || !fpn_deferred_on(e, N, H, W)) return 0;
+  const int want = e->fpn_levels_deferred == 1 ? mcg_engine::kDeferLevelsDefault : e->fpn_levels_deferred;
+  int mask = 0;
+  for (int i = 1; i < 4; ++i) {
+    const mcg_conv_weights& cw = e->fpn_out[i];
+    const int h = (H / 4) >> i, w = (W / 4) >> i;
+    if (((want >> i) & 1) && wino_kind(e, e->dt, cw, N, h, w, MCG_RES_NONE) == 2 && wino_x3_frames_applicable(N, h, w, cw.cin, cw.cout)) mask |= 1 << i;
+  }
+  return mask;
 }
 static DeferSlot defer_layout(const mcg_engine* e, int N, int H, int W, char* base) {
   DeferSlot d;
@@ -612,9 +637,21 @@
     d.inner = take((size_t)N * (H / 4) * (W / 4) * 256 * esize(e->dt));
     d.nblk = N * wino_x3_blocks_per_frame(H / 4, W / 4);
     d.lateral = fpn_lateral_deferred_on(e, N, H, W);
-    const size_t per = (size_t)d.nblk + e->num_stages;
-    d.state = (int*)take(sizeof(int) * per * (d.lateral ? 2 : 1));
+    d.level_mask = fpn_levels_deferred_mask(e, N, H, W);
+    const size_t per = (size_t)d.nblk + e->num_stages, fper = (size_t)N + e->num_stages;
+    size_t ints = per * (d.lateral ? 2 : 1);
+    const size_t fints0 = ints;
+    for (int i = 1; i < 4; ++i) ints += ((d.level_mask >> i) & 1) ? fper : 0;
+    d.clear_n = (int)ints;
+    d.state = (int*)take(sizeof(int) * ints);
     d.count = d.state ? d.state + d.nblk : nullptr;
+    for (int i = 1, k = 0; i < 4; ++i) {
+      if (!((d.level_mask >> i) & 1)) continue;
+      d.fstate[i] = d.state ? d.state + fints0 + fper * k : nullptr;
+      d.fcount[i] = d.fstate[i] ? d.fstate[i] + N : nullptr;
+      d.flist[i] = (int*)take(sizeof(int) * (size_t)N * e->num_stages);
+      ++k;
+    }
     d.list = (int*)take(sizeof(int) * (size_t)d.nblk * e->num_stages);
     if (d.lateral) {
       d.istate = d.state ? d.state + per : nullptr;
@@ -623,6 +660,8 @@
       d.c2 = take((size_t)N * (H / 4) * (W / 4) * 256 * esize(e->dt));
       d.l1 = take((size_t)N * (H / 8) * (W / 8) * 256 * esize(e->dt));
     }
+    for (int i = 1; i < 4; ++i)
+      if ((d.level_mask >> i) & 1) d.lin[i] = (i == 1 && d.lateral) ? d.l1 : take((size_t)N * ((H / 4) >> i) * ((W / 4) >> i) * 256 * esize(e->dt));
   }
   d.total = off;
   return d;
@@ -661,7 +700,7 @@
 }
 
 static int trunk_forward(mcg_engine* e, mcg_stream s_, const float* img, int N, int H, int W, int chunk,
-                         void* const pyramid[4], void* ws, size_t ws_bytes, bool backbone_only, const TrunkKeep tk = TrunkKeep{nullptr, nullptr, nullptr}) {
+                         void* const pyramid[4], void* ws, size_t ws_bytes, bool backbone_only, const TrunkKeep tk = kNoKeep) {
   MCG_CHECK_ARG(e && img && (pyramid || backbone_only) && ws, "mcg_backbone_fpn_forward: null pointer");
   MCG_TRY(check_shape(N, H, W));
   std::lock_guard<std::mutex> lock(e->mu);
@@ -739,6 +778,25 @@
   wp.wscale = wscale;
   if (launch_wino_x3_blocks((hipStream_t)s, wp, block_list, block_count, max_blocks, grid_cap)) {
     mcg_set_error("mcg_conv3x3_wino_x3_blocks: launch failed");
+    return MCG_ERR_HIP;
+  }
+  return MCG_OK;
+}
+
+extern "C" int mcg_conv3x3_wino_x3_frames(mcg_stream s, const float* x, const void* u, const float* bias, float* y, int frames, int H, int W,
+                                          int Cin, int Cout, const int* frame_list, const int* frame_count, int grid_cap) {
+  MCG_CHECK_ARG(x && u && y && frame_list && frame_count, "mcg_conv3x3_wino_x3_frames: null pointer");
+  MCG_CHECK_ARG(grid_cap >= 0, "mcg_conv3x3_wino_x3_frames: grid_cap >= 0 (got %d)", grid_cap);
+  if (H <= 0 || W <= 0 || !wino_x3_frames_applicable(frames, H, W, Cin, Cout)) {
+    mcg_set_error("mcg_conv3x3_wino_x3_frames: unsupported shape (frames=%d %dx%d, %d -> %d channels): Cin %% 32, Cout %% 128, 2 <= W <= 30, a frame's rows of a tile within the window buffer, operands within 2 GiB",
+                  frames, H, W, Cin, Cout);
+    return MCG_ERR_UNSUPPORTED;
+  }
+  WinoParams wp;
+  memset(&wp, 0, sizeof(wp));
+  wp.x = x; wp.u = u; wp.bias = bias; wp.y = y; wp.H = H; wp.W = W; wp.frames = frames; wp.Cin = Cin; wp.Cout = Cout;
+  if (launch_wino_x3_frames((hipStream_t)s, wp, frame_list, frame_count, grid_cap)) {
+    mcg_set_error("mcg_conv3x3_wino_x3_frames: launch failed");
     return MCG_ERR_HIP;
   }
   return MCG_OK;
@@ -811,10 +869,21 @@
   return MCG_OK;
 }
 
-static int defer_stage_forward(const mcg_engine* e, hipStream_t s, const DeferSlot& d, int st, const float* boxes, int N, int h, int w) {
+static int defer_stage_forward(const mcg_engine* e, hipStream_t s, const DeferSlot& d, int st, const float* boxes, int N, const int fh[4],
+                               const int fw[4]) {
   const mcg_conv_weights& cw = e->fpn_out[0];
+  const int h = fh[0], w = fw[0];
   int* list = d.list + (size_t)st * d.nblk;
-  MCG_TRY(launch_roi_mark(s, boxes, N * 3, 3, 0, h, w, 4, d.state, list, d.count + st));
+  int *fstate[4] = {nullptr, nullptr, nullptr, nullptr}, *flist[4] = {nullptr, nullptr, nullptr, nullptr}, *fcount[4] = {nullptr, nullptr, nullptr, nullptr};
+  for (int i = 1; i < 4; ++i)
+    if ((d.level_mask >> i) & 1) { fstate[i] = d.fstate[i]; flist[i] = d.flist[i] + (size_t)st * N; fcount[i] = d.fcount[i] + st; }
+  MCG_TRY(launch_roi_mark(s, boxes, N * 3, 3, 0, h, w, 4, d.state, list, d.count + st, fstate, flist, fcount));
+  for (int i = 1; i < 4; ++i) {
+    if (!fstate[i]) continue;
+    const mcg_conv_weights& fc = e->fpn_out[i];
+    ProfRec* frec = prof_begin_wino(e->ctx, s, fc, (long long)N * fh[i] * fw[i], st == 0);
+    MCG_TRY(launch_done(frec, s, launch_wino_x3_frames(s, wino_params(fc, 2, d.lin[i], N, fh[i], fw[i], d.p[i], 0), flist[i], fcount[i]), "wino_x3 frames"));
+  }
   if (d.lateral) {
     const mcg_conv_weights& lw = e->lateral[0];
     int* ilist = d.ilist + (size_t)st * d.nblk;
@@ -849,9 +918,9 @@
   char* obj_in = c.obj_a; char* obj_out = c.obj_b;
   float* b_in = c.boxes_a; float* b_out = c.boxes_b;
   const bool defer = d && d->deferred;
-  if (defer) MCG_TRY(launch_defer_clear(s, d->state, (d->nblk + e->num_stages) * (d->lateral ? 2 : 1)));
+  if (defer) MCG_TRY(launch_defer_clear(s, d->state, d->clear_n));
   for (int st = 0; st < e->num_stages; ++st) {
-    if (defer) MCG_TRY(defer_stage_forward(e, s, *d, st, b_in, N, fh[0], fw[0]));
+    if (defer) MCG_TRY(defer_stage_forward(e, s, *d, st, b_in, N, fh, fw));
     MCG_TRY(launch_roi_align(s, e->dt, pyramid, fh, fw, strides, 256, b_in, N * 3, 3, frame_of, pyramid_frames, c.roi, nullptr));
     float* bdst = (st == e->num_stages - 1) ? boxes_out : b_out;
     MCG_TRY(stage_forward_ctx(s, e->dt, &e->stage_w[(size_t)st * MCG_SW_COUNT], c.roi, obj_in, b_in, N, ct, obj_out, bdst,
@@ -905,7 +974,7 @@
   const DeferSlot d = defer_layout(e, N, H, W, (char*)slot);
   if (slot_bytes < d.total) { mcg_set_error("mcg_backbone_fpn_forward_deferred: slot too small (%zu < %zu)", slot_bytes, d.total); return MCG_ERR_WORKSPACE; }
   return trunk_forward(e, s, img, N, H, W, chunk, d.p, ws, ws_bytes, false,
-                       TrunkKeep{d.deferred ? d.inner : nullptr, d.lateral ? d.c2 : nullptr, d.lateral ? d.l1 : nullptr});
+                       TrunkKeep{d.deferred ? d.inner : nullptr, d.lateral ? d.c2 : nullptr, d.lateral ? d.l1 : nullptr, {nullptr, d.lin[1], d.lin[2], d.lin[3]}});
 }
 
 extern "C" int mcg_deferred_pyramid_state(const mcg_engine* e, void* slot, int N, int H, int W, void** inner, int** flags, int** counts, int** lists,
@@ -919,6 +988,18 @@
   if (lists) *lists = d.ilist;
   if (blocks) *blocks = d.nblk;
   if (lateral_deferred) *lateral_deferred = d.lateral ? 1 : 0;
+  return MCG_OK;
+}
+
+extern "C" int mcg_deferred_pyramid_frame_state(const mcg_engine* e, void* slot, int N, int H, int W, int level, int** flags, int** counts,
+                                                int** lists, int* frame_deferred) {
+  MCG_CHECK_ARG(e && slot && level >= 1 && level <= 3, "mcg_deferred_pyramid_frame_state: null pointer or level outside 1 .. 3");
+  MCG_TRY(check_shape(N, H, W));
+  const DeferSlot d = defer_layout(e, N, H, W, (char*)slot);
+  if (flags) *flags = d.fstate[level];
+  if (counts) *counts = d.fcount[level];
+  if (lists) *lists = d.flist[level];
+  if (frame_deferred) *frame_deferred = (d.level_mask >> level) & 1;
   return MCG_OK;
 }
 
diff --git a/mcgaze_amd/csrc/roi_align.hip b/mcgaze_amd/csrc/roi_align.hip
--- a/mcgaze_amd/csrc/roi_align.hip
+++ b/mcgaze_amd/csrc/roi_align.hip
@@ -81,14 +81,20 @@
 }
 
 constexpr int kMarkMaxBlocks = 64;
+struct FrameMark { int *state[4], *list[4], *count[4]; };
 __global__ __launch_bounds__(256) void roi_mark_kernel(const float* __restrict__ boxes, int boxes_per_frame, int level_deferred, int H, int W,
                                                        float ss, int* __restrict__ state, int* __restrict__ list, int* __restrict__ count,
-                                                       float finest_scale) {
+                                                       float finest_scale, const FrameMark fm) {
   constexpr int P = 7, S = 2, NS = P * S;
   __shared__ int s_hit[2][kMarkMaxBlocks];
   const int box = blockIdx.x, tid = threadIdx.x;
   const float x1 = boxes[box * 4 + 0], y1 = boxes[box * 4 + 1], x2 = boxes[box * 4 + 2], y2 = boxes[box * 4 + 3];
-  if (roi_level(x1, y1, x2, y2, finest_scale) != level_deferred) return;
+  const int level = roi_level(x1, y1, x2, y2, finest_scale);
+  if (tid == 0 && fm.state[level]) {
+    const int f = box / boxes_per_frame;
+    if (atomicCAS(&fm.state[level][f], 0, 1) == 0) fm.list[level][atomicAdd(fm.count[level], 1)] = f;
+  }
+  if (level != level_deferred) return;
   const int by_n = (H + 7) / 8, bx_n = (W + 7) / 8;
   if (tid < 2 * kMarkMaxBlocks) s_hit[tid / kMarkMaxBlocks][tid % kMarkMaxBlocks] = 0;
   __syncthreads();
@@ -150,10 +156,15 @@
   return MCG_OK;
 }
 int launch_roi_mark(hipStream_t s, const float* boxes, int num_boxes, int boxes_per_frame, int level, int H, int W, int stride, int* state,
-                    int* list, int* count) {
+                    int* list, int* count, int* const* frame_state, int* const* frame_list, int* const* frame_count) {
   MCG_CHECK_ARG(roi_mark_supported(H, W), "roi_mark: deferred level of %dx%d pixels exceeds %d blocks per axis", H, W, kMarkMaxBlocks);
+  FrameMark fm;
+  for (int l = 0; l < 4; ++l) {
+    const bool on = frame_state && frame_list && frame_count && frame_state[l] && frame_list[l] && frame_count[l];
+    fm.state[l] = on ? frame_state[l] : nullptr; fm.list[l] = on ? frame_list[l] : nullptr; fm.count[l] = on ? frame_count[l] : nullptr;
+  }
   hipLaunchKernelGGL(roi_mark_kernel, dim3(num_boxes), dim3(256), 0, s, boxes, boxes_per_frame, level, H, W, 1.0f / (float)stride, state, list,
-                     count, 56.f);
+                     count, 56.f, fm);
   MCG_CHECK_LAUNCH("roi_mark");
   return MCG_OK;
 }
@@ -162,7 +173,17 @@
   MCG_CHECK_ARG(boxes && state && list && count, "mcg_roi_mark_blocks: null pointer");
   MCG_CHECK_ARG(num_boxes > 0 && boxes_per_frame > 0, "mcg_roi_mark_blocks: empty box set");
   MCG_CHECK_ARG(level >= 0 && level <= 3 && H > 0 && W > 0 && stride > 0, "mcg_roi_mark_blocks: bad level (level=%d %dx%d stride=%d)", level, H, W, stride);
-  return launch_roi_mark((hipStream_t)s, boxes, num_boxes, boxes_per_frame, level, H, W, stride, state, list, count);
+  return launch_roi_mark((hipStream_t)s, boxes, num_boxes, boxes_per_frame, level, H, W, stride, state, list, count, nullptr, nullptr, nullptr);
+}
+extern "C" int mcg_roi_mark_frames(mcg_stream s, const float* boxes, int num_boxes, int boxes_per_frame, int level, int* state, int* list,
+                                   int* count) {
+  MCG_CHECK_ARG(boxes && state && list && count, "mcg_roi_mark_frames: null pointer");
+  MCG_CHECK_ARG(num_boxes > 0 && boxes_per_frame > 0 && num_boxes % boxes_per_frame == 0,
+                "mcg_roi_mark_frames: whole frames of boxes (num_boxes=%d boxes_per_frame=%d)", num_boxes, boxes_per_frame);
+  MCG_CHECK_ARG(level >= 0 && level <= 3, "mcg_roi_mark_frames: bad level %d", level);
+  int *fs[4] = {nullptr, nullptr, nullptr, nullptr}, *fl[4] = {nullptr, nullptr, nullptr, nullptr}, *fc[4] = {nullptr, nullptr, nullptr, nullptr};
+  fs[level] = state; fl[level] = list; fc[level] = count;
+  return launch_roi_mark((hipStream_t)s, boxes, num_boxes, boxes_per_frame, -1, 8, 8, 1, nullptr, nullptr, nullptr, fs, fl, fc);
 }
 extern "C" int mcg_inner_mark_blocks(mcg_stream s, const int* out_list, const int* out_count, int H, int W, int nblk, int* state, int* list,
                                      int* count) {
diff --git a/mcgaze_amd/csrc/wino_x3.hpp b/mcgaze_amd/csrc/wino_x3.hpp
--- a/mcgaze_amd/csrc/wino_x3.hpp
+++ b/mcgaze_amd/csrc/wino_x3.hpp
@@ -607,6 +607,16 @@
     if (logical < units) wino_x3w_tile<1, true>(p, logical);
   }
 }
+template <int NB>
+__global__ __launch_bounds__(256, 1) void wino_x3w_frames_kernel(const WinoParams p) {
+  const int per = p.tpf * p.n_tiles;
+  const int units = __builtin_amdgcn_readfirstlane(min(max(*p.blk_count, 0), p.frames)) * per;
+  for (int u = blockIdx.x; u < units; u += gridDim.x) {
+    const int e = u / per;
+    const int f = __builtin_amdgcn_readfirstlane(p.blk_list[e]);
+    if ((unsigned)f < (unsigned)p.frames) wino_x3w_tile<NB, false>(p, f * per + (u - e * per));
+  }
+}
 
 static inline int wino_x3_tile_groups(int g, int shape) { return g == 2 ? ((shape == 0 || shape == 3) ? 128 : (shape == 1 ? 64 : 32)) : (shape == 0 ? 64 : 32); }
 static inline int wino_x3_tile_channels(int shape) { return (shape == 0 || shape == 3) ? 128 : 64; }
@@ -675,6 +685,29 @@
   hipLaunchKernelGGL(wino_x3w_blocks_kernel, dim3(grid > 0 ? grid : 1), dim3(256), wnx::W_LDS, s, p);
   return hipGetLastError() == hipSuccess ? 0 : 1;
 }
+static inline bool wino_x3_frames_applicable(int frames, int H, int W, int Cin, int Cout) {
+  if (!wino_x3_operands_ok(frames, H, W, Cin, Cout)) return false;
+  const int pcs = wino_x3_pieces(W, 2);
+  return pcs <= 2 && wino_x3_max_rows(H, W, wino_x3_tile_groups(2, 3), 2, false) * wino_x3_nb_template(pcs) * 1024 <= wnx::wcap(2, 4);
+}
+static inline int launch_wino_x3_frames(hipStream_t s, WinoParams p, const int* list, const int* count, int cap = 0) {
+  if (!wino_x3_frames_applicable(p.frames, p.H, p.W, p.Cin, p.Cout)) return 1;
+  const int nb = wino_x3_nb_template(wino_x3_pieces(p.W, 2));
+  int cus;
+  if (nb == 1 ? kernel_ready<wino_x3w_frames_kernel<1>>(wnx::W_LDS, &cus) : kernel_ready<wino_x3w_frames_kernel<2>>(wnx::W_LDS, &cus)) return 1;
+  p.PW = (p.W + 1) / 2;
+  p.gpf = p.H * p.PW;
+  p.total_pairs = p.frames * p.gpf;
+  p.n_tiles = p.Cout / 128;
+  p.tpf = (p.gpf + 127) / 128;
+  p.blk_list = list; p.blk_count = count;
+  const long long units = (long long)p.frames * p.tpf * p.n_tiles;
+  int grid = units < cus ? (int)units : cus;
+  if (cap > 0 && grid > cap) grid = cap;
+  if (nb == 1) hipLaunchKernelGGL(wino_x3w_frames_kernel<1>, dim3(grid > 0 ? grid : 1), dim3(256), wnx::W_LDS, s, p);
+  else hipLaunchKernelGGL(wino_x3w_frames_kernel<2>, dim3(grid > 0 ? grid : 1), dim3(256), wnx::W_LDS, s, p);
+  return hipGetLastError() == hipSuccess ? 0 : 1;
+}
 static const int kWinoMinGrid = 130;
 static inline int launch_wino_x3(hipStream_t s, WinoParams p, int shape = -1, int g = 2) {
   const int mode = wino_x3_mode(p.frames, p.H, p.W, p.Cin, p.Cout, g);
diff --git a/mcgaze_amd/engine.py b/mcgaze_amd/engine.py
--- a/mcgaze_amd/engine.py
+++ b/mcgaze_amd/engine.py
@@ -171,6 +171,32 @@
     L.check(lib.mcg_conv3x3_wino_x3_blocks(_stream(), _ptr(x), _ptr(u), _ptr(bias), _ptr(out), N, H, W, Cin, Cout, int(relu), wscale,
                                            _ptr(blist), _ptr(bcount), blist.numel(), grid_cap), 'mcg_conv3x3_wino_x3_blocks')
     return out
+
+
+def conv3x3_wino_frames(x, u, frames, out, bias=None, grid_cap=0):
+    _require_gpu()
+    lib = L.load()
+    N, H, W, Cin = x.shape
+    Cout = out.shape[-1]
+    assert x.dtype == torch.float32 and x.is_contiguous() and out.dtype == torch.float32 and out.is_contiguous() and tuple(out.shape) == (N, H, W, Cout)
+    assert u.numel() * 2 == lib.mcg_conv3x3_wino_x3_weight_bytes(Cin, Cout, 2), (u.numel(), Cin, Cout)
+    flist, fcount = _block_list(frames, x.device)
+    if flist.numel() < N:
+        flist = torch.cat([flist, torch.zeros(N - flist.numel(), dtype=torch.int32, device=x.device)])
+    L.check(lib.mcg_conv3x3_wino_x3_frames(_stream(), _ptr(x), _ptr(u), _ptr(bias), _ptr(out), N, H, W, Cin, Cout, _ptr(flist), _ptr(fcount),
+                                           grid_cap), 'mcg_conv3x3_wino_x3_frames')
+    return out
+
+
+def roi_mark_frames(boxes, level, state=None, flist=None, count=None):
+    _require_gpu()
+    lib = L.load()
+    N, P, _ = boxes.shape
+    assert boxes.dtype == torch.float32
+    state, flist, count = _mark_buffers(N, state, flist, count, boxes.device)
+    L.check(lib.mcg_roi_mark_frames(_stream(), _ptr(boxes.contiguous()), N * P, P, int(level), _ptr(state), _ptr(flist), _ptr(count)),
+            'mcg_roi_mark_frames')
+    return state, flist, count
 
 
 def bottleneck_x3(x, src2, wstream, bias, cn, nsrc, trace=None):
diff --git a/mcgaze_amd/lib.py b/mcgaze_amd/lib.py
--- a/mcgaze_amd/lib.py
+++ b/mcgaze_amd/lib.py
@@ -34,7 +34,8 @@
            'mcg_deferred_pyramid_state', 'mcg_inner_block_neighbours', 'mcg_gaze_targets', 'mcg_gaze_dwell', 'mcg_gaze_targets_poly',
            'mcg_pointwise_stream', 'mcg_pointwise_dyn', 'mcg_pointwise_pair', 'mcg_draw_attention', 'mcg_draw_attention_nv12',
            'mcg_format_labels', 'mcg_draw_labels', 'mcg_draw_labels_nv12', 'mcg_gaze_heat_add', 'mcg_draw_heat', 'mcg_draw_heat_nv12',
-           'mcg_anonymize_heads', 'mcg_anonymize_heads_nv12', 'mcg_roi_mark_blocks', 'mcg_inner_mark_blocks', 'mcg_conv3x3_wino_x3_blocks']
+           'mcg_anonymize_heads', 'mcg_anonymize_heads_nv12', 'mcg_roi_mark_blocks', 'mcg_inner_mark_blocks', 'mcg_conv3x3_wino_x3_blocks',
+           'mcg_conv3x3_wino_x3_frames', 'mcg_roi_mark_frames', 'mcg_deferred_pyramid_frame_state']
 LABEL_CHARS = 24
 LETTERBOX_U8, LETTERBOX_F16, LETTERBOX_F32 = 0, 1, 2
 
@@ -216,6 +217,9 @@
     lib.mcg_conv3x3_wino_x3.argtypes = [vp, vp, vp, vp, vp, i, i, i, i, i, i, i, C.c_float, i]
     lib.mcg_conv3x3_wino_x3_blocks.argtypes = [vp, vp, vp, vp, vp, i, i, i, i, i, i, C.c_float, vp, vp, i, i]
     lib.mcg_roi_mark_blocks.argtypes = [vp, vp, i, i, i, i, i, i, vp, vp, vp]
+    lib.mcg_roi_mark_frames.argtypes = [vp, vp, i, i, i, vp, vp, vp]
+    lib.mcg_conv3x3_wino_x3_frames.argtypes = [vp, vp, vp, vp, vp, i, i, i, i, i, vp, vp, i]
+    lib.mcg_deferred_pyramid_frame_state.argtypes = [vp, vp, i, i, i, i, C.POINTER(vp), C.POINTER(vp), C.POINTER(vp), C.POINTER(i)]
     lib.mcg_inner_mark_blocks.argtypes = [vp, vp, vp, i, i, i, vp, vp, vp]
     lib.mcg_conv3x3_wino_x3_weight_bytes.restype = sz
     lib.mcg_pointwise_stream.argtypes = [vp, i, vp, vp, vp, vp, vp, i, i, i, i, i, i, i, i, i, C.c_float, vp, vp, i]
```

New measurement: 3677 clips/s (median of 6 runs). 1.3% higher.
